# MisEty/X-SLAM

Measured on AMD Instinct MI355X. Metric: fps XKinectFusion 512^3 TSDF 640x480 CSFD @1/2/4/8 GPU; HBM GB/s on integrate, higher is better.
Workload: dtype f32 (complex<f32> CSFD)

## Files before the change

### include/xslam_amd.h

```cpp
#ifndef XSLAM_AMD_H
#define XSLAM_AMD_H
#include <stddef.h>
#include <stdint.h>

#ifdef __cplusplus
extern "C" {
#endif

const char *xs_last_error(void);

unsigned xs_const_div_prepare(float c);
unsigned xs_const_div_state(float c);
int xs_const_div_enable(int on);
int xs_abi_version(void);

int xs_init_volume(float *value, int *weight, float *grad, size_t step_bytes, const int *res, int z0, int z1, void *stream);

int xs_scale_depth(const uint16_t *depth, size_t depth_step, int rows, int cols, float *scaled, size_t scaled_step, void *stream);
int xs_scale_depth_max(const uint16_t *depth, size_t depth_step, int rows, int cols, float *scaled, size_t scaled_step,
                       float *max_dev, void *stream);
size_t xs_depth_tiles_bytes(int rows, int cols);
int xs_scale_depth_tiles(const uint16_t *depth, size_t depth_step, int rows, int cols, float *scaled, size_t scaled_step,
                         float *max_dev, void *tiles_dev, void *stream);
int xs_depth_tiles(const float *scaled, size_t scaled_step, int rows, int cols, void *tiles_dev, void *stream);

int xs_integrate_tsdf_volume(const uint16_t *depth, size_t depth_step, int rows, int cols, const float *intr4, int max_weight,
                             const int *res, float voxel_size, const float *Rv2c18, const float *tv2c6, float tranc_dist,
                             float *value, int *weight, float *grad, size_t vol_step, float *depth_scaled, size_t scaled_step,
                             float threshold, int z0, int z1, unsigned long long *updated_dev, void *stream);
int xs_integrate_scaled(const float *depth_scaled, size_t scaled_step, int rows, int cols, const float *intr4, int max_weight,
                        const int *res, float voxel_size, const float *Rv2c18, const float *tv2c6, float tranc_dist, float *value,
                        int *weight, float *grad, size_t vol_step, float threshold, int z0, int z1,
                        unsigned long long *updated_dev, const float *depth_max_dev, void *workspace, void *stream);
#define XS_INTEGRATE_HEADER_IS_CLEAR 1u
#define XS_INTEGRATE_NO_FOLD 2u
#define XS_INTEGRATE_ALWAYS_STORE 8u
#define XS_INTEGRATE_NO_TILES 32u
#define XS_INTEGRATE_COUNT_CLASSES 64u
#define XS_INTEGRATE_RECLASSIFY_BOXES 128u
#define XS_INTEGRATE_LIST_IS_READY 4u
int xs_integrate_scaled_ex(const float *depth_scaled, size_t scaled_step, int rows, int cols, const float *intr4, int max_weight,
                           const int *res, float voxel_size, const float *Rv2c18, const float *tv2c6, float tranc_dist, float *value,
                           int *weight, float *grad, size_t vol_step, float threshold, int z0, int z1,
                           unsigned long long *updated_dev, const float *depth_max_dev, void *workspace, unsigned flags, void *stream);
int xs_integrate_workspace_clear(void *workspace, void *stream);
int xs_integrate_fold_counts(void *workspace, unsigned long long *updated_dev, void *stream);
int xs_integrate_classify(int rows, int cols, const float *intr4, const int *res, float voxel_size, const float *Rv2c18, const float *tv2c6,
                          float tranc_dist, int z0, int z1, const float *depth_max_dev, void *workspace, float slack_scale, unsigned flags,
                          void *stream);
int xs_integrate_list_covers(int rows, int cols, const float *intr4, const int *res, float voxel_size, const float *Rv2c18_list,
                             const float *tv2c6_list, float slack_scale, const float *Rv2c18, const float *tv2c6);
size_t xs_integrate_workspace_bytes(const int *res, int nz);

typedef struct xs_integrate_opts {
    unsigned struct_bytes;
    unsigned flags;
    const void *depth_tiles;
    void *signmap;
    void *start_event, *stop_event;
} xs_integrate_opts;
int xs_integrate_scaled_ex2(const float *depth_scaled, size_t scaled_step, int rows, int cols, const float *intr4, int max_weight,
                            const int *res, float voxel_size, const float *Rv2c18, const float *tv2c6, float tranc_dist, float *value,
                            int *weight, float *grad, size_t vol_step, float threshold, int z0, int z1,
                            unsigned long long *updated_dev, const float *depth_max_dev, void *workspace, const xs_integrate_opts *opts, void *stream);
int xs_integrate_classify_ex(int rows, int cols, const float *intr4, const int *res, float voxel_size, const float *Rv2c18, const float *tv2c6,
                             float tranc_dist, int z0, int z1, const float *depth_max_dev, void *workspace, float slack_scale,
                             const xs_integrate_opts *opts, void *stream);
typedef struct xs_raycast_opts {
    unsigned struct_bytes;
    int signmap_shift;
    const void *signmap;
    float signmap_tranc_dist;
    float *pyr_vmap1, *pyr_nmap1;
    size_t pyr_step1;
    float *pyr_vmap2, *pyr_nmap2;
    size_t pyr_step2;
    void *completion_event;
    int *steps_dev;
    int pyramid_built;
} xs_raycast_opts;
int xs_raycast_ex(const float *intr4, const float *Rc2v18, const float *tc2v6, const float *Rv2w18, const float *tv2w6,
                  float tranc_dist, const int *res, float voxel_size, const float *value, const float *grad, size_t vol_step,
                  float *vmap, float *nmap, size_t map_step, int rows, int cols, unsigned long long *hits_dev, float *workspace,
                  xs_raycast_opts *opts, void *stream);
int xs_raycast_slab_ex(const float *intr4, const float *Rc2v18, const float *tc2v6, const float *Rv2w18, const float *tv2w6,
                       float tranc_dist, const int *res, float voxel_size, const float *value, const float *grad, size_t vol_step,
                       int zs0, int zs1, int z0, int z1, float *vmap, float *nmap, size_t map_step, int rows, int cols, int *keys_dev,
                       const xs_raycast_opts *opts, void *stream);
int xs_resize_pyramid_ex(const float *vmap0, const float *nmap0, size_t in_step, int rows0, int cols0, float *vmap1, float *nmap1,
                         size_t mid_step, float *vmap2, float *nmap2, size_t out_step, void *completion_event, void *stream);

size_t xs_tsdf_reduce_workspace_bytes(void);
int xs_tsdf_reduce_workspace_init(void *workspace, void *stream);
int xs_compute_local_tsdf_hessian(const float *depth_scaled, size_t scaled_step, int rows, int cols, const float *intr4,
                                  const int *res, float voxel_size, const float *Rv2c36, const float *tv2c12, float tranc_dist,
                                  const float *gt, float *real_out, float *grad_out, float *hess_out, int *count_out, int z0, int z1,
                                  void *workspace, double *out4_dev, void *stream);
int xs_compute_local_tsdf_loss(const float *depth_scaled, size_t scaled_step, int rows, int cols, const float *intr4, const int *res,
                               float voxel_size, const float *Rv2c9, const float *tv2c3, float tranc_dist, const float *gt,
                               float *real_out, int *count_out, int z0, int z1, void *workspace, double *out2_dev, void *stream);

int xs_bilateral_filter(const uint16_t *src, size_t src_step, int rows, int cols, float *dst, size_t dst_step, void *stream);
int xs_pyr_down(const float *src, size_t src_step, int src_rows, int src_cols, float *dst, size_t dst_step, void *stream);
int xs_create_vmap(const float *intr4, const float *depth, size_t depth_step, int rows, int cols, float *vmap, size_t vmap_step,
                   void *stream);
int xs_create_nmap(const float *vmap, float *nmap, size_t map_step, int rows, int cols, void *stream);
int xs_create_vnmaps(int levels, const float *intr4s, const float *const *depths, const size_t *depth_steps, int rows0, int cols0,
                     float *const *vmaps, float *const *nmaps, const size_t *map_steps, void *stream);
int xs_create_vnmaps_real(int levels, const float *intr4s, const float *const *depths, const size_t *depth_steps, int rows0, int cols0,
                          float *const *vmaps, float *const *nmaps, const size_t *map_steps, float *const *vreal, float *const *nreal,
                          const size_t *real_steps, void *stream);
int xs_resize_vmap(const float *in, size_t in_step, int src_rows, int src_cols, float *out, size_t out_step, void *stream);
int xs_resize_nmap(const float *in, size_t in_step, int src_rows, int src_cols, float *out, size_t out_step, void *stream);
int xs_resize_pyramid(const float *vmap0, const float *nmap0, size_t in_step, int rows0, int cols0, float *vmap1, float *nmap1,
                      size_t mid_step, float *vmap2, float *nmap2, size_t out_step, void *stream);

int xs_raycast(const float *intr4, const float *Rc2v18, const float *tc2v6, const float *Rv2w18, const float *tv2w6,
               float tranc_dist, const int *res, float voxel_size, const float *value, const float *grad, size_t vol_step,
               float *vmap, float *nmap, size_t map_step, int rows, int cols, unsigned long long *hits_dev, float *workspace,
               void *stream);

int xs_raycast_signmap_shift(const float *intr4, float voxel_size, float tranc_dist);
size_t xs_signmap_bytes(const int *res, int shift);
int xs_signmap_reset(void *signmap, const int *res, int shift, float tranc_dist, void *stream);
int xs_signmap_rebuild(void *signmap, const int *res, int shift, float tranc_dist, const float *value, size_t vol_step, void *stream);
int xs_signmap_rebuild_slab(void *signmap, const int *res, int shift, float tranc_dist, const float *value, size_t vol_step, int zs0, int zs1,
                            void *stream);


int xs_raycast_slab(const float *intr4, const float *Rc2v18, const float *tc2v6, const float *Rv2w18, const float *tv2w6,
                    float tranc_dist, const int *res, float voxel_size, const float *value, const float *grad, size_t vol_step,
                    int zs0, int zs1, int z0, int z1, float *vmap, float *nmap, size_t map_step, int rows, int cols, int *keys_dev,
                    void *stream);
int xs_raycast_compose_mask(const int *own_keys_dev, const int *min_keys_dev, float *vmap, float *nmap, size_t map_step, int rows,
                            int cols, void *stream);
int xs_raycast_compose_finish(const int *min_keys_dev, float *vmap, float *nmap, size_t map_step, int rows, int cols,
                              unsigned long long *hits_dev, void *stream);
size_t xs_raycast_compose_entry_bytes(void);
int xs_raycast_compose_pack(const int *own_keys_dev, const int *min_keys_dev, const float *vmap, const float *nmap, size_t map_step, int rows, int cols,
                            void *entries_dev, int *count_dev, void *stream);
int xs_raycast_compose_scatter(const void *entries_dev, long n, float *vmap, float *nmap, size_t map_step, int rows, int cols, void *stream);

int xs_tsdf_gauss_newton_terms(const float *depth_scaled, size_t scaled_step, int rows, int cols, const float *intr4, const int *res,
                               float voxel_size, const float *Rv2c108, const float *tv2c36, float tranc_dist, const float *gt, int z0, int z1,
                               void *workspace, double *out29_dev, void *stream);
typedef struct xs_gn_opts {
    unsigned struct_bytes;
    unsigned mailbox_seq;
    const void *pose_mailbox;
    double *publish_host;
    unsigned long long publish_seq;
} xs_gn_opts;
int xs_tsdf_gauss_newton_terms_ex(const float *depth_scaled, size_t scaled_step, int rows, int cols, const float *intr4, const int *res,
                                  float voxel_size, const float *Rv2c108, const float *tv2c36, float tranc_dist, const float *gt, int z0, int z1,
                                  void *workspace, double *out29_dev, const xs_gn_opts *opts, void *stream);
size_t xs_gn_publish_bytes(void);
size_t xs_gn_mailbox_bytes(void);
void xs_gn_post_poses(void *mailbox_host, const float *Rv2c108, const float *tv2c36, unsigned mailbox_seq, int cmd);
int xs_gn_publish_sums(const double *sums_dev, int n, double *publish_host, unsigned long long seq, void *stream);

#define XS_BAND_MAX_FRAMES 32
#define XS_BAND_OVER_CAPACITY (-3)
typedef struct xs_band_index {
    unsigned long long *keys;
    float *values;
    long long capacity;
    long long *segs;
    long long count;
    int nblocks;
    int res[3], z0, z1;
} xs_band_index;
size_t xs_tsdf_band_segs_bytes(const int *res, int z0, int z1);
int xs_tsdf_band_build(const float *gt, const int *res, int z0, int z1, xs_band_index *index, void *stream);
size_t xs_tsdf_band_workspace_bytes(int frames);
int xs_tsdf_gauss_newton_terms_band(int frames, const float *const *depth_scaled, size_t scaled_step, int rows, int cols, const float *intr4,
                                    float voxel_size, const float *Rv2c108xF, const float *tv2c36xF, float tranc_dist, const xs_band_index *index,
                                    void *workspace, double *out29xF_dev, void *stream);
size_t xs_tsdf_pose_hessian_workspace_bytes(int frames);
int xs_tsdf_pose_hessian_band(int frames, const float *const *depth_scaled, size_t scaled_step, int rows, int cols, const float *intr4,
                              float voxel_size, const float *Rv2c36x21xF, const float *tv2c12x21xF, float tranc_dist, const xs_band_index *index,
                              void *workspace, double *out29xF_dev, void *stream);
#define XS_SCORE_MAX_POSES 4096
size_t xs_tsdf_score_poses_workspace_bytes(int poses);
int xs_tsdf_score_poses_band(int poses, const float *depth_scaled, size_t scaled_step, int rows, int cols, const float *intr4,
                             float voxel_size, const float *Rv2c9xP, const float *tv2c3xP, float tranc_dist,
                             const xs_band_index *index, void *workspace, double *out2xP_dev, void *stream);

size_t xs_view_grid_bytes(const int *res);
int xs_view_grid_build(const float *value, const int *weight, size_t vol_step, const int *res, int min_weight, void *grid, void *stream);
int xs_view_grid_expand(const void *grid, const int *res, unsigned char *states_dev, void *stream);
#define XS_VIEW_MAX_POSES 4096
typedef struct xs_view_opts {
    unsigned struct_bytes;
    int rays_x, rays_y;
    float t_near, t_far;
    float step;
} xs_view_opts;
int xs_score_views(int poses, const float *Rc2v9xP, const float *tc2v3xP, const float *intr4, int rows, int cols, const int *res,
                   float voxel_size, const void *grid, const xs_view_opts *opts, unsigned *out4xP_dev, void *stream);

#define XS_CLEARANCE_MAX_RADIUS 255
size_t xs_clearance_bytes(const int *res);
size_t xs_clearance_workspace_bytes(const int *res);
int xs_clearance_build(const void *grid, const int *res, int max_radius, int unknown_blocks, void *workspace, unsigned short *field_dev, void *stream);
#define XS_REACH_MAX_SEEDS 64
size_t xs_reach_bytes(const int *res);
int xs_reach_passable(const void *grid, const unsigned short *field_dev, const int *res, int r2, void *reach, void *stream);
int xs_reach_flood(const void *grid, const unsigned short *field_dev, const int *res, int r2, const int *seeds3xN, int seeds, void *reach,
                   int *rounds_out, void *stream);
int xs_reach_expand(const void *reach, const int *res, int passable, unsigned char *out_dev, void *stream);
#define XS_REACH_MAX_SNAP 16
int xs_reach_query(int n, const float *points3xN_dev, const int *res, float voxel_size, const void *reach, int over_passable,
                   const unsigned short *field_dev, int snap, unsigned char *reachable_dev, unsigned short *clear2_dev, int *voxel3xN_dev,
                   void *stream);

#define XS_TRAVEL_NONE 65535
#define XS_TRAVEL_MAX 65534
#define XS_TRAVEL_MAX_TARGETS 64
size_t xs_travel_bytes(const int *res);
size_t xs_travel_workspace_bytes(void);
int xs_travel_build(const void *reach, const int *res, const int *seeds3xN, int seeds, int limit, unsigned short *travel_dev, void *workspace,
                    int *rounds_out, void *stream);
int xs_travel_query(int n, const int *voxel3xN_dev, const int *res, const unsigned short *travel_dev, unsigned short *out_dev, void *stream);
int xs_travel_path(int n, const int *target3xN_dev, const int *res, const void *reach, const unsigned short *travel_dev, int limit, int capacity,
                   int *path3_dev, int *len_dev, void *stream);

#define XS_FRONTIER_NONE 0xFFFFFFFFu
#define XS_FRONTIER_RECORD_WORDS 8
size_t xs_frontier_mask_bytes(const int *res);
size_t xs_frontier_label_bytes(const int *res);
size_t xs_frontier_workspace_bytes(const int *res, int capacity);
int xs_frontier_mask(const void *grid, const int *res, void *mask, void *stream);
int xs_frontier_label(const void *mask, const int *res, int cell, unsigned *labels_dev, void *workspace, int *rounds_out, void *stream);
int xs_frontier_clusters(const void *mask, const unsigned *labels_dev, const int *res, int capacity, unsigned long long *records_dev,
                         unsigned *count_dev, unsigned *count_host, void *workspace, void *stream);
int xs_frontier_expand(const void *mask, const int *res, unsigned char *out_dev, void *stream);

size_t xs_extract_workspace_bytes(const int *res);
int xs_extract_points(const float *value, size_t vol_step, const int *res, float voxel_size, int zs0, int z0, int z1, float *points_dev,
                      size_t capacity, void *workspace, size_t *count_host, size_t *found_host, void *stream);
int xs_extract_normals(const float *value, size_t vol_step, const int *res, float voxel_size, int zs0, int zs1, const float *points_dev,
                       size_t n, float *normals_dev, void *stream);

#define XS_MESH_OVER_CAPACITY (-2)
typedef struct xs_mesh_opts {
    unsigned struct_bytes;
    int zs0, zs1;
    int z0, z1;
    int min_weight;
    int want_normals;
    const void *signmap;
    int signmap_shift;
} xs_mesh_opts;
size_t xs_mesh_workspace_bytes(const int *res, const xs_mesh_opts *opts);
int xs_extract_mesh(const float *value, const int *weight, const float *grad, size_t vol_step, const int *res, float voxel_size,
                    const xs_mesh_opts *opts, float *vertices_dev, float *vertex_im_dev, float *normals_dev, unsigned long long *keys_dev,
                    size_t vertex_capacity, int *triangles_dev, size_t triangle_capacity, void *workspace, size_t *vertex_count_host,
                    size_t *triangle_count_host, void *stream);
int xs_mesh_case_table(int cube_case, signed char out16[16]);

size_t xs_icp_workspace_bytes(void);
int xs_icp_workspace_init(void *workspace, void *stream);
#define XS_ICP_PUBLISH_PAIRS ((unsigned long long *)(size_t)1)
#define XS_ICP_PAIRS_BYTES (55 * 16)
int xs_icp_wait_pairs(const void *pairs_host, unsigned long long seq, double *sums55, long long max_spins);
int xs_icp_accumulate(const float *Rcurr18, const float *tcurr6, const float *vmap_curr, const float *nmap_curr,
                      const float *Rprev_inv18, const float *tprev6, const float *intr4, const float *vmap_g_prev,
                      const float *nmap_g_prev, size_t map_step, int rows, int cols, float distThres, float angleThres, int y0, int y1,
                      void *workspace, double *sums_dev, unsigned long long *done_flag, unsigned long long done_seq, void *stream);
size_t xs_icp_records_bytes(void);
int xs_icp_records_count(int cols, int y0, int y1);
int xs_icp_accumulate_records(const float *Rcurr18, const float *tcurr6, const void *mailbox, unsigned mailbox_seq, const float *vmap_curr,
                              const float *nmap_curr, const float *Rprev_inv18, const float *tprev6, const float *intr4, const float *vmap_g_prev,
                              const float *nmap_g_prev, size_t map_step, int rows, int cols, float distThres, float angleThres, int y0, int y1,
                              double *records_host, unsigned long long seq, void *stream);
int xs_icp_sum_records(const double *records_host, int count, unsigned long long seq, double *sums55, long long max_spins);

int xs_icp_gate_selftest(const float *z2n_dev, int n, float thres, int or_equal, unsigned *counts_dev, void *stream);
size_t xs_icp_mailbox_bytes(void);
int xs_icp_mailbox_alloc(void **mailbox, int *in_device_memory);
int xs_icp_mailbox_free(void *mailbox, int in_device_memory);
int xs_icp_accumulate_posted(const void *mailbox, unsigned mailbox_seq, const float *vmap_curr, const float *nmap_curr,
                             const float *Rprev_inv18, const float *tprev6, const float *intr4, const float *vmap_g_prev,
                             const float *nmap_g_prev, size_t map_step, int rows, int cols, float distThres, float angleThres, int y0,
                             int y1, void *workspace, double *sums_dev, unsigned long long *done_flag, unsigned long long done_seq,
                             void *stream);
void xs_icp_post_pose(void *mailbox_host, const float *Rcurr18, const float *tcurr6, unsigned mailbox_seq, int cmd);
int xs_icp_accumulate_real(const float *Rcurr18, const float *tcurr6, const float *vmap_curr, const float *nmap_curr,
                           const float *vmap_curr_real, const float *nmap_curr_real, size_t real_step, const float *Rprev_inv18,
                           const float *tprev6, const float *intr4, const float *vmap_g_prev, const float *nmap_g_prev, size_t map_step,
                           int rows, int cols, float distThres, float angleThres, int y0, int y1, void *workspace, double *sums_dev,
                           unsigned long long *done_flag, unsigned long long done_seq, void *stream);
int xs_icp_accumulate_posted_real(const void *mailbox, unsigned mailbox_seq, const float *vmap_curr, const float *nmap_curr,
                                  const float *vmap_curr_real, const float *nmap_curr_real, size_t real_step, const float *Rprev_inv18,
                                  const float *tprev6, const float *intr4, const float *vmap_g_prev, const float *nmap_g_prev,
                                  size_t map_step, int rows, int cols, float distThres, float angleThres, int y0, int y1, void *workspace,
                                  double *sums_dev, unsigned long long *done_flag, unsigned long long done_seq, void *stream);
size_t xs_icp_pose_state_bytes(void);
int xs_icp_iterate(const float *Rcurr18, const float *tcurr6, const float *vmap_curr, const float *nmap_curr,
                   const float *Rprev_inv18, const float *tprev6, const float *intr4, const float *vmap_g_prev,
                   const float *nmap_g_prev, size_t map_step, int rows, int cols, float distThres, float angleThres, void *workspace,
                   double *sums_dev, double *sums_host, void *pose_state, void *pose_state_host, unsigned long long *done_flag,
                   unsigned long long done_seq, void *stream);
int xs_estimate_combined(const float *Rcurr18, const float *tcurr6, const float *vmap_curr, const float *nmap_curr,
                         const float *Rprev_inv18, const float *tprev6, const float *intr4, const float *vmap_g_prev,
                         const float *nmap_g_prev, size_t map_step, int rows, int cols, float distThres, float angleThres,
                         void *workspace, double *sums_dev, double *A72_host, double *b12_host, long long *inliers, void *stream);
void xs_icp_unpack(const double *sums54, double *A72, double *b12);

int xs_csfd_array_op(int which, int our, const float *a, const float *b, float *out, long n, void *stream);
int xs_dcsfd_f1(const float *x, const float *y, float *out, long n, void *stream);
int xs_complex_table(int dual, int op, const float *a, const float *b, float *out, long n, void *stream);

#ifdef __cplusplus
}
#endif
#endif
```

### x-slam_amd/capi.py

```python
import ctypes as C
import os

import numpy as np

_HERE = os.path.dirname(os.path.abspath(__file__))
LIB_PATH = os.path.join(_HERE, "libxslam_hip.so")

_vp = C.c_void_p
_sz = C.c_size_t
_f32p = C.POINTER(C.c_float)
_i32p = C.POINTER(C.c_int)
_f64p = C.POINTER(C.c_double)


class XsError(RuntimeError):
    pass


def _load():
    if not os.path.exists(LIB_PATH):
        raise ImportError(
            f"{LIB_PATH} not found: build the HIP extension first (python -c 'import __graft_entry__ as g; g.build()' "
            "or make -C x-slam_amd/csrc).  There is no CPU fallback.")
    return C.CDLL(LIB_PATH)


_lib = _load()

class IntegrateOpts(C.Structure):
    _fields_ = [("struct_bytes", C.c_uint), ("flags", C.c_uint), ("depth_tiles", C.c_void_p), ("signmap", C.c_void_p),
                ("start_event", C.c_void_p), ("stop_event", C.c_void_p)]


class RaycastOpts(C.Structure):
    _fields_ = [("struct_bytes", C.c_uint), ("signmap_shift", C.c_int), ("signmap", C.c_void_p), ("signmap_tranc_dist", C.c_float),
                ("pyr_vmap1", C.c_void_p), ("pyr_nmap1", C.c_void_p), ("pyr_step1", C.c_size_t), ("pyr_vmap2", C.c_void_p), ("pyr_nmap2", C.c_void_p),
                ("pyr_step2", C.c_size_t), ("completion_event", C.c_void_p), ("steps_dev", C.c_void_p), ("pyramid_built", C.c_int)]


class MeshOpts(C.Structure):
    _fields_ = [("struct_bytes", C.c_uint), ("zs0", C.c_int), ("zs1", C.c_int), ("z0", C.c_int), ("z1", C.c_int), ("min_weight", C.c_int),
                ("want_normals", C.c_int), ("signmap", C.c_void_p), ("signmap_shift", C.c_int)]


class BandIndex(C.Structure):
    _fields_ = [("keys", C.c_void_p), ("values", C.c_void_p), ("capacity", C.c_longlong), ("segs", C.c_void_p), ("count", C.c_longlong),
                ("nblocks", C.c_int), ("res", C.c_int * 3), ("z0", C.c_int), ("z1", C.c_int)]


class ViewOpts(C.Structure):
    _fields_ = [("struct_bytes", C.c_uint), ("rays_x", C.c_int), ("rays_y", C.c_int), ("t_near", C.c_float), ("t_far", C.c_float), ("step", C.c_float)]


_SIGS = {
    "xs_view_grid_bytes": (_sz, [_i32p]),
    "xs_view_grid_build": (C.c_int, [_vp, _vp, _sz, _i32p, C.c_int, _vp, _vp]),
    "xs_view_grid_expand": (C.c_int, [_vp, _i32p, _vp, _vp]),
    "xs_score_views": (C.c_int, [C.c_int, _f32p, _f32p, _f32p, C.c_int, C.c_int, _i32p, C.c_float, _vp, C.POINTER(ViewOpts), _vp, _vp]),
    "xs_clearance_bytes": (_sz, [_i32p]),
    "xs_clearance_workspace_bytes": (_sz, [_i32p]),
    "xs_clearance_build": (C.c_int, [_vp, _i32p, C.c_int, C.c_int, _vp, _vp, _vp]),
    "xs_reach_bytes": (_sz, [_i32p]),
    "xs_reach_passable": (C.c_int, [_vp, _vp, _i32p, C.c_int, _vp, _vp]),
    "xs_reach_flood": (C.c_int, [_vp, _vp, _i32p, C.c_int, _i32p, C.c_int, _vp, _i32p, _vp]),
    "xs_reach_expand": (C.c_int, [_vp, _i32p, C.c_int, _vp, _vp]),
    "xs_reach_query": (C.c_int, [C.c_int, _vp, _i32p, C.c_float, _vp, C.c_int, _vp, C.c_int, _vp, _vp, _vp, _vp]),
    "xs_travel_bytes": (_sz, [_i32p]),
    "xs_travel_workspace_bytes": (_sz, []),
    "xs_travel_build": (C.c_int, [_vp, _i32p, _i32p, C.c_int, C.c_int, _vp, _vp, _i32p, _vp]),
    "xs_travel_query": (C.c_int, [C.c_int, _vp, _i32p, _vp, _vp, _vp]),
    "xs_travel_path": (C.c_int, [C.c_int, _vp, _i32p, _vp, _vp, C.c_int, C.c_int, _vp, _vp, _vp]),
    "xs_frontier_mask_bytes": (_sz, [_i32p]),
    "xs_frontier_label_bytes": (_sz, [_i32p]),
    "xs_frontier_workspace_bytes": (_sz, [_i32p, C.c_int]),
    "xs_frontier_mask": (C.c_int, [_vp, _i32p, _vp, _vp]),
    "xs_frontier_label": (C.c_int, [_vp, _i32p, C.c_int, _vp, _vp, _i32p, _vp]),
    "xs_frontier_clusters": (C.c_int, [_vp, _vp, _i32p, C.c_int, _vp, _vp, C.POINTER(C.c_uint), _vp, _vp]),
    "xs_frontier_expand": (C.c_int, [_vp, _i32p, _vp, _vp]),
    "xs_integrate_scaled_ex2": (C.c_int, [_vp, _sz, C.c_int, C.c_int, _f32p, C.c_int, _i32p, C.c_float, _f32p, _f32p, C.c_float, _vp, _vp, _vp,
                                         _sz, C.c_float, C.c_int, C.c_int, _vp, _vp, _vp, C.POINTER(IntegrateOpts), _vp]),
    "xs_integrate_classify_ex": (C.c_int, [C.c_int, C.c_int, _f32p, _i32p, C.c_float, _f32p, _f32p, C.c_float, C.c_int, C.c_int, _vp, _vp,
                                           C.c_float, C.POINTER(IntegrateOpts), _vp]),
    "xs_raycast_ex": (C.c_int, [_f32p, _f32p, _f32p, _f32p, _f32p, C.c_float, _i32p, C.c_float, _vp, _vp, _sz, _vp, _vp, _sz,
                                C.c_int, C.c_int, _vp, _vp, C.POINTER(RaycastOpts), _vp]),
    "xs_raycast_slab_ex": (C.c_int, [_f32p, _f32p, _f32p, _f32p, _f32p, C.c_float, _i32p, C.c_float, _vp, _vp, _sz, C.c_int, C.c_int,
                                     C.c_int, C.c_int, _vp, _vp, _sz, C.c_int, C.c_int, _vp, C.POINTER(RaycastOpts), _vp]),
    "xs_resize_pyramid_ex": (C.c_int, [_vp, _vp, _sz, C.c_int, C.c_int, _vp, _vp, _sz, _vp, _vp, _sz, _vp, _vp]),
    "xs_last_error": (C.c_char_p, []),
    "xs_abi_version": (C.c_int, []),
    "xs_init_volume": (C.c_int, [_vp, _vp, _vp, _sz, _i32p, C.c_int, C.c_int, _vp]),
    "xs_scale_depth": (C.c_int, [_vp, _sz, C.c_int, C.c_int, _vp, _sz, _vp]),
    "xs_integrate_tsdf_volume": (C.c_int, [_vp, _sz, C.c_int, C.c_int, _f32p, C.c_int, _i32p, C.c_float, _f32p, _f32p, C.c_float,
                                           _vp, _vp, _vp, _sz, _vp, _sz, C.c_float, C.c_int, C.c_int, _vp, _vp]),
    "xs_integrate_scaled": (C.c_int, [_vp, _sz, C.c_int, C.c_int, _f32p, C.c_int, _i32p, C.c_float, _f32p, _f32p, C.c_float,
                                      _vp, _vp, _vp, _sz, C.c_float, C.c_int, C.c_int, _vp, _vp, _vp, _vp]),
    "xs_integrate_scaled_ex": (C.c_int, [_vp, _sz, C.c_int, C.c_int, _f32p, C.c_int, _i32p, C.c_float, _f32p, _f32p, C.c_float, _vp, _vp, _vp,
                                        _sz, C.c_float, C.c_int, C.c_int, _vp, _vp, _vp, C.c_uint, _vp]),
    "xs_integrate_workspace_clear": (C.c_int, [_vp, _vp]),
    "xs_integrate_fold_counts": (C.c_int, [_vp, _vp, _vp]),
    "xs_integrate_classify": (C.c_int, [C.c_int, C.c_int, _f32p, _i32p, C.c_float, _f32p, _f32p, C.c_float, C.c_int, C.c_int, _vp, _vp,
                                        C.c_float, C.c_uint, _vp]),
    "xs_integrate_list_covers": (C.c_int, [C.c_int, C.c_int, _f32p, _i32p, C.c_float, _f32p, _f32p, C.c_float, _f32p, _f32p]),
    "xs_integrate_workspace_bytes": (_sz, [_i32p, C.c_int]),
    "xs_scale_depth_max": (C.c_int, [_vp, _sz, C.c_int, C.c_int, _vp, _sz, _vp, _vp]),
    "xs_scale_depth_tiles": (C.c_int, [_vp, _sz, C.c_int, C.c_int, _vp, _sz, _vp, _vp, _vp]),
    "xs_depth_tiles": (C.c_int, [_vp, _sz, C.c_int, C.c_int, _vp, _vp]),
    "xs_depth_tiles_bytes": (_sz, [C.c_int, C.c_int]),
    "xs_tsdf_reduce_workspace_bytes": (_sz, []),
    "xs_tsdf_band_segs_bytes": (_sz, [_i32p, C.c_int, C.c_int]),
    "xs_tsdf_band_build": (C.c_int, [_vp, _i32p, C.c_int, C.c_int, C.POINTER(BandIndex), _vp]),
    "xs_tsdf_band_workspace_bytes": (_sz, [C.c_int]),
    "xs_tsdf_gauss_newton_terms_band": (C.c_int, [C.c_int, C.POINTER(_vp), _sz, C.c_int, C.c_int, _f32p, C.c_float, _f32p, _f32p, C.c_float,
                                                  C.POINTER(BandIndex), _vp, _vp, _vp]),
    "xs_tsdf_pose_hessian_workspace_bytes": (_sz, [C.c_int]),
    "xs_tsdf_pose_hessian_band": (C.c_int, [C.c_int, C.POINTER(_vp), _sz, C.c_int, C.c_int, _f32p, C.c_float, _f32p, _f32p, C.c_float,
                                            C.POINTER(BandIndex), _vp, _vp, _vp]),
    "xs_tsdf_score_poses_workspace_bytes": (_sz, [C.c_int]),
    "xs_tsdf_score_poses_band": (C.c_int, [C.c_int, _vp, _sz, C.c_int, C.c_int, _f32p, C.c_float, _f32p, _f32p, C.c_float, C.POINTER(BandIndex), _vp,
                                           _vp, _vp]),
    "xs_tsdf_reduce_workspace_init": (C.c_int, [_vp, _vp]),
    "xs_compute_local_tsdf_hessian": (C.c_int, [_vp, _sz, C.c_int, C.c_int, _f32p, _i32p, C.c_float, _f32p, _f32p, C.c_float, _vp,
                                                _vp, _vp, _vp, _vp, C.c_int, C.c_int, _vp, _vp, _vp]),
    "xs_compute_local_tsdf_loss": (C.c_int, [_vp, _sz, C.c_int, C.c_int, _f32p, _i32p, C.c_float, _f32p, _f32p, C.c_float, _vp,
                                             _vp, _vp, C.c_int, C.c_int, _vp, _vp, _vp]),
    "xs_bilateral_filter": (C.c_int, [_vp, _sz, C.c_int, C.c_int, _vp, _sz, _vp]),
    "xs_pyr_down": (C.c_int, [_vp, _sz, C.c_int, C.c_int, _vp, _sz, _vp]),
    "xs_create_vmap": (C.c_int, [_f32p, _vp, _sz, C.c_int, C.c_int, _vp, _sz, _vp]),
    "xs_create_nmap": (C.c_int, [_vp, _vp, _sz, C.c_int, C.c_int, _vp]),
    "xs_create_vnmaps": (C.c_int, [C.c_int, _f32p, C.POINTER(_vp), C.POINTER(_sz), C.c_int, C.c_int, C.POINTER(_vp), C.POINTER(_vp),
                                   C.POINTER(_sz), _vp]),
    "xs_create_vnmaps_real": (C.c_int, [C.c_int, _f32p, C.POINTER(_vp), C.POINTER(_sz), C.c_int, C.c_int, C.POINTER(_vp), C.POINTER(_vp),
                                        C.POINTER(_sz), C.POINTER(_vp), C.POINTER(_vp), C.POINTER(_sz), _vp]),
    "xs_resize_vmap": (C.c_int, [_vp, _sz, C.c_int, C.c_int, _vp, _sz, _vp]),
    "xs_resize_nmap": (C.c_int, [_vp, _sz, C.c_int, C.c_int, _vp, _sz, _vp]),
    "xs_raycast": (C.c_int, [_f32p, _f32p, _f32p, _f32p, _f32p, C.c_float, _i32p, C.c_float, _vp, _vp, _sz, _vp, _vp, _sz,
                             C.c_int, C.c_int, _vp, _vp, _vp]),
    "xs_raycast_slab": (C.c_int, [_f32p, _f32p, _f32p, _f32p, _f32p, C.c_float, _i32p, C.c_float, _vp, _vp, _sz, C.c_int, C.c_int,
                                  C.c_int, C.c_int, _vp, _vp, _sz, C.c_int, C.c_int, _vp, _vp]),
    "xs_raycast_compose_mask": (C.c_int, [_vp, _vp, _vp, _vp, _sz, C.c_int, C.c_int, _vp]),
    "xs_raycast_compose_finish": (C.c_int, [_vp, _vp, _vp, _sz, C.c_int, C.c_int, _vp, _vp]),
    "xs_raycast_compose_entry_bytes": (_sz, []),
    "xs_raycast_compose_pack": (C.c_int, [_vp, _vp, _vp, _vp, _sz, C.c_int, C.c_int, _vp, _vp, _vp]),
    "xs_raycast_compose_scatter": (C.c_int, [_vp, C.c_long, _vp, _vp, _sz, C.c_int, C.c_int, _vp]),
    "xs_resize_pyramid": (C.c_int, [_vp, _vp, _sz, C.c_int, C.c_int, _vp, _vp, _sz, _vp, _vp, _sz, _vp]),
    "xs_tsdf_gauss_newton_terms": (C.c_int, [_vp, _sz, C.c_int, C.c_int, _f32p, _i32p, C.c_float, _f32p, _f32p, C.c_float, _vp, C.c_int,
                                             C.c_int, _vp, _vp, _vp]),
    "xs_tsdf_gauss_newton_terms_ex": (C.c_int, [_vp, _sz, C.c_int, C.c_int, _f32p, _i32p, C.c_float, _f32p, _f32p, C.c_float, _vp, C.c_int,
                                                C.c_int, _vp, _vp, _vp, _vp]),
    "xs_gn_publish_bytes": (_sz, []),
    "xs_gn_mailbox_bytes": (_sz, []),
    "xs_gn_post_poses": (None, [_vp, _f32p, _f32p, C.c_uint, C.c_int]),
    "xs_gn_publish_sums": (C.c_int, [_vp, C.c_int, _vp, C.c_ulonglong, _vp]),
    "xs_extract_workspace_bytes": (_sz, [_i32p]),
    "xs_extract_points": (C.c_int, [_vp, _sz, _i32p, C.c_float, C.c_int, C.c_int, C.c_int, _vp, _sz, _vp, C.POINTER(_sz), C.POINTER(_sz), _vp]),
    "xs_extract_normals": (C.c_int, [_vp, _sz, _i32p, C.c_float, C.c_int, C.c_int, _vp, _sz, _vp, _vp]),
    "xs_mesh_workspace_bytes": (_sz, [_i32p, C.POINTER(MeshOpts)]),
    "xs_extract_mesh": (C.c_int, [_vp, _vp, _vp, _sz, _i32p, C.c_float, C.POINTER(MeshOpts), _vp, _vp, _vp, _vp, _sz, _vp, _sz, _vp,
                                  C.POINTER(_sz), C.POINTER(_sz), _vp]),
    "xs_mesh_case_table": (C.c_int, [C.c_int, C.c_void_p]),
    "xs_icp_wait_pairs": (C.c_int, [_vp, C.c_ulonglong, _vp, C.c_longlong]),
    "xs_icp_workspace_bytes": (_sz, []),
    "xs_icp_workspace_init": (C.c_int, [_vp, _vp]),
    "xs_icp_accumulate": (C.c_int, [_f32p, _f32p, _vp, _vp, _f32p, _f32p, _f32p, _vp, _vp, _sz, C.c_int, C.c_int, C.c_float,
                                    C.c_float, C.c_int, C.c_int, _vp, _vp, _vp, C.c_ulonglong, _vp]),
    "xs_icp_pose_state_bytes": (_sz, []),
    "xs_icp_mailbox_bytes": (_sz, []),
    "xs_icp_mailbox_alloc": (C.c_int, [C.POINTER(C.c_void_p), C.POINTER(C.c_int)]),
    "xs_icp_mailbox_free": (C.c_int, [_vp, C.c_int]),
    "xs_icp_accumulate_posted": (C.c_int, [_vp, C.c_uint, _vp, _vp, _f32p, _f32p, _f32p, _vp, _vp, _sz, C.c_int, C.c_int, C.c_float,
                                           C.c_float, C.c_int, C.c_int, _vp, _vp, _vp, C.c_ulonglong, _vp]),
    "xs_icp_post_pose": (None, [_vp, _f32p, _f32p, C.c_uint, C.c_int]),
    "xs_icp_accumulate_real": (C.c_int, [_f32p, _f32p, _vp, _vp, _vp, _vp, _sz, _f32p, _f32p, _f32p, _vp, _vp, _sz, C.c_int, C.c_int, C.c_float,
                                         C.c_float, C.c_int, C.c_int, _vp, _vp, _vp, C.c_ulonglong, _vp]),
    "xs_icp_accumulate_posted_real": (C.c_int, [_vp, C.c_uint, _vp, _vp, _vp, _vp, _sz, _f32p, _f32p, _f32p, _vp, _vp, _sz, C.c_int, C.c_int,
                                                C.c_float, C.c_float, C.c_int, C.c_int, _vp, _vp, _vp, C.c_ulonglong, _vp]),
    "xs_icp_records_bytes": (_sz, []),
    "xs_icp_records_count": (C.c_int, [C.c_int, C.c_int, C.c_int]),
    "xs_icp_accumulate_records": (C.c_int, [_f32p, _f32p, _vp, C.c_uint, _vp, _vp, _f32p, _f32p, _f32p, _vp, _vp, _sz, C.c_int, C.c_int, C.c_float,
                                            C.c_float, C.c_int, C.c_int, _vp, C.c_ulonglong, _vp]),
    "xs_icp_sum_records": (C.c_int, [_vp, C.c_int, C.c_ulonglong, _f64p, C.c_longlong]),
    "xs_icp_gate_selftest": (C.c_int, [_vp, C.c_int, C.c_float, C.c_int, _vp, _vp]),
    "xs_icp_iterate": (C.c_int, [_f32p, _f32p, _vp, _vp, _f32p, _f32p, _f32p, _vp, _vp, _sz, C.c_int, C.c_int, C.c_float,
                                 C.c_float, _vp, _vp, _vp, _vp, _vp, _vp, C.c_ulonglong, _vp]),
    "xs_estimate_combined": (C.c_int, [_f32p, _f32p, _vp, _vp, _f32p, _f32p, _f32p, _vp, _vp, _sz, C.c_int, C.c_int, C.c_float,
                                       C.c_float, _vp, _vp, _f64p, _f64p, C.POINTER(C.c_longlong), _vp]),
    "xs_icp_unpack": (None, [_f64p, _f64p, _f64p]),
    "xs_csfd_array_op": (C.c_int, [C.c_int, C.c_int, _vp, _vp, _vp, C.c_long, _vp]),
    "xs_dcsfd_f1": (C.c_int, [_vp, _vp, _vp, C.c_long, _vp]),
    "xs_complex_table": (C.c_int, [C.c_int, C.c_int, _vp, _vp, _vp, C.c_long, _vp]),
    "xs_const_div_prepare": (C.c_uint, [C.c_float]),
    "xs_raycast_signmap_shift": (C.c_int, [_f32p, C.c_float, C.c_float]),
    "xs_signmap_bytes": (C.c_size_t, [_i32p, C.c_int]),
    "xs_signmap_reset": (C.c_int, [_vp, _i32p, C.c_int, C.c_float, _vp]),
    "xs_signmap_rebuild": (C.c_int, [_vp, _i32p, C.c_int, C.c_float, _vp, C.c_size_t, _vp]),
    "xs_signmap_rebuild_slab": (C.c_int, [_vp, _i32p, C.c_int, C.c_float, _vp, C.c_size_t, C.c_int, C.c_int, _vp]),
    "xs_const_div_state": (C.c_uint, [C.c_float]),
    "xs_const_div_enable": (C.c_int, [C.c_int]),
}


def _bind():
    for name, (res, args) in _SIGS.items():
        f = getattr(_lib, name)
        f.restype = res
        f.argtypes = args


_bind()


def const_div_prepare(c):
    return int(_lib.xs_const_div_prepare(float(c)))


def const_div_state(c):
    return int(_lib.xs_const_div_state(float(c)))


def const_div_enable(on):
    return int(_lib.xs_const_div_enable(int(bool(on))))


_prepared = set()


def _prep(*consts):
    for c in consts:
        c = float(np.float32(c))
        if c not in _prepared:
            _prepared.add(c)
            _lib.xs_const_div_prepare(c)


def check(rc):
    if rc != 0:
        raise XsError(f"hip error {rc}: {_lib.xs_last_error().decode()}")


def _fa(x, n):
    a = np.ascontiguousarray(x, dtype=np.float32).reshape(-1)
    assert a.size == n, (a.size, n)
    return a


def _ia(x, n):
    a = np.ascontiguousarray(x, dtype=np.int32).reshape(-1)
    assert a.size == n
    return a


def _ptr(t):
    if t is None:
        return None
    if isinstance(t, int):
        return t
    return t.data_ptr()


def _stream(stream):
    if stream is None:
        return None
    return stream.cuda_stream if hasattr(stream, "cuda_stream") else int(stream)


def abi_version():
    return _lib.xs_abi_version()
# ... 303 lines not shown
    k, R, t, r = _fa(intr, 4), _fa(R, 9 * P), _fa(tc2vxP, 3 * P), _ia(res, 3)
    check(_lib.xs_score_views(P, R.ctypes.data_as(_f32p), t.ctypes.data_as(_f32p), k.ctypes.data_as(_f32p), rows, cols, r.ctypes.data_as(_i32p),
                              voxel_size, _ptr(grid), C.byref(opts) if opts is not None else None, _ptr(out4xP), _stream(stream)))


CLEARANCE_MAX_RADIUS, REACH_MAX_SEEDS, REACH_MAX_SNAP = 255, 64, 16


def _res3(res):
    r = np.ascontiguousarray(res, dtype=np.int32).reshape(-1)
    assert r.size == 3
    return r


def clearance_bytes(res):
    return int(_lib.xs_clearance_bytes(_res3(res).ctypes.data_as(_i32p)))


def clearance_workspace_bytes(res):
    return int(_lib.xs_clearance_workspace_bytes(_res3(res).ctypes.data_as(_i32p)))


def reach_bytes(res):
    return int(_lib.xs_reach_bytes(_res3(res).ctypes.data_as(_i32p)))


def clearance_build(grid, res, max_radius, unknown_blocks, workspace, field, stream=None):
    r = _res3(res)
    check(_lib.xs_clearance_build(_ptr(grid), r.ctypes.data_as(_i32p), int(max_radius), int(unknown_blocks), _ptr(workspace), _ptr(field), _stream(stream)))


def reach_passable(grid, field, res, r2, reach, stream=None):
    r = _res3(res)
    check(_lib.xs_reach_passable(_ptr(grid), _ptr(field), r.ctypes.data_as(_i32p), int(r2), _ptr(reach), _stream(stream)))


def reach_flood(grid, field, res, r2, seeds, reach, stream=None):
    r = _res3(res)
    s = np.ascontiguousarray(seeds, dtype=np.int32).reshape(-1)
    assert s.size % 3 == 0
    rounds = C.c_int(-1)
    check(_lib.xs_reach_flood(_ptr(grid), _ptr(field), r.ctypes.data_as(_i32p), int(r2), s.ctypes.data_as(_i32p), s.size // 3, _ptr(reach),
                              C.byref(rounds), _stream(stream)))
    return int(rounds.value)


def reach_expand(reach, res, out, passable=False, stream=None):
    r = _res3(res)
    check(_lib.xs_reach_expand(_ptr(reach), r.ctypes.data_as(_i32p), int(bool(passable)), _ptr(out), _stream(stream)))


def reach_query(n, points, res, voxel_size, reach, field, reachable, clear2, snap=0, over_passable=False, voxel=None, stream=None):
    r = _res3(res)
    check(_lib.xs_reach_query(int(n), _ptr(points), r.ctypes.data_as(_i32p), float(voxel_size), _ptr(reach), int(bool(over_passable)), _ptr(field),
                              int(snap), _ptr(reachable), _ptr(clear2), _ptr(voxel), _stream(stream)))


TRAVEL_NONE, TRAVEL_MAX, TRAVEL_MAX_TARGETS = 65535, 65534, 64


def travel_bytes(res):
    return int(_lib.xs_travel_bytes(_res3(res).ctypes.data_as(_i32p)))


def travel_workspace_bytes():
    return int(_lib.xs_travel_workspace_bytes())


def travel_build(reach, res, seeds, limit, travel, workspace, stream=None):
    r = _res3(res)
    s = np.ascontiguousarray(seeds, dtype=np.int32).reshape(-1)
    assert s.size % 3 == 0
    rounds = C.c_int(0)
    check(_lib.xs_travel_build(_ptr(reach), r.ctypes.data_as(_i32p), s.ctypes.data_as(_i32p), s.size // 3, int(limit), _ptr(travel), _ptr(workspace),
                               C.byref(rounds), _stream(stream)))
    return int(rounds.value)


def travel_query(n, voxels, res, travel, out, stream=None):
    r = _res3(res)
    check(_lib.xs_travel_query(int(n), _ptr(voxels), r.ctypes.data_as(_i32p), _ptr(travel), _ptr(out), _stream(stream)))


def travel_path(n, targets, res, reach, travel, limit, capacity, path, lengths, stream=None):
    r = _res3(res)
    check(_lib.xs_travel_path(int(n), _ptr(targets), r.ctypes.data_as(_i32p), _ptr(reach), _ptr(travel), int(limit), int(capacity), _ptr(path),
                              _ptr(lengths), _stream(stream)))


FRONTIER_NONE, FRONTIER_RECORD_WORDS = 0xFFFFFFFF, 8


def frontier_mask_bytes(res):
    return int(_lib.xs_frontier_mask_bytes(_res3(res).ctypes.data_as(_i32p)))


def frontier_label_bytes(res):
    return int(_lib.xs_frontier_label_bytes(_res3(res).ctypes.data_as(_i32p)))


def frontier_workspace_bytes(res, capacity=0):
    return int(_lib.xs_frontier_workspace_bytes(_res3(res).ctypes.data_as(_i32p), int(capacity)))


def frontier_mask(grid, res, mask, stream=None):
    r = _res3(res)
    check(_lib.xs_frontier_mask(_ptr(grid), r.ctypes.data_as(_i32p), _ptr(mask), _stream(stream)))


def frontier_label(mask, res, cell, labels, workspace, stream=None):
    r = _res3(res)
    rounds = C.c_int(0)
    check(_lib.xs_frontier_label(_ptr(mask), r.ctypes.data_as(_i32p), int(cell), _ptr(labels), _ptr(workspace), C.byref(rounds), _stream(stream)))
    return int(rounds.value)


def frontier_clusters(mask, labels, res, capacity, records, count, workspace, stream=None):
    r = _res3(res)
    n = C.c_uint(0)
    check(_lib.xs_frontier_clusters(_ptr(mask), _ptr(labels), r.ctypes.data_as(_i32p), int(capacity), _ptr(records), _ptr(count), C.byref(n), _ptr(workspace),
                                    _stream(stream)))
    return int(n.value)


def frontier_expand(mask, res, out, stream=None):
    r = _res3(res)
    check(_lib.xs_frontier_expand(_ptr(mask), r.ctypes.data_as(_i32p), _ptr(out), _stream(stream)))



class GnOpts(C.Structure):
    _fields_ = [("struct_bytes", C.c_uint), ("mailbox_seq", C.c_uint), ("pose_mailbox", C.c_void_p), ("publish_host", C.c_void_p),
                ("publish_seq", C.c_ulonglong)]


def tsdf_gauss_newton_terms_ex(depth_scaled, scaled_step, rows, cols, intr, res, voxel_size, Rv2c6, tv2c6, tranc_dist, gt, workspace, out29,
                               z0=0, z1=None, stream=None, pose_mailbox=None, mailbox_seq=0, publish_host=None, publish_seq=0):
    r = _ia(res, 3)
    k = _fa(intr, 4)
    z1 = int(r[2]) if z1 is None else z1
    o = GnOpts()
    o.struct_bytes = C.sizeof(GnOpts)
    o.mailbox_seq, o.pose_mailbox, o.publish_host, o.publish_seq = mailbox_seq, _ptr(pose_mailbox), _ptr(publish_host), publish_seq
    if Rv2c6 is None:
        pR = pt = None
    else:
        R, t = _fa(Rv2c6, 108), _fa(tv2c6, 36)
        pR, pt = R.ctypes.data_as(_f32p), t.ctypes.data_as(_f32p)
    check(_lib.xs_tsdf_gauss_newton_terms_ex(_ptr(depth_scaled), scaled_step, rows, cols, k.ctypes.data_as(_f32p), r.ctypes.data_as(_i32p),
                                             voxel_size, pR, pt, tranc_dist, _ptr(gt), z0, z1, _ptr(workspace), _ptr(out29), C.byref(o),
                                             _stream(stream)))


def gn_publish_bytes():
    return int(_lib.xs_gn_publish_bytes())


def gn_post_poses(mailbox, Rv2c6, tv2c6, mailbox_seq, cmd=0):
    if Rv2c6 is None:
        _lib.xs_gn_post_poses(_ptr(mailbox), None, None, mailbox_seq, cmd)
    else:
        R, t = _fa(Rv2c6, 108), _fa(tv2c6, 36)
        _lib.xs_gn_post_poses(_ptr(mailbox), R.ctypes.data_as(_f32p), t.ctypes.data_as(_f32p), mailbox_seq, cmd)


def extract_workspace_bytes(res):
    r = _ia(res, 3)
    return _lib.xs_extract_workspace_bytes(r.ctypes.data_as(_i32p))


def extract_points(value, vol_step, res, voxel_size, points, capacity, workspace, zs0=0, z0=0, z1=None, stream=None):
    r = _ia(res, 3)
    z1 = int(r[2]) - 1 if z1 is None else z1
    cnt, found = _sz(0), _sz(0)
    check(_lib.xs_extract_points(_ptr(value), vol_step, r.ctypes.data_as(_i32p), voxel_size, zs0, z0, z1, _ptr(points), capacity,
                                 _ptr(workspace), C.byref(cnt), C.byref(found), _stream(stream)))
    return int(cnt.value), int(found.value)


def extract_normals(value, vol_step, res, voxel_size, points, n, normals, zs0=0, zs1=None, stream=None):
    r = _ia(res, 3)
    zs1 = int(r[2]) if zs1 is None else zs1
    check(_lib.xs_extract_normals(_ptr(value), vol_step, r.ctypes.data_as(_i32p), voxel_size, zs0, zs1, _ptr(points), n, _ptr(normals),
                                  _stream(stream)))


MESH_OVER_CAPACITY = -2


def mesh_opts(z0=0, z1=None, res=None, zs0=0, zs1=0, min_weight=1, want_normals=True, signmap=None, signmap_shift=3):
    o = MeshOpts()
    o.struct_bytes = C.sizeof(MeshOpts)
    o.zs0, o.zs1, o.z0 = zs0, zs1, z0
    o.z1 = int(res[2]) - 1 if z1 is None else z1
    o.min_weight, o.want_normals = min_weight, int(bool(want_normals))
    o.signmap, o.signmap_shift = _ptr(signmap), signmap_shift if signmap is not None else 0
    return o


def mesh_workspace_bytes(res, opts=None):
    r = _ia(res, 3)
    return _lib.xs_mesh_workspace_bytes(r.ctypes.data_as(_i32p), C.byref(opts) if opts is not None else None)


def mesh_case_table(cube_case):
    out = (C.c_byte * 16)()
    check(_lib.xs_mesh_case_table(int(cube_case), out))
    e = [v for v in out if v >= 0]
    return [tuple(e[i:i + 3]) for i in range(0, len(e), 3)]


def extract_mesh_raw(value, weight, grad, vol_step, res, voxel_size, opts, vertices, vertex_im, normals, keys, vcap, triangles, tcap,
                     workspace, stream=None):
    r = _ia(res, 3)
    nv, nt = _sz(0), _sz(0)
    rc = _lib.xs_extract_mesh(_ptr(value), _ptr(weight), _ptr(grad), vol_step, r.ctypes.data_as(_i32p), voxel_size, C.byref(opts),
                              _ptr(vertices), _ptr(vertex_im), _ptr(normals), _ptr(keys), vcap, _ptr(triangles), tcap, _ptr(workspace),
                              C.byref(nv), C.byref(nt), _stream(stream))
    if rc != MESH_OVER_CAPACITY:
        check(rc)
    return rc, int(nv.value), int(nt.value)


def extract_mesh(value, weight, grad, vol_step, res, voxel_size, z0=0, z1=None, zs0=0, zs1=0, min_weight=1, want_normals=True,
                 signmap=None, signmap_shift=3, stream=None):
    import torch
    dev = value.device
    opts = mesh_opts(z0, z1, res, zs0, zs1, min_weight, want_normals, signmap, signmap_shift)
    ws = torch.empty(max(1, mesh_workspace_bytes(res, opts)), dtype=torch.uint8, device=dev)
    args = (value, weight, grad, vol_step, res, voxel_size, opts)
    rc, nv, nt = extract_mesh_raw(*args, None, None, None, None, 0, None, 0, ws, stream)
    f = lambda n: torch.empty((n, 3), dtype=torch.float32, device=dev)
    out = {"vertices": f(nv), "vertex_im": f(nv) if grad is not None else None, "normals": f(nv) if want_normals else None,
           "triangles": torch.empty((nt, 3), dtype=torch.int32, device=dev), "edge_keys": torch.empty(nv, dtype=torch.uint64, device=dev)}
    if rc == MESH_OVER_CAPACITY:
        rc, nv2, nt2 = extract_mesh_raw(*args, out["vertices"], out["vertex_im"], out["normals"], out["edge_keys"], nv, out["triangles"], nt,
                                        ws, stream)
        assert rc == 0 and (nv2, nt2) == (nv, nt), (rc, nv2, nt2, nv, nt)
    return out


def resize_pyramid(vmap0, nmap0, in_step, rows0, cols0, vmap1, nmap1, mid_step, vmap2, nmap2, out_step, stream=None):
    check(_lib.xs_resize_pyramid(_ptr(vmap0), _ptr(nmap0), in_step, rows0, cols0, _ptr(vmap1), _ptr(nmap1), mid_step, _ptr(vmap2), _ptr(nmap2),
                                 out_step, _stream(stream)))


def create_nmap(vmap, nmap, map_step, rows, cols, stream=None):
    check(_lib.xs_create_nmap(_ptr(vmap), _ptr(nmap), map_step, rows, cols, _stream(stream)))


def resize_vmap(src, src_step, src_rows, src_cols, dst, dst_step, stream=None):
    check(_lib.xs_resize_vmap(_ptr(src), src_step, src_rows, src_cols, _ptr(dst), dst_step, _stream(stream)))


def resize_nmap(src, src_step, src_rows, src_cols, dst, dst_step, stream=None):
    check(_lib.xs_resize_nmap(_ptr(src), src_step, src_rows, src_cols, _ptr(dst), dst_step, _stream(stream)))


def raycast(intr, Rc2v, tc2v, Rv2w, tv2w, tranc_dist, res, voxel_size, value, grad, vol_step, vmap, nmap, map_step, rows, cols,
            hits=None, workspace=None, stream=None, **opts):
    if opts:
        o = _ray_opts(opts)
        raycast_ex(intr, Rc2v, tc2v, Rv2w, tv2w, tranc_dist, res, voxel_size, value, grad, vol_step, vmap, nmap, map_step, rows, cols, o, hits=hits,
                   workspace=workspace, stream=stream)
        return o
    r = _ia(res, 3)
    _prep(voxel_size)
    k, a, b, c, d = _fa(intr, 4), _fa(Rc2v, 18), _fa(tc2v, 6), _fa(Rv2w, 18), _fa(tv2w, 6)
    P = lambda x: x.ctypes.data_as(_f32p)
    check(_lib.xs_raycast(P(k), P(a), P(b), P(c), P(d), tranc_dist, r.ctypes.data_as(_i32p), voxel_size, _ptr(value), _ptr(grad),
                          vol_step, _ptr(vmap), _ptr(nmap), map_step, rows, cols, _ptr(hits), _ptr(workspace), _stream(stream)))


def _ray_opts(kw):
    kw = dict(kw)
    if "signmap_shift" in kw:
        kw["shift"] = kw.pop("signmap_shift")
    if "signmap_tranc_dist" in kw:
        kw["tranc_dist"] = kw.pop("signmap_tranc_dist")
    return raycast_opts(**kw)


def raycast_opts(signmap=None, shift=3, tranc_dist=0.0, pyramid=None, completion_event=None, steps=None):
    o = RaycastOpts()
    o.struct_bytes = C.sizeof(RaycastOpts)
    o.signmap, o.signmap_shift, o.signmap_tranc_dist = _ptr(signmap), shift, tranc_dist
    if pyramid is not None:
        o.pyr_vmap1, o.pyr_nmap1, o.pyr_step1, o.pyr_vmap2, o.pyr_nmap2, o.pyr_step2 = (_ptr(pyramid[0]), _ptr(pyramid[1]), pyramid[2],
                                                                                       _ptr(pyramid[3]), _ptr(pyramid[4]), pyramid[5])
    o.completion_event = completion_event.value if hasattr(completion_event, "value") else completion_event
    o.steps_dev = _ptr(steps)
    return o


def raycast_ex(intr, Rc2v, tc2v, Rv2w, tv2w, tranc_dist, res, voxel_size, value, grad, vol_step, vmap, nmap, map_step, rows, cols, opts,
               hits=None, workspace=None, stream=None):
    _prep(voxel_size)
    r = _ia(res, 3)
    k = _fa(intr, 4)
    a, b, c, d = _fa(Rc2v, 18), _fa(tc2v, 6), _fa(Rv2w, 18), _fa(tv2w, 6)
    P = lambda x: x.ctypes.data_as(_f32p)
    check(_lib.xs_raycast_ex(P(k), P(a), P(b), P(c), P(d), tranc_dist, r.ctypes.data_as(_i32p), voxel_size, _ptr(value), _ptr(grad), vol_step,
                             _ptr(vmap), _ptr(nmap), map_step, rows, cols, _ptr(hits), _ptr(workspace), C.byref(opts), _stream(stream)))


def raycast_signmap_shift(intr, voxel_size, tranc_dist):
# ... 212 lines not shown
```

### x-slam_amd/csrc/xs_band.hip

```cpp
#include <hip/hip_runtime.h>
#include <string.h>
#include <type_traits>
#include <vector>
#include "xs_gn_band.h"
#include "../../include/xslam_amd.h"

static_assert(XS_BAND_MAX_FRAMES == 32, "the header's bound");
enum { BAND_RECORD_DOUBLES = 32, BAND_POSES_OFFSET = 256 };
static size_t band_records_offset() { return BAND_POSES_OFFSET + (size_t)XS_BAND_MAX_FRAMES * sizeof(GnPoses); }

__device__ __forceinline__ unsigned long long band_key(int x, int y, int z) {
    return (unsigned long long)x | ((unsigned long long)y << 21) | ((unsigned long long)z << 42);
}

template <bool WRITE>
__global__ void __launch_bounds__(256) k_band_record(const HessArgs a, long long *segs, unsigned long long *keys, unsigned *values) {
    const int lane = threadIdx.x, wave = threadIdx.y;
    const unsigned nseg = gridDim.x * 4u, seg = blockIdx.x * 4u + (unsigned)wave;
    const long long base = WRITE ? segs[seg] : 0;
    long long k = 0;
    walk_band(a, [&](int x, int y, int z, size_t, float gt) {
        if (WRITE) {
            const long long e = base + 64 * k + lane;
            keys[e] = band_key(x, y, z);
            values[e] = __float_as_uint(gt);
        }
        ++k;
    });
    if (!WRITE) {
        const unsigned long long n = wave_sum_u64((unsigned long long)k);
        if (lane == 0) segs[nseg + seg] = (long long)n;
    }
}

struct BandGnArgs {
    HessArgs a;
    const float *depth[XS_BAND_MAX_FRAMES];
    const unsigned long long *keys;
    const float *values;
    const long long *segs;
    const GnPoses *poses;
    double *records;
    unsigned *tickets;
    double *out;
};
__global__ void __launch_bounds__(256) k_band_gauss_newton(const BandGnArgs g) {
    __shared__ GnPoses P;
    const int f = blockIdx.y, lane = threadIdx.x, wave = threadIdx.y;
    const unsigned nblocks = gridDim.x, nseg = 4u * nblocks, seg = blockIdx.x * 4u + (unsigned)wave;
    {
        const float *src = reinterpret_cast<const float *>(g.poses + f);
        float *dst = reinterpret_cast<float *>(&P);
        for (int i = threadIdx.y * 64 + threadIdx.x; i < (int)(sizeof(GnPoses) / sizeof(float)); i += 256) dst[i] = src[i];
        __syncthreads();
    }
    HessArgs a = g.a;
    a.depth = g.depth[f];
    double acc[29];
#pragma unroll
    for (int k = 0; k < 29; ++k) acc[k] = 0.0;
    const long long off = g.segs[seg], n = g.segs[nseg + seg];
    for (long long e = lane; e < n; e += 64) {
        const unsigned long long key = g.keys[off + e];
        const int x = (int)(key & 0x1fffff), y = (int)((key >> 21) & 0x1fffff), z = (int)(key >> 42);
        gn_terms_add(a, P, x, y, z, g.values[off + e], acc);
    }
    block_fold_and_finish_of<29>(acc, g.records + (size_t)f * nblocks * BAND_RECORD_DOUBLES, g.tickets + f, g.out + 29 * f, nullptr, 0, false,
                                 nblocks, blockIdx.x);
}

extern "C" size_t xs_tsdf_band_segs_bytes(const int *res, int z0, int z1) {
    if (!res || z0 < 0 || z1 > res[2] || z1 <= z0) return 0;
    unsigned most = 0;
    for (uintptr_t addr : {(uintptr_t)256, (uintptr_t)4}) {
        HessArgs a; dim3 grid;
        if (hess_tiling(a, res, reinterpret_cast<const float *>(addr), z0, z1, grid, true)) return 0;
        most = grid.x > most ? grid.x : most;
    }
    return (size_t)most * 4 * 2 * sizeof(long long);
}

extern "C" int xs_tsdf_band_build(const float *gt, const int *res, int z0, int z1, xs_band_index *index, void *stream) {
    if (!gt || !res || !index || !index->segs) return xs_set_error(hipErrorInvalidValue, "xs_tsdf_band_build: null pointer");
    if (z0 < 0 || z1 > res[2] || z1 <= z0) return xs_set_error(hipErrorInvalidValue, "xs_tsdf_band_build: bad slab");
    if (index->capacity > 0 && (!index->keys || !index->values)) return xs_set_error(hipErrorInvalidValue, "xs_tsdf_band_build: capacity without arrays");
    if ((long long)res[0] > 0x1fffff || (long long)res[1] > 0x1fffff || (long long)res[2] > 0x3fffff)
        return xs_set_error(hipErrorInvalidValue, "xs_tsdf_band_build: volume too large for the packed keys");
    hipStream_t st = (hipStream_t)stream;
    HessArgs a; dim3 grid;
    memset(&a, 0, sizeof(a));
    int rc = hess_tiling(a, res, gt, z0, z1, grid, true);
    if (rc) return rc;
    const unsigned nseg = grid.x * 4u;
    index->count = 0; index->nblocks = 0;
    hipLaunchKernelGGL(k_band_record<false>, grid, dim3(64, 4), 0, st, a, index->segs, nullptr, nullptr);
    XS_CHECK(hipGetLastError());
    std::vector<long long> segs(2 * (size_t)nseg);
    XS_CHECK(hipMemcpyAsync(segs.data() + nseg, index->segs + nseg, nseg * sizeof(long long), hipMemcpyDeviceToHost, st));
    XS_CHECK(hipStreamSynchronize(st));
    long long total = 0;
    for (unsigned s = 0; s < nseg; ++s) { segs[s] = total; total += segs[nseg + s]; }
    index->count = total;
    index->nblocks = (int)grid.x;
    index->res[0] = res[0]; index->res[1] = res[1]; index->res[2] = res[2];
    index->z0 = z0; index->z1 = z1;
    if (total > index->capacity) return XS_BAND_OVER_CAPACITY;
    XS_CHECK(hipMemcpyAsync(index->segs, segs.data(), nseg * sizeof(long long), hipMemcpyHostToDevice, st));
    hipLaunchKernelGGL(k_band_record<true>, grid, dim3(64, 4), 0, st, a, index->segs, index->keys, reinterpret_cast<unsigned *>(index->values));
    XS_CHECK(hipGetLastError());
    XS_CHECK(hipStreamSynchronize(st));
    return 0;
}

extern "C" size_t xs_tsdf_band_workspace_bytes(int frames) {
    if (frames < 1 || frames > XS_BAND_MAX_FRAMES) return 0;
    return band_records_offset() + (size_t)frames * XS_TSDF_REDUCE_MAX_BLOCKS_C * BAND_RECORD_DOUBLES * sizeof(double);
}

extern "C" int xs_tsdf_gauss_newton_terms_band(int frames, const float *const *depth_scaled, size_t scaled_step, int rows, int cols, const float *intr4,
                                               float voxel_size, const float *Rv2c108xF, const float *tv2c36xF, float tranc_dist,
                                               const xs_band_index *index, void *workspace, double *out29xF_dev, void *stream) {
    if (frames < 1 || frames > XS_BAND_MAX_FRAMES) return xs_set_error(hipErrorInvalidValue, "xs_tsdf_gauss_newton_terms_band: frames outside 1 .. XS_BAND_MAX_FRAMES");
    if (!depth_scaled || !intr4 || !Rv2c108xF || !tv2c36xF || !index || !workspace || !out29xF_dev)
        return xs_set_error(hipErrorInvalidValue, "xs_tsdf_gauss_newton_terms_band: null pointer");
    if (index->nblocks < 1 || index->nblocks > XS_TSDF_REDUCE_MAX_BLOCKS_C || !index->segs || (index->count > 0 && (!index->keys || !index->values)))
        return xs_set_error(hipErrorInvalidValue, "xs_tsdf_gauss_newton_terms_band: the index was not built");
    BandGnArgs g;
    memset(&g, 0, sizeof(g));
    for (int f = 0; f < frames; ++f) {
        if (!depth_scaled[f]) return xs_set_error(hipErrorInvalidValue, "xs_tsdf_gauss_newton_terms_band: null depth");
        g.depth[f] = depth_scaled[f];
    }
    HessArgs &a = g.a;
    a.depth = depth_scaled[0]; a.dstep = scaled_step; a.drows = rows; a.dcols = cols;
    a.voxel_size = voxel_size; a.tranc_dist = tranc_dist; a.tranc_dist_inv = 1.0f / tranc_dist;
    a.intr = Intr{intr4[0], intr4[1], intr4[2], intr4[3]};
    a.X = index->res[0]; a.Y = index->res[1]; a.Z = index->res[2]; a.z0 = index->z0; a.z1 = index->z1;
    std::vector<GnPoses> P((size_t)frames);
    memset(P.data(), 0, P.size() * sizeof(GnPoses));
    for (int f = 0; f < frames; ++f)
        for (int k = 0; k < 6; ++k) { load_mat(Rv2c108xF + 108 * f + 18 * k, P[f].R[k]); load_vec(tv2c36xF + 36 * f + 6 * k, P[f].t[k]); }
    char *ws = static_cast<char *>(workspace);
    g.tickets = reinterpret_cast<unsigned *>(ws);
    g.poses = reinterpret_cast<const GnPoses *>(ws + BAND_POSES_OFFSET);
    g.records = reinterpret_cast<double *>(ws + band_records_offset());
    g.keys = index->keys; g.values = index->values; g.segs = index->segs; g.out = out29xF_dev;
    hipStream_t st = (hipStream_t)stream;
    XS_CHECK(hipMemcpyAsync(ws + BAND_POSES_OFFSET, P.data(), P.size() * sizeof(GnPoses), hipMemcpyHostToDevice, st));
    hipLaunchKernelGGL(k_band_gauss_newton, dim3((unsigned)index->nblocks, (unsigned)frames), dim3(64, 4), 0, st, g);
    XS_CHECK(hipGetLastError());
    return 0;
}

enum { NEWTON_PAIRS = 21, NEWTON_TERMS = 28, NEWTON_POSES_OFFSET = 256 };
static size_t newton_records_offset() { return NEWTON_POSES_OFFSET + (size_t)XS_BAND_MAX_FRAMES * NEWTON_PAIRS * sizeof(HessPoseD); }
static_assert(sizeof(HessPoseD) == 48 * sizeof(float), "36 + 12 floats per dual-complex pose");

struct BandHessArgs {
    HessArgs a;
    const float *depth[XS_BAND_MAX_FRAMES];
    const unsigned long long *keys;
    const float *values;
    long long count;
    const HessPoseD *poses;
    double *records;
    unsigned *tickets;
    double *out;
};
__global__ void __launch_bounds__(256) k_band_pose_hessian(const BandHessArgs g) {
    __shared__ HessPoseD P[NEWTON_PAIRS];
    __shared__ float s_term[NEWTON_TERMS][256];
    const int f = blockIdx.y, lane = threadIdx.x, wave = threadIdx.y, tid = wave * 64 + lane;
    {
        const float *src = reinterpret_cast<const float *>(g.poses + (size_t)f * NEWTON_PAIRS);
        float *dst = reinterpret_cast<float *>(&P[0]);
        for (int i = tid; i < (int)(NEWTON_PAIRS * sizeof(HessPoseD) / sizeof(float)); i += 256) dst[i] = src[i];
        __syncthreads();
    }
    HessArgs a = g.a;
    a.depth = g.depth[f];
    double acc[29];
#pragma unroll
    for (int k = 0; k < 29; ++k) acc[k] = 0.0;
    const long long nchunks = (g.count + 63) / 64;
    for (long long c = (long long)blockIdx.x * 4 + wave; c < nchunks; c += 4ll * gridDim.x) {
        const long long e = c * 64 + lane;
        if (e >= g.count) continue;
        const unsigned long long key = g.keys[e];
        const int x = (int)(key & 0x1fffff), y = (int)((key >> 21) & 0x1fffff), z = (int)(key >> 42);
        const float gt = g.values[e];
        bool ok = true;
        int pa = 0, pb = 0;
#pragma unroll 1
        for (int p = 0; p < NEWTON_PAIRS; ++p) {
            dcfloat loss;
            if (!tsdf_loss_d(a, P[p], x, y, z, gt, loss)) { ok = false; break; }
            s_term[p][tid] = loss.hessian();
            if (pa == pb) s_term[NEWTON_PAIRS + pa][tid] = loss.grad();
            if (p == 0) s_term[27][tid] = loss.value();
            if (++pb == 6) { ++pa; pb = pa; }
        }
        if (!ok) continue;
#pragma unroll
        for (int k = 0; k < NEWTON_TERMS; ++k) acc[k] += (double)s_term[k][tid];
        acc[28] += 1.0;
    }
    block_fold_and_finish_of<29>(acc, g.records + (size_t)f * gridDim.x * BAND_RECORD_DOUBLES, g.tickets + f, g.out + 29 * f, nullptr, 0, false,
                                 gridDim.x, blockIdx.x);
}

extern "C" size_t xs_tsdf_pose_hessian_workspace_bytes(int frames) {
    if (frames < 1 || frames > XS_BAND_MAX_FRAMES) return 0;
    return newton_records_offset() + (size_t)frames * XS_TSDF_REDUCE_MAX_BLOCKS_C * BAND_RECORD_DOUBLES * sizeof(double);
}

extern "C" int xs_tsdf_pose_hessian_band(int frames, const float *const *depth_scaled, size_t scaled_step, int rows, int cols, const float *intr4,
                                         float voxel_size, const float *Rv2c36x21xF, const float *tv2c12x21xF, float tranc_dist,
                                         const xs_band_index *index, void *workspace, double *out29xF_dev, void *stream) {
    if (frames < 1 || frames > XS_BAND_MAX_FRAMES) return xs_set_error(hipErrorInvalidValue, "xs_tsdf_pose_hessian_band: frames outside 1 .. XS_BAND_MAX_FRAMES");
    if (!depth_scaled || !intr4 || !Rv2c36x21xF || !tv2c12x21xF || !index || !workspace || !out29xF_dev)
        return xs_set_error(hipErrorInvalidValue, "xs_tsdf_pose_hessian_band: null pointer");
    if (index->nblocks < 1 || index->count < 0 || index->count > index->capacity || (index->count > 0 && (!index->keys || !index->values)))
        return xs_set_error(hipErrorInvalidValue, "xs_tsdf_pose_hessian_band: the index was not built");
    if (rows < 4 || cols < 4 || scaled_step < (size_t)cols * sizeof(float)) return xs_set_error(hipErrorInvalidValue, "xs_tsdf_pose_hessian_band: bad depth shape");
    BandHessArgs g;
    memset(&g, 0, sizeof(g));
    for (int f = 0; f < frames; ++f) {
        if (!depth_scaled[f]) return xs_set_error(hipErrorInvalidValue, "xs_tsdf_pose_hessian_band: null depth");
        g.depth[f] = depth_scaled[f];
    }
    HessArgs &a = g.a;
    a.depth = depth_scaled[0]; a.dstep = scaled_step; a.drows = rows; a.dcols = cols;
    a.voxel_size = voxel_size; a.tranc_dist = tranc_dist; a.tranc_dist_inv = 1.0f / tranc_dist;
    a.intr = Intr{intr4[0], intr4[1], intr4[2], intr4[3]};
    a.X = index->res[0]; a.Y = index->res[1]; a.Z = index->res[2]; a.z0 = index->z0; a.z1 = index->z1;
    std::vector<HessPoseD> P((size_t)frames * NEWTON_PAIRS);
    for (size_t k = 0; k < P.size(); ++k) {
        const float *p = Rv2c36x21xF + 36 * k, *t = tv2c12x21xF + 12 * k;
        for (int r = 0; r < 3; ++r) {
            P[k].R.data[r].x = dcfloat(p[12 * r + 0], p[12 * r + 1], p[12 * r + 2], p[12 * r + 3]);
            P[k].R.data[r].y = dcfloat(p[12 * r + 4], p[12 * r + 5], p[12 * r + 6], p[12 * r + 7]);
            P[k].R.data[r].z = dcfloat(p[12 * r + 8], p[12 * r + 9], p[12 * r + 10], p[12 * r + 11]);
        }
        P[k].t.x = dcfloat(t[0], t[1], t[2], t[3]);
        P[k].t.y = dcfloat(t[4], t[5], t[6], t[7]);
        P[k].t.z = dcfloat(t[8], t[9], t[10], t[11]);
    }
    const long long nchunks = (index->count + 63) / 64, want = (nchunks + 3) / 4;
    const unsigned nblocks = (unsigned)(want < 1 ? 1 : (want > XS_TSDF_REDUCE_MAX_BLOCKS_C ? XS_TSDF_REDUCE_MAX_BLOCKS_C : want));
    char *ws = static_cast<char *>(workspace);
    g.tickets = reinterpret_cast<unsigned *>(ws);
    g.poses = reinterpret_cast<const HessPoseD *>(ws + NEWTON_POSES_OFFSET);
    g.records = reinterpret_cast<double *>(ws + newton_records_offset());
    g.keys = index->keys; g.values = index->values; g.count = index->count; g.out = out29xF_dev;
    hipStream_t st = (hipStream_t)stream;
    XS_CHECK(hipMemcpyAsync(ws + NEWTON_POSES_OFFSET, P.data(), P.size() * sizeof(HessPoseD), hipMemcpyHostToDevice, st));
    hipLaunchKernelGGL(k_band_pose_hessian, dim3(nblocks, (unsigned)frames), dim3(64, 4), 0, st, g);
    XS_CHECK(hipGetLastError());
    return 0;
}

enum { SCORE_TILE = 64, SCORE_POSES_OFFSET = 256, SCORE_MAX_BLOCKS = 1024, SCORE_RECORD_BYTES = SCORE_TILE * (sizeof(double) + sizeof(unsigned)) };
static_assert(XS_SCORE_MAX_POSES / SCORE_TILE * sizeof(unsigned) == SCORE_POSES_OFFSET, "one ticket per tile in the first 256 bytes");
static_assert(sizeof(HessPoseF) == 12 * sizeof(float), "twelve floats per real pose");
static size_t score_records_offset() { return SCORE_POSES_OFFSET + (size_t)XS_SCORE_MAX_POSES * sizeof(HessPoseF); }

__device__ __forceinline__ float wave_tree_sum_f32(float v) {
    auto dpp = [](float x, auto ctrl) { return __int_as_float(__builtin_amdgcn_update_dpp(0, __float_as_int(x), decltype(ctrl)::value, 0xf, 0xf, false)); };
    v += dpp(v, std::integral_constant<int, 0xb1>());
    v += dpp(v, std::integral_constant<int, 0x4e>());
    v += dpp(v, std::integral_constant<int, 0x141>());
    v += dpp(v, std::integral_constant<int, 0x140>());
    v += __shfl_xor(v, 16, 64);
    v += __shfl_xor(v, 32, 64);
    return v;
}

struct BandScoreArgs {
    HessArgs a;
    const unsigned long long *keys;
    const float *values;
    long long count;
    int poses;
    const HessPoseF *poses_dev;
    char *records;
    unsigned *tickets;
    double *out;
};
__global__ void __launch_bounds__(256) k_band_score_poses(const BandScoreArgs g) {
    __shared__ double s_sum[4][SCORE_TILE];
    __shared__ unsigned s_cnt[4][SCORE_TILE];
    __shared__ unsigned s_last;
    const int lane = threadIdx.x, wave = __builtin_amdgcn_readfirstlane(threadIdx.y), tid = wave * 64 + lane;
    const unsigned nblocks = gridDim.x, bid = blockIdx.x, tile = blockIdx.y;
    const int p0 = (int)tile * SCORE_TILE, np = min(SCORE_TILE, g.poses - p0);
    const HessPoseF *__restrict__ poses = g.poses_dev + p0;
    double acc = 0.0;
    unsigned cnt = 0;
    const long long nchunks = (g.count + 63) / 64;
    for (long long c = (long long)bid * 4 + wave; c < nchunks; c += 4ll * nblocks) {
        const long long e = c * 64 + lane;
        const bool valid = e < g.count;
// ... 103 lines not shown
```

### x-slam_amd/csrc/xs_gn_band.h

```cpp
#pragma once
#include "xs_device.h"
#include "xs_env.h"

using namespace xs;
#if defined(__HIP_DEVICE_COMPILE__) && !defined(__gfx942__) && !defined(__gfx950__)
#error "write-through record publish: gfx942 / gfx950 only (use a release fence + acq_rel ticket on other targets)"
#endif

struct HessArgs {
    const float *depth; size_t dstep; int drows, dcols;
    int X, Y, Z, z0, z1, zchunk;
    float voxel_size, tranc_dist, tranc_dist_inv;
    Intr intr;
    const float *gt;
    double *partials;
    unsigned *ticket;
    double *out;
    float *real_out, *grad_out, *hess_out; int *count_out;
    int tiles_x, tiles_y, tiles_z;
    double *publish; unsigned long long publish_seq;
    const unsigned *mailbox; unsigned mailbox_seq;
    int il;
    int wide;
};
struct HessPoseD { MatD33 R; dcfloat3 t; };
struct HessPoseF { float R[9]; float t[3]; };

enum { XS_TSDF_REDUCE_MAX_BLOCKS_C = 4096 };
enum : unsigned { TICKET_ARRIVED = 1u, TICKET_LEFT = 0x10000u, TICKET_COUNT_MASK = 0xffffu };
template <int NV>
__device__ __forceinline__ void block_fold_and_finish_of(double (&v)[NV], double *partials, unsigned *ticket, double *out, double *publish,
                                                         unsigned long long publish_seq, bool left, unsigned nblocks, unsigned bid) {
    constexpr int STRIDE = NV <= 8 ? 8 : 32;
    __shared__ double sm[4][NV];
    __shared__ unsigned s_last;
    const int tid = threadIdx.y * blockDim.x + threadIdx.x;
    const int lane = tid & 63, wave = tid >> 6;
    if (!left) {
#pragma unroll
        for (int k = 0; k < NV; ++k) {
            const double s = wave_sum_f64(v[k]);
            if (lane == 0) sm[wave][k] = s;
        }
        __syncthreads();
        if (tid < NV) {
            const double s = ((sm[0][tid] + sm[1][tid]) + sm[2][tid]) + sm[3][tid];
            __hip_atomic_store(&partials[(size_t)bid * STRIDE + tid], s, __ATOMIC_RELAXED, __HIP_MEMORY_SCOPE_AGENT);
        }
    }
    static_assert(NV <= 64, "the record is stored by one wave");
    static_assert(XS_TSDF_REDUCE_MAX_BLOCKS_C <= (int)TICKET_COUNT_MASK, "the ticket counts arrivals in sixteen bits");
    if (wave == 0) asm volatile("s_waitcnt vmcnt(0)" ::: "memory");
    if (tid == 0) {
        const unsigned tk = __hip_atomic_fetch_add(ticket, left ? TICKET_ARRIVED + TICKET_LEFT : TICKET_ARRIVED, __ATOMIC_RELAXED, __HIP_MEMORY_SCOPE_AGENT);
        s_last = (tk & TICKET_COUNT_MASK) != nblocks - 1 ? 0u : ((tk >> 16) != 0 || left ? 2u : 1u);
        if (s_last) __builtin_amdgcn_fence(__ATOMIC_ACQUIRE, "agent");
        asm volatile("s_waitcnt vmcnt(0)" ::: "memory");
    }
    __syncthreads();
    if (s_last == 2u) {
        if (tid == 0) {
            __hip_atomic_store(ticket, 0u, __ATOMIC_RELAXED, __HIP_MEMORY_SCOPE_AGENT);
            if (publish) __hip_atomic_store(reinterpret_cast<unsigned long long *>(publish) + 32, publish_seq | (1ull << 63), __ATOMIC_RELAXED, __HIP_MEMORY_SCOPE_SYSTEM);
        }
        return;
    }
    if (s_last) {
        constexpr int G = 256 / STRIDE;
        __shared__ double s_red[G][STRIDE];
        const int c = tid % STRIDE, g = tid / STRIDE;
        const double *p = partials + c;
        double s = 0.0;
        unsigned b = g;
        for (; b + G * 15 < nblocks; b += G * 16) {
            double v[16];
#pragma unroll
            for (int k = 0; k < 16; ++k) v[k] = p[(size_t)(b + G * k) * STRIDE];
#pragma unroll
            for (int k = 0; k < 16; ++k) s += v[k];
        }
        for (; b < nblocks; b += G) s += p[(size_t)b * STRIDE];
        s_red[g][c] = s;
        __syncthreads();
        if (tid < NV) {
            double t = s_red[0][tid];
#pragma unroll
            for (int gg = 1; gg < G; ++gg) t += s_red[gg][tid];
            out[tid] = t;
            if (publish) __hip_atomic_store(&publish[tid], t, __ATOMIC_RELAXED, __HIP_MEMORY_SCOPE_SYSTEM);
        }
        if (tid == 0) __hip_atomic_store(ticket, 0u, __ATOMIC_RELAXED, __HIP_MEMORY_SCOPE_AGENT);
        if (publish && wave == 0) {
            __builtin_amdgcn_fence(__ATOMIC_RELEASE, "");
            if (tid == 0) __hip_atomic_store(reinterpret_cast<unsigned long long *>(publish) + 32, publish_seq, __ATOMIC_RELAXED, __HIP_MEMORY_SCOPE_SYSTEM);
        }
    }
}

template <int NV>
__device__ __forceinline__ void block_fold_and_finish(double (&v)[NV], double *partials, unsigned *ticket, double *out, double *publish = nullptr,
                                                      unsigned long long publish_seq = 0, bool left = false) {
    block_fold_and_finish_of(v, partials, ticket, out, publish, publish_seq, left, gridDim.x * gridDim.y * gridDim.z,
                             blockIdx.x + gridDim.x * (blockIdx.y + gridDim.y * blockIdx.z));
}

struct BandQueue {
    enum { CAP = 128 };
    unsigned long long (*q)[CAP];
    unsigned head, tail;
};
template <class F>
__device__ __forceinline__ void band_queue_take(const HessArgs &a, BandQueue &Q, int wave, int lane, unsigned count, F &&body) {
    asm volatile("s_waitcnt lgkmcnt(0)" ::: "memory");
    if ((unsigned)lane < count) {
        const unsigned long long e = Q.q[wave][(Q.head + lane) % BandQueue::CAP];
        const int x = (int)(e & 0x1fffff), y = (int)((e >> 21) & 0x1fffff), z = (int)(e >> 42);
        const size_t index = ((size_t)(z - a.z0) * a.Y + y) * a.X + x;
        body(x, y, z, index, a.gt[index]);
    }
    Q.head += count;
    asm volatile("s_waitcnt lgkmcnt(0)" ::: "memory");
}
template <class F, class XYZ>
__device__ __forceinline__ void band_queue_append(const HessArgs &a, BandQueue &Q, int wave, int lane, bool mine, XYZ &&xyz, F &&body) {
    const unsigned long long who = __ballot(mine);
    if (!who) return;
    if (mine) {
        const unsigned pos = Q.tail + __popcll(who & ((1ull << lane) - 1ull));
        Q.q[wave][pos % BandQueue::CAP] = xyz();
    }
    Q.tail += (unsigned)__popcll(who);
    if (Q.tail - Q.head >= 64u) band_queue_take(a, Q, wave, lane, 64u, body);
}
typedef float xs_f4 __attribute__((ext_vector_type(4)));
template <class F>
__device__ __forceinline__ void for_band_voxels(const HessArgs &a, BandQueue &Q, int wave, int lane, int x, int y, bool in_volume, int zb, int ze,
                                                F &&body) {
    constexpr int ZB = 32;
    const size_t plane = (size_t)a.Y * a.X;
    const size_t first = in_volume ? (size_t)(zb - a.z0) * plane + (size_t)y * a.X + x : 0;
    for (int zc = zb; zc < ze; zc += ZB) {
        const float *col = a.gt + first + (size_t)(zc - zb) * plane;
        unsigned mask = 0;
        if (in_volume) {
#pragma unroll
            for (int j = 0; j < ZB; ++j) {
                const float g = (zc + j < ze) ? col[(size_t)j * plane] : 0.f;
                if (!(g == 0 || fabsf(g) > 0.95)) mask |= 1u << j;
            }
        }
        if (!__ballot(mask != 0)) continue;
        for (int j = 0; j < ZB; ++j)
            band_queue_append(a, Q, wave, lane, (mask >> j) & 1u,
                              [&] { return (unsigned long long)x | ((unsigned long long)y << 21) | ((unsigned long long)(zc + j) << 42); }, body);
    }
}
template <class F>
__device__ __forceinline__ void for_band_voxels_wide(const HessArgs &a, BandQueue &Q, int wave, int lane, int x0, int y, bool in_volume, int zfirst, int zstep, int zend,
                                                     F &&body) {
    constexpr int ZB = 8;
    const size_t plane = (size_t)a.Y * a.X;
    const int il = a.il;
    auto zof = [&](int zc, int j) { return zc + (j % il) + (j / il) * il * zstep; };
    const float *col = a.gt + (in_volume ? (size_t)(zfirst - a.z0) * plane + (size_t)y * a.X + x0 : 0);
    for (int zc = zfirst; zc < zend; zc += ZB * zstep, col += (size_t)ZB * zstep * plane) {
        unsigned mask = 0;
        if (in_volume) {
            xs_f4 v[ZB];
#pragma unroll
            for (int j = 0; j < ZB; ++j)
                v[j] = (zof(zc, j) < zend) ? __builtin_nontemporal_load(reinterpret_cast<const xs_f4 *>(col + (size_t)(zof(zc, j) - zc) * plane)) : xs_f4{0.f, 0.f, 0.f, 0.f};
#pragma unroll
            for (int j = 0; j < ZB; ++j) {
                if (!(v[j].x == 0 || fabsf(v[j].x) > 0.95)) mask |= 1u << (4 * j);
                if (!(v[j].y == 0 || fabsf(v[j].y) > 0.95)) mask |= 2u << (4 * j);
                if (!(v[j].z == 0 || fabsf(v[j].z) > 0.95)) mask |= 4u << (4 * j);
                if (!(v[j].w == 0 || fabsf(v[j].w) > 0.95)) mask |= 8u << (4 * j);
            }
        }
        if (!__ballot(mask != 0)) continue;
        for (int b = 0; b < 32; ++b)
            band_queue_append(a, Q, wave, lane, (mask >> b) & 1u,
                              [&] { return (unsigned long long)(x0 + (b & 3)) | ((unsigned long long)y << 21) | ((unsigned long long)zof(zc, b >> 2) << 42); }, body);
    }
}
template <class F>
__device__ __forceinline__ void walk_band(const HessArgs &a, F &&body) {
    __shared__ unsigned long long s_queue[4][BandQueue::CAP];
    BandQueue Q{s_queue, 0u, 0u};
    const int lane = threadIdx.x, wave = threadIdx.y;
    const int ntiles = a.tiles_x * a.tiles_y * a.tiles_z;
    const bool skew = a.wide == 2 && (gridDim.x % (unsigned)a.tiles_z) == 0;
    for (int tile = blockIdx.x, round = 0; tile < ntiles; tile += gridDim.x, ++round) {
        if (a.wide == 2) {
            const int G = a.tiles_z, column = tile / G, g = (tile % G + (skew ? round : 0)) % G;
            const int x0 = 4 * (int)threadIdx.x + (column % a.tiles_x) * 256, y = threadIdx.y + (column / a.tiles_x) * 4;
            for_band_voxels_wide(a, Q, wave, lane, x0, y, x0 < a.X && y < a.Y, a.z0 + g * a.il, G, a.z1, body);
            continue;
        }
        const int y = threadIdx.y + ((tile / a.tiles_x) % a.tiles_y) * 4;
        const int zb = a.z0 + (tile / (a.tiles_x * a.tiles_y)) * a.zchunk, ze = min(zb + a.zchunk, a.z1);
        if (a.wide) {
            const int x0 = 4 * (int)threadIdx.x + (tile % a.tiles_x) * 256;
            for_band_voxels_wide(a, Q, wave, lane, x0, y, x0 < a.X && y < a.Y, zb, 1, ze, body);
        } else {
            const int x = threadIdx.x + (tile % a.tiles_x) * 64;
            for_band_voxels(a, Q, wave, lane, x, y, x < a.X && y < a.Y, zb, ze, body);
        }
    }
    band_queue_take(a, Q, wave, lane, Q.tail - Q.head, body);
}

struct GnPoses { MatS33 R[6]; cfloat3 t[6]; };
__device__ __forceinline__ bool tsdf_error_c(const HessArgs &a, const MatS33 &R, const cfloat3 &t, float vgx, float vgy, float vgz, float gt,
                                             cfloat &error) {
    cfloat3 v_g; v_g.x = cfloat(vgx); v_g.y = cfloat(vgy); v_g.z = cfloat(vgz);
    cfloat3 v_c;
    v_c.x = dot(R.data[0], v_g) + t.x;
    v_c.y = dot(R.data[1], v_g) + t.y;
    v_c.z = dot(R.data[2], v_g) + t.z;
    const cfloat inv_z = cfloat(1.0f) / v_c.z;
    if (inv_z.re < 0) return false;
    const cfloat image_x = v_c.x * inv_z * a.intr.fx + a.intr.cx;
    const cfloat image_y = v_c.y * inv_z * a.intr.fy + a.intr.cy;
    const int coo_x = __float2int_rd(image_x.re - 0.5f), coo_y = __float2int_rd(image_y.re - 0.5f);
    if (!(coo_x > 1 && coo_y > 1 && coo_x < a.dcols - 1 && coo_y < a.drows - 1)) return false;
    const int near_x = __float2int_rn(image_x.re), near_y = __float2int_rn(image_y.re);
    cfloat Dp(row_ptr(a.depth, a.dstep, near_y)[near_x]);
    const float d00 = row_ptr(a.depth, a.dstep, coo_y)[coo_x], d10 = row_ptr(a.depth, a.dstep, coo_y)[coo_x + 1];
    const float d01 = row_ptr(a.depth, a.dstep, coo_y + 1)[coo_x], d11 = row_ptr(a.depth, a.dstep, coo_y + 1)[coo_x + 1];
    if (d00 != 0.0f && d01 != 0.0f && d10 != 0.0f && d11 != 0.0f) {
        const cfloat one(1.0f);
        const cfloat fa = image_x - cfloat(float(coo_x) + 0.5f);
        const cfloat fb = image_y - cfloat(float(coo_y) + 0.5f);
        Dp = d00 * (one - fa) * (one - fb) + d10 * fa * (one - fb) + d01 * (one - fa) * fb + d11 * fa * fb;
    }
    if (Dp.re > 5 || Dp.re < 0.2) return false;
    const cfloat xl = (image_x - a.intr.cx) / a.intr.fx;
    const cfloat yl = (image_y - a.intr.cy) / a.intr.fy;
    const cfloat3 v_c_1 = mk3(Dp * xl, Dp * yl, Dp);
    const cfloat distance = norm(v_c_1) - norm(v_c);
    const cfloat gt_distance = cfloat(gt) * a.tranc_dist;
    error = (distance - gt_distance) * a.tranc_dist_inv;
    return !(fabsf(error.re) > 1);
}

__device__ __forceinline__ void gn_terms_add(const HessArgs &a, const GnPoses &P, int xq, int yq, int z, float gt, double (&acc)[29]) {
    const float vgx = (float(xq) + 0.5f) * a.voxel_size, vgy = (float(yq) + 0.5f) * a.voxel_size, vgz = (float(z) + 0.5f) * a.voxel_size;
    cfloat e[6];
    bool ok = true;
#pragma unroll
    for (int k = 0; k < 6; ++k) {
        ok = ok && tsdf_error_c(a, P.R[k], P.t[k], vgx, vgy, vgz, gt, e[k]);
        asm volatile("" : "+v"(e[k].re), "+v"(e[k].im) :: "memory");
    }
    if (!ok) return;
    const double r = (double)e[0].re;
    int s = 0;
#pragma unroll
    for (int j = 0; j < 6; ++j)
#pragma unroll
        for (int k = j; k < 6; ++k) acc[s++] += (double)e[j].im * (double)e[k].im;
#pragma unroll
    for (int k = 0; k < 6; ++k) acc[21 + k] += (double)e[k].im * r;
    acc[27] += r * r;
    acc[28] += 1.0;
}

__device__ __forceinline__ bool tsdf_loss_d(const HessArgs &a, const HessPoseD &P, int xq, int yq, int z, float gt, dcfloat &loss) {
    const dcfloat gt_tsdf(gt);
    const dcfloat vgx((float(xq) + 0.5f) * a.voxel_size);
    const dcfloat vgy((float(yq) + 0.5f) * a.voxel_size);
    const dcfloat vgz((float(z) + 0.5f) * a.voxel_size);
    dcfloat3 v_g; v_g.x = vgx; v_g.y = vgy; v_g.z = vgz;
    dcfloat3 v_c;
    v_c.x = dot(P.R.data[0], v_g) + P.t.x;
    v_c.y = dot(P.R.data[1], v_g) + P.t.y;
    v_c.z = dot(P.R.data[2], v_g) + P.t.z;
    const dcfloat inv_z = dcfloat(1.0f) / v_c.z;
    if (inv_z.value() < 0) return false;
    const dcfloat image_x = v_c.x * inv_z * a.intr.fx + a.intr.cx;
    const dcfloat image_y = v_c.y * inv_z * a.intr.fy + a.intr.cy;
    const int coo_x = __float2int_rd(image_x.value() - 0.5f), coo_y = __float2int_rd(image_y.value() - 0.5f);
    if (!(coo_x > 1 && coo_y > 1 && coo_x < a.dcols - 1 && coo_y < a.drows - 1)) return false;
    const int near_x = __float2int_rn(image_x.value()), near_y = __float2int_rn(image_y.value());
    dcfloat Dp(row_ptr(a.depth, a.dstep, near_y)[near_x]);
    const dcfloat d00(row_ptr(a.depth, a.dstep, coo_y)[coo_x]), d10(row_ptr(a.depth, a.dstep, coo_y)[coo_x + 1]);
    const dcfloat d01(row_ptr(a.depth, a.dstep, coo_y + 1)[coo_x]), d11(row_ptr(a.depth, a.dstep, coo_y + 1)[coo_x + 1]);
    if (d00.value() != 0.0f && d01.value() != 0.0f && d10.value() != 0.0f && d11.value() != 0.0f) {
        const dcfloat one(1.0f);
        const dcfloat fa = image_x - dcfloat(float(coo_x) + 0.5f);
        const dcfloat fb = image_y - dcfloat(float(coo_y) + 0.5f);
        Dp = d00 * (one - fa) * (one - fb) + d10 * fa * (one - fb) + d01 * (one - fa) * fb + d11 * fa * fb;
    }
    if (Dp.value() > 5 || Dp.value() < 0.2) return false;
    const dcfloat xl = (image_x - a.intr.cx) / a.intr.fx;
    const dcfloat yl = (image_y - a.intr.cy) / a.intr.fy;
    dcfloat3 v_c_1; v_c_1.x = Dp * xl; v_c_1.y = Dp * yl; v_c_1.z = Dp;
    const dcfloat distance = norm(v_c_1) - norm(v_c);
    const dcfloat gt_distance = gt_tsdf * a.tranc_dist;
    const dcfloat error = (distance - gt_distance) * a.tranc_dist_inv;
    if (fabsf(error.value()) > 1) return false;
    loss = error * error;
    return true;
}

__device__ __forceinline__ bool tsdf_loss_f(const HessArgs &a, const HessPoseF &P, int xq, int yq, int z, float gt, float &loss) {
    const float vgx = (float(xq) + 0.5f) * a.voxel_size, vgy = (float(yq) + 0.5f) * a.voxel_size, vgz = (float(z) + 0.5f) * a.voxel_size;
    const float vcx = (P.R[0] * vgx + P.R[1] * vgy + P.R[2] * vgz) + P.t[0];
    const float vcy = (P.R[3] * vgx + P.R[4] * vgy + P.R[5] * vgz) + P.t[1];
    const float vcz = (P.R[6] * vgx + P.R[7] * vgy + P.R[8] * vgz) + P.t[2];
    const float inv_z = 1.0f / vcz;
    if (inv_z < 0) return false;
    const float image_x = vcx * inv_z * a.intr.fx + a.intr.cx;
    const float image_y = vcy * inv_z * a.intr.fy + a.intr.cy;
    const int coo_x = __float2int_rd(image_x - 0.5f), coo_y = __float2int_rd(image_y - 0.5f);
    if (!(coo_x > 1 && coo_y > 1 && coo_x < a.dcols - 1 && coo_y < a.drows - 1)) return false;
    const int near_x = __float2int_rn(image_x), near_y = __float2int_rn(image_y);
    float Dp = row_ptr(a.depth, a.dstep, near_y)[near_x];
    const float d00 = row_ptr(a.depth, a.dstep, coo_y)[coo_x], d10 = row_ptr(a.depth, a.dstep, coo_y)[coo_x + 1];
    const float d01 = row_ptr(a.depth, a.dstep, coo_y + 1)[coo_x], d11 = row_ptr(a.depth, a.dstep, coo_y + 1)[coo_x + 1];
    if (d00 != 0.0f && d01 != 0.0f && d10 != 0.0f && d11 != 0.0f) {
        const float one = 1.0f;
        const float fa = image_x - (float(coo_x) + 0.5f), fb = image_y - (float(coo_y) + 0.5f);
        Dp = d00 * (one - fa) * (one - fb) + d10 * fa * (one - fb) + d01 * (one - fa) * fb + d11 * fa * fb;
    }
    if (Dp > 5 || Dp < 0.2) return false;
    const float xl = (image_x - a.intr.cx) / a.intr.fx, yl = (image_y - a.intr.cy) / a.intr.fy;
    const float v1x = Dp * xl, v1y = Dp * yl, v1z = Dp;
    const float distance = sqrtf(v1x * v1x + v1y * v1y + v1z * v1z) - sqrtf(vcx * vcx + vcy * vcy + vcz * vcz);
    const float gt_distance = gt * a.tranc_dist;
    const float error = (distance - gt_distance) * a.tranc_dist_inv;
    if (fabsf(error) > 1) return false;
    loss = error * error;
    return true;
}

int hess_tiling(HessArgs &a, const int *res, const float *gt, int z0, int z1, dim3 &grid, bool heavy_body);
```

### x-slam_amd/csrc/xs_residual.hip

```cpp
#include <string.h>
#include "xs_gn_band.h"
#include "xs_mailbox.h"
#include "xs_env.h"
#include "../../include/xslam_amd.h"

#ifndef XS_HESS_WAVES_PER_EU
#define XS_HESS_WAVES_PER_EU 3
#endif
#define XS_HESS_OCC __attribute__((amdgpu_waves_per_eu(XS_HESS_WAVES_PER_EU, XS_HESS_WAVES_PER_EU)))
__global__ void __launch_bounds__(256) XS_HESS_OCC k_tsdf_hessian(const HessArgs a, const HessPoseD Pk) {
    __shared__ HessPoseD P;
    {
        const float *src = reinterpret_cast<const float *>(&Pk);
        float *dst = reinterpret_cast<float *>(&P);
        for (int i = threadIdx.y * 64 + threadIdx.x; i < (int)(sizeof(HessPoseD) / sizeof(float)); i += 256) dst[i] = src[i];
    }
    __syncthreads();
    double acc[4] = {0.0, 0.0, 0.0, 0.0};
    walk_band(a, [&](int xq, int yq, int z, size_t index, float gt) {
        dcfloat loss;
        if (!tsdf_loss_d(a, P, xq, yq, z, gt, loss)) return;
        if (a.real_out) {
            a.real_out[index] = loss.value(); a.grad_out[index] = loss.grad();
            a.hess_out[index] = loss.hessian(); a.count_out[index] = 1;
        }
        acc[0] += loss.value(); acc[1] += loss.grad(); acc[2] += loss.hessian(); acc[3] += 1.0;
    });
    block_fold_and_finish<4>(acc, a.partials, a.ticket, a.out);
}

__global__ void __launch_bounds__(256) k_tsdf_loss(const HessArgs a, const HessPoseF P) {
    double acc[2] = {0.0, 0.0};
    walk_band(a, [&](int xq, int yq, int z, size_t index, float gt_tsdf) {
        float loss;
        if (!tsdf_loss_f(a, P, xq, yq, z, gt_tsdf, loss)) return;
        if (a.real_out) { a.real_out[index] = loss; a.count_out[index] = 1; }
        acc[0] += loss; acc[1] += 1.0;
    });
    block_fold_and_finish<2>(acc, a.partials, a.ticket, a.out);
}

#ifdef XS_GN_WAVES_PER_EU
#define XS_GN_OCC __attribute__((amdgpu_waves_per_eu(XS_GN_WAVES_PER_EU, XS_GN_WAVES_PER_EU)))
#else
#define XS_GN_OCC
#endif
template <bool POSTED>
__global__ void __launch_bounds__(256) XS_GN_OCC k_tsdf_gauss_newton(const HessArgs a, const GnPoses Pk) {
    __shared__ GnPoses P;
    bool left = false;
    if constexpr (POSTED) {
        __shared__ unsigned s_mail[xs::MAILBOX_WORDS];
        __shared__ unsigned s_cmd;
        if (threadIdx.y == 0) {
            const int lane = threadIdx.x;
            const unsigned long long t_resident = wall_clock64();
            const bool somebody_left = (__hip_atomic_load(a.ticket, __ATOMIC_RELAXED, __HIP_MEMORY_SCOPE_AGENT) >> 16) != 0;
            if (!somebody_left) xs::mailbox_wait(a.mailbox + 5 * xs::MAILBOX_WORDS, a.mailbox_seq, s_mail, lane);
            if (a.publish && blockIdx.x == 0 && lane == 0)
                __hip_atomic_store(&a.publish[30], (double)(wall_clock64() - t_resident), __ATOMIC_RELAXED, __HIP_MEMORY_SCOPE_SYSTEM);
            unsigned cmd = somebody_left ? 1u : (unsigned)__builtin_amdgcn_readfirstlane((int)s_mail[1]);
            float *dst = reinterpret_cast<float *>(&P);
            for (int k = 0; k < 6 && cmd == 0; ++k) {
                const unsigned w = __hip_atomic_load(a.mailbox + k * xs::MAILBOX_WORDS + (lane & 31), __ATOMIC_RELAXED, __HIP_MEMORY_SCOPE_SYSTEM);
                const unsigned s0 = __builtin_amdgcn_readlane(w, 0), s1 = __builtin_amdgcn_readlane(w, 8), s2 = __builtin_amdgcn_readlane(w, 16),
                               s3 = __builtin_amdgcn_readlane(w, 24);
                if (s0 != a.mailbox_seq || s1 != a.mailbox_seq || s2 != a.mailbox_seq || s3 != a.mailbox_seq) { cmd = 2; break; }
                const int f = xs::mailbox_float_of(lane & 31);
                if (lane < 32 && f >= 0) dst[f < 18 ? 18 * k + f : 108 + 6 * k + (f - 18)] = __uint_as_float(w);
            }
            if (lane == 0) s_cmd = cmd;
        }
        __syncthreads();
        left = s_cmd != 0;
    } else {
        const float *src = reinterpret_cast<const float *>(&Pk);
        float *dst = reinterpret_cast<float *>(&P);
        for (int i = threadIdx.y * 64 + threadIdx.x; i < (int)(sizeof(GnPoses) / sizeof(float)); i += 256) dst[i] = src[i];
        __syncthreads();
    }
    double acc[29];
#pragma unroll
    for (int k = 0; k < 29; ++k) acc[k] = 0.0;
    if (!left) walk_band(a, [&](int xq, int yq, int z, size_t, float gt) { gn_terms_add(a, P, xq, yq, z, gt, acc); });
    block_fold_and_finish<29>(acc, a.partials, a.ticket, a.out, a.publish, a.publish_seq, left);
}

enum { XS_TSDF_REDUCE_MAX_BLOCKS = XS_TSDF_REDUCE_MAX_BLOCKS_C };
extern "C" size_t xs_tsdf_reduce_workspace_bytes(void) { return (size_t)XS_TSDF_REDUCE_MAX_BLOCKS * 32 * sizeof(double) + 256; }
extern "C" int xs_tsdf_reduce_workspace_init(void *workspace, void *stream) {
    if (!workspace) return xs_set_error(hipErrorInvalidValue, "xs_tsdf_reduce_workspace_init: null pointer");
    XS_CHECK(hipMemsetAsync(workspace, 0, 256, (hipStream_t)stream));
    return 0;
}

static int hess_common(HessArgs &a, const float *depth_scaled, size_t scaled_step, int rows, int cols, const float *intr4, const int *res,
                       float voxel_size, float tranc_dist, const float *gt, int z0, int z1, void *workspace, double *out_dev, dim3 &grid,
                       void *stream, bool heavy_body) {
    if (!depth_scaled || !intr4 || !res || !gt || !workspace || !out_dev) return xs_set_error(hipErrorInvalidValue, "xs_tsdf_hessian/loss: null pointer");
    if (z0 < 0 || z1 > res[2] || z1 <= z0) return xs_set_error(hipErrorInvalidValue, "xs_tsdf_hessian/loss: bad slab");
    a.depth = depth_scaled; a.dstep = scaled_step; a.drows = rows; a.dcols = cols;
    a.voxel_size = voxel_size; a.tranc_dist = tranc_dist; a.tranc_dist_inv = 1.0f / tranc_dist;
    a.intr = Intr{intr4[0], intr4[1], intr4[2], intr4[3]};
    a.publish = nullptr; a.publish_seq = 0; a.mailbox = nullptr; a.mailbox_seq = 0;
    a.ticket = (unsigned *)workspace; a.partials = (double *)((char *)workspace + 256); a.out = out_dev;
    return hess_tiling(a, res, gt, z0, z1, grid, heavy_body);
}
int hess_tiling(HessArgs &a, const int *res, const float *gt, int z0, int z1, dim3 &grid, bool heavy_body) {
    a.X = res[0]; a.Y = res[1]; a.Z = res[2]; a.z0 = z0; a.z1 = z1;
    a.gt = gt;
    static const int env_blocks = exp_env_int("XS_HESS_BLOCKS", 0);
    static const bool env_narrow = exp_env_set("XS_HESS_NARROW");
    static const int env_ilg = exp_env_int("XS_HESS_IL", 1);
    a.il = (env_ilg == 2 || env_ilg == 4 || env_ilg == 8) ? env_ilg : 1;
    static const int env_il = exp_env_int("XS_HESS_INTERLEAVE", -1);
    const bool interleave = env_il < 0 ? heavy_body : env_il != 0;
    a.wide = (a.X % 4 == 0 && (reinterpret_cast<uintptr_t>(gt) % 16) == 0 && !env_narrow) ? (interleave ? 2 : 1) : 0;
    int gx = div_up(a.X, a.wide ? 256 : 64), gy = div_up(a.Y, 4), nz = z1 - z0, zsplit = 1;
    const long long cols_xy = (long long)gx * gy;
    const int cap = env_blocks > 0 && env_blocks <= XS_TSDF_REDUCE_MAX_BLOCKS ? env_blocks
                    : a.wide == 2 ? (int)XS_TSDF_REDUCE_MAX_BLOCKS
                    : a.wide ? (int)(cols_xy < 1024 ? 1024 : (cols_xy > XS_TSDF_REDUCE_MAX_BLOCKS ? XS_TSDF_REDUCE_MAX_BLOCKS : cols_xy))
                    : (int)(cols_xy < 1024 ? 1024 : (cols_xy > XS_TSDF_REDUCE_MAX_BLOCKS ? XS_TSDF_REDUCE_MAX_BLOCKS : cols_xy));
    if (a.wide == 2) {
        static const int env_zt = exp_env_int("XS_HESS_TILE_PLANES", 0);
        int G = nz >= 80 ? 5 : (nz >= 48 ? 3 : (nz >= 24 ? 2 : 1));
        if (env_zt >= 8) { G = 1; while (G * 2 * env_zt <= nz) G *= 2; }
        static const int env_g = exp_env_int("XS_HESS_GROUPS", 0);
        if (env_g >= 1 && env_g * 8 <= nz) G = env_g;
        a.tiles_x = gx; a.tiles_y = gy; a.tiles_z = G; a.zchunk = div_up(nz, G);
    } else {
        while ((long long)gx * gy * zsplit < cap && zsplit < nz && nz / (zsplit * 2) >= 16) zsplit *= 2;
        a.zchunk = div_up(nz, zsplit);
        a.tiles_x = gx; a.tiles_y = gy; a.tiles_z = div_up(nz, a.zchunk);
    }
    const long long ntiles = (long long)a.tiles_x * a.tiles_y * a.tiles_z;
    grid = dim3((unsigned)(ntiles < cap ? ntiles : cap));
    if ((long long)grid.x * grid.y * grid.z > XS_TSDF_REDUCE_MAX_BLOCKS) return xs_set_error(hipErrorInvalidValue, "xs_tsdf_hessian/loss: volume too large for the reduce workspace");
    return 0;
}

extern "C" int xs_compute_local_tsdf_hessian(const float *depth_scaled, size_t scaled_step, int rows, int cols, const float *intr4,
                                             const int *res, float voxel_size, const float *Rv2c36, const float *tv2c12,
                                             float tranc_dist, const float *gt, float *real_out, float *grad_out, float *hess_out,
                                             int *count_out, int z0, int z1, void *workspace, double *out4_dev, void *stream) {
    HessArgs a; dim3 grid;
    int rc = hess_common(a, depth_scaled, scaled_step, rows, cols, intr4, res, voxel_size, tranc_dist, gt, z0, z1, workspace, out4_dev, grid, stream, true);
    if (rc) return rc;
    if (!Rv2c36 || !tv2c12) return xs_set_error(hipErrorInvalidValue, "xs_compute_local_tsdf_hessian: null pose");
    const bool all = real_out && grad_out && hess_out && count_out, none = !real_out && !grad_out && !hess_out && !count_out;
    if (!all && !none) return xs_set_error(hipErrorInvalidValue, "xs_compute_local_tsdf_hessian: pass all four volumes or none");
    a.real_out = real_out; a.grad_out = grad_out; a.hess_out = hess_out; a.count_out = count_out;
    HessPoseD P;
    for (int r = 0; r < 3; ++r) {
        const float *p = Rv2c36 + r * 12;
        P.R.data[r].x = dcfloat(p[0], p[1], p[2], p[3]);
        P.R.data[r].y = dcfloat(p[4], p[5], p[6], p[7]);
        P.R.data[r].z = dcfloat(p[8], p[9], p[10], p[11]);
    }
    P.t.x = dcfloat(tv2c12[0], tv2c12[1], tv2c12[2], tv2c12[3]);
    P.t.y = dcfloat(tv2c12[4], tv2c12[5], tv2c12[6], tv2c12[7]);
    P.t.z = dcfloat(tv2c12[8], tv2c12[9], tv2c12[10], tv2c12[11]);
    hipLaunchKernelGGL(k_tsdf_hessian, grid, dim3(64, 4), 0, (hipStream_t)stream, a, P);
    XS_CHECK(hipGetLastError());
    return 0;
}

extern "C" int xs_compute_local_tsdf_loss(const float *depth_scaled, size_t scaled_step, int rows, int cols, const float *intr4,
                                          const int *res, float voxel_size, const float *Rv2c9, const float *tv2c3, float tranc_dist,
                                          const float *gt, float *real_out, int *count_out, int z0, int z1, void *workspace,
                                          double *out2_dev, void *stream) {
    HessArgs a; dim3 grid;
    int rc = hess_common(a, depth_scaled, scaled_step, rows, cols, intr4, res, voxel_size, tranc_dist, gt, z0, z1, workspace, out2_dev, grid, stream, false);
    if (rc) return rc;
    if (!Rv2c9 || !tv2c3) return xs_set_error(hipErrorInvalidValue, "xs_compute_local_tsdf_loss: null pose");
    if ((real_out == nullptr) != (count_out == nullptr)) return xs_set_error(hipErrorInvalidValue, "xs_compute_local_tsdf_loss: pass both volumes or none");
    a.real_out = real_out; a.grad_out = nullptr; a.hess_out = nullptr; a.count_out = count_out;
    HessPoseF P;
    for (int i = 0; i < 9; ++i) P.R[i] = Rv2c9[i];
    for (int i = 0; i < 3; ++i) P.t[i] = tv2c3[i];
    hipLaunchKernelGGL(k_tsdf_loss, grid, dim3(64, 4), 0, (hipStream_t)stream, a, P);
    XS_CHECK(hipGetLastError());
    return 0;
}

extern "C" int xs_tsdf_gauss_newton_terms(const float *depth_scaled, size_t scaled_step, int rows, int cols, const float *intr4, const int *res,
                                          float voxel_size, const float *Rv2c108, const float *tv2c36, float tranc_dist, const float *gt, int z0,
                                          int z1, void *workspace, double *out29_dev, void *stream) {
    return xs_tsdf_gauss_newton_terms_ex(depth_scaled, scaled_step, rows, cols, intr4, res, voxel_size, Rv2c108, tv2c36, tranc_dist, gt, z0, z1, workspace,
                                         out29_dev, nullptr, stream);
}
extern "C" int xs_tsdf_gauss_newton_terms_ex(const float *depth_scaled, size_t scaled_step, int rows, int cols, const float *intr4, const int *res,
                                             float voxel_size, const float *Rv2c108, const float *tv2c36, float tranc_dist, const float *gt, int z0,
                                             int z1, void *workspace, double *out29_dev, const xs_gn_opts *opts, void *stream) {
    if (opts && opts->struct_bytes != sizeof(xs_gn_opts)) return xs_set_error(hipErrorInvalidValue, "xs_tsdf_gauss_newton_terms_ex: opts->struct_bytes is not sizeof(xs_gn_opts)");
    HessArgs a; dim3 grid;
    int rc = hess_common(a, depth_scaled, scaled_step, rows, cols, intr4, res, voxel_size, tranc_dist, gt, z0, z1, workspace, out29_dev, grid, stream, true);
    if (rc) return rc;
    const bool posted = opts && opts->pose_mailbox && !Rv2c108 && !tv2c36;
    if (!posted && (!Rv2c108 || !tv2c36)) return xs_set_error(hipErrorInvalidValue, "xs_tsdf_gauss_newton_terms: give the six poses or a mailbox");
    a.real_out = nullptr; a.grad_out = nullptr; a.hess_out = nullptr; a.count_out = nullptr;
    if (opts) { a.publish = opts->publish_host; a.publish_seq = opts->publish_seq; }
    GnPoses P;
    memset(&P, 0, sizeof(P));
    if (posted) {
        a.mailbox = static_cast<const unsigned *>(opts->pose_mailbox); a.mailbox_seq = opts->mailbox_seq;
        hipLaunchKernelGGL(k_tsdf_gauss_newton<true>, grid, dim3(64, 4), 0, (hipStream_t)stream, a, P);
    } else {
        for (int k = 0; k < 6; ++k) { load_mat(Rv2c108 + 18 * k, P.R[k]); load_vec(tv2c36 + 6 * k, P.t[k]); }
        hipLaunchKernelGGL(k_tsdf_gauss_newton<false>, grid, dim3(64, 4), 0, (hipStream_t)stream, a, P);
    }
    XS_CHECK(hipGetLastError());
    return 0;
}
extern "C" size_t xs_gn_publish_bytes(void) { return 33 * sizeof(double); }
extern "C" size_t xs_gn_mailbox_bytes(void) { return 6 * xs::MAILBOX_WORDS * sizeof(unsigned); }
extern "C" void xs_gn_post_poses(void *mailbox_host, const float *Rv2c108, const float *tv2c36, unsigned mailbox_seq, int cmd) {
    alignas(64) unsigned img[6][xs::MAILBOX_WORDS];
    for (int k = 0; k < 6; ++k) mailbox_image(img[k], Rv2c108 ? Rv2c108 + 18 * k : nullptr, tv2c36 ? tv2c36 + 6 * k : nullptr, mailbox_seq, cmd);
    mailbox_post(mailbox_host, img, 6);
}
__global__ void k_publish_sums(const double *sums, int n, double *publish, unsigned long long seq) {
    const int tid = threadIdx.x;
    if (tid < n) __hip_atomic_store(&publish[tid], sums[tid], __ATOMIC_RELAXED, __HIP_MEMORY_SCOPE_SYSTEM);
    __builtin_amdgcn_fence(__ATOMIC_RELEASE, "");
    if (tid == 0) __hip_atomic_store(reinterpret_cast<unsigned long long *>(publish) + 32, seq, __ATOMIC_RELAXED, __HIP_MEMORY_SCOPE_SYSTEM);
}
extern "C" int xs_gn_publish_sums(const double *sums_dev, int n, double *publish_host, unsigned long long seq, void *stream) {
    if (!sums_dev || !publish_host || n < 1 || n > 32) return xs_set_error(hipErrorInvalidValue, "xs_gn_publish_sums: bad argument");
    hipLaunchKernelGGL(k_publish_sums, dim3(1), dim3(64), 0, (hipStream_t)stream, sums_dev, n, publish_host, seq);
    XS_CHECK(hipGetLastError());
    return 0;
}
// ... 1 lines not shown
```

### x-slam_amd/host/KinectFusionReconstruction.cpp

```cpp
#include "kf_internal.hpp"
#include <cmath>

using namespace xs_host;

KinectFusionReconstruction::KinectFusionReconstruction() {
    depth_width = 0;
    depth_height = 0;
    hipSafeCall(hipStreamCreateWithFlags(&aux_stream_, hipStreamNonBlocking));
    hipSafeCall(hipEventCreateWithFlags(&surface_done_, hipEventDisableTiming));
    hipSafeCall(hipEventCreateWithFlags(&integrate_done_, hipEventDisableTiming));
    hipSafeCall(hipEventCreateWithFlags(&scale_done_, hipEventDisableTiming));
    hipSafeCall(hipEventCreateWithFlags(&tail_done_, hipEventDisableTiming));
    hipSafeCall(hipEventCreateWithFlags(&surface_done_next_, hipEventDisableTiming));
    hipSafeCall(hipEventCreateWithFlags(&scale_done_next_, hipEventDisableTiming));
    hipSafeCall(hipHostMalloc((void **)&pinned_counters_, COUNTER_RING * 2 * sizeof(unsigned long long)));
    hipSafeCall(hipHostMalloc((void **)&pinned_sums_, PINNED_DOUBLES * sizeof(double), hipHostMallocCoherent | hipHostMallocMapped));
    for (int i = 0; i < PINNED_DOUBLES; ++i) pinned_sums_[i] = 0.0;
    hipSafeCall(hipHostMalloc((void **)&pinned_pairs_, XS_ICP_PAIRS_BYTES, hipHostMallocCoherent | hipHostMallocMapped));
    std::memset(pinned_pairs_, 0, XS_ICP_PAIRS_BYTES);
    hipSafeCall(hipHostMalloc((void **)&pinned_records_, xs_icp_records_bytes(), hipHostMallocCoherent | hipHostMallocMapped));
    std::memset(pinned_records_, 0, xs_icp_records_bytes());
}

void KinectFusionReconstruction::SetSharding(int rank, int count, collective_fn fn, void *user) {
    shard_rank = rank; shard_count = count < 1 ? 1 : count; collective = fn; collective_user = user;
}

KinectFusionReconstruction::~KinectFusionReconstruction() {
    if (aux_stream_) { (void)hipStreamSynchronize(aux_stream_); (void)hipStreamDestroy(aux_stream_); }
    if (surface_done_) (void)hipEventDestroy(surface_done_);
    if (integrate_done_) (void)hipEventDestroy(integrate_done_);
    if (tail_done_) (void)hipEventDestroy(tail_done_);
    if (surface_done_next_) (void)hipEventDestroy(surface_done_next_);
    if (scale_done_next_) (void)hipEventDestroy(scale_done_next_);
    if (scale_done_) (void)hipEventDestroy(scale_done_);
    if (pinned_counters_) (void)hipHostFree(pinned_counters_);
    if (gather_counts_host_) (void)hipHostFree(gather_counts_host_);
    if (pinned_sums_) (void)hipHostFree(pinned_sums_);
    if (pinned_pairs_) (void)hipHostFree(pinned_pairs_);
    if (pinned_records_) (void)hipHostFree(pinned_records_);
    if (icp_mailbox_) (void)xs_icp_mailbox_free(icp_mailbox_, icp_mailbox_in_device_);
    if (reloc_.gn_mailbox) (void)xs_icp_mailbox_free(reloc_.gn_mailbox, reloc_.gn_mailbox_in_device);
    if (reloc_.gn_publish) (void)hipHostFree(reloc_.gn_publish);
    for (int i = 0; i < 2; ++i) {
        if (ingest_pinned_[i]) { (void)hipEventSynchronize(ingest_done_[i]); (void)hipHostFree(ingest_pinned_[i]); (void)hipEventDestroy(ingest_done_[i]); }
    }
    if (tsdf_volume_d_ptr) ReleaseBuffers();
    for (auto &slot : prof_ring_)
        for (int s = 0; s < ST_COUNT; ++s) { (void)hipEventDestroy(slot.ev[s][0]); (void)hipEventDestroy(slot.ev[s][1]); }
}

void KinectFusionReconstruction::SetYamlParameters(const FlatYaml &config_) {
    for (const char *key : {"integrate_post_pose", "integrate_post_early", "integrate_classify_beside_icp", "integrate_classify_predicted"})
        if (config_.as<bool>(key, false)) throw std::runtime_error(std::string("retired YAML key (code removed): ") + key);
    if (config_.as<int>("integrate_classify_early", 0) != 0) throw std::runtime_error("retired YAML key (code removed): integrate_classify_early");
    this->config = config_;
    const int resolutionX = config.as<int>("tsdf_size_x");
    const int resolutionY = config.as<int>("tsdf_size_y");
    const int resolutionZ = config.as<int>("tsdf_size_z");
    volume_resolution = Vector3i(resolutionX, resolutionY, resolutionZ);
    voxel_size = config.as<float>("tsdf_voxel_size");
    max_integration_weight = config.as<int>("max_integration_weight");
    const float thres_range = config.as<float>("thres_range");

    csfd_seed_row = config.as<int>("csfd_seed_row", -1);
    csfd_seed_col = config.as<int>("csfd_seed_col", -1);
    csfd_seed_h = config.as<float>("csfd_seed_h", (float)H_);

    world2camera = Matrix4cf::Identity();
    if (csfd_seed_row >= 0 && csfd_seed_row < 4 && csfd_seed_col >= 0 && csfd_seed_col < 4)
        world2camera(csfd_seed_row, csfd_seed_col).imag(csfd_seed_h);
    world2camera_record.clear();
    world2camera_record.reserve(10000);
    world2camera_record.push_back(world2camera);
    world2volume = Matrix4cf::Identity();
    const float init_x = config.as<float>("init_x"), init_y = config.as<float>("init_y"), init_z = config.as<float>("init_z");
    const float r_x = config.as<float>("r_x") / 180.0f * float(M_PI);
    const float r_y = config.as<float>("r_y") / 180.0f * float(M_PI);
    const float r_z = config.as<float>("r_z") / 180.0f * float(M_PI);
    const Matrix3cf rotation = (angle_axis(hostComplex(r_x, 0.f), 0) * angle_axis(hostComplex(r_y, 0.f), 1)) * angle_axis(hostComplex(r_z, 0.f), 2);
    for (int i = 0; i < 3; ++i) for (int j = 0; j < 3; ++j) world2volume(i, j) = hostComplex(rotation(i, j).real(), 0.f);
    world2volume(0, 3) = hostComplex(init_x, 0.f);
    world2volume(1, 3) = hostComplex(init_y, 0.f);
    world2volume(2, 3) = hostComplex(init_z, 0.f);

    depth_width = config.as<int>("depth_width");
    depth_height = config.as<int>("depth_height");
    kinect_intrinsic.fx = config.as<float>("fx");
    kinect_intrinsic.fy = config.as<float>("fy");
    kinect_intrinsic.cx = config.as<float>("cx");
    kinect_intrinsic.cy = config.as<float>("cy");

    num_levels = config.as<int>("num_levels");
    if (num_levels > 3) {
        std::cout << "sorry, the max supported multi-level = 3" << "\n";
        num_levels = 3;
    }
    const int iters[] = {5, 4, 3};
    std::copy(iters, iters + num_levels, icp_iterations);

    distThres = config.as<float>("distThres");
    angleThres = float(sin(config.as<float>("angleThres") / 180.f * M_PI));

    biInterpolate_threshold = config.as<float>("biInterpolate_threshold");
    trunc_logistic_k = config.as<float>("trunc_logistic_k", 0.f);

    zo0 = (int)((long long)resolutionZ * shard_rank / shard_count);
    zo1 = (int)((long long)resolutionZ * (shard_rank + 1) / shard_count);
    zs0 = shard_count > 1 ? std::max(0, zo0 - HALO) : 0;
    zs1 = shard_count > 1 ? std::min(resolutionZ, zo1 + HALO) : resolutionZ;
    icp_solve_on_device = config.as<bool>("icp_solve_on_device", false);
    icp_shard_rows = config.as<bool>("icp_shard_rows", false);
    icp_post_pose = config.as<bool>("icp_post_pose", true);
    icp_real_current_maps = config.as<bool>("icp_real_current_maps", true);
    integrate_classify_ahead = config.as<bool>("integrate_classify_ahead", true);
    integrate_classify_slack = std::max(1.0f, config.as<float>("integrate_classify_slack", 2.0f));
    raycast_sign_map = config.as<bool>("raycast_sign_map", true);
    raycast_sign_map_shift = std::min(6, std::max(0, config.as<int>("raycast_sign_map_shift", 0)));
    icp_lookahead = config.as<int>("icp_lookahead", 1);
    icp_host_fold = config.as<bool>("icp_host_fold", false);
    icp_publish_pairs = config.as<bool>("icp_publish_pairs", true);
    force_shard_composite = config.as<bool>("force_shard_composite", false);
    shard_composite_gather = config.as<bool>("shard_composite_gather", true);
    raycast_builds_pyramid = config.as<bool>("raycast_builds_pyramid", true);
    gn_post_pose = config.as<bool>("gn_post_pose", true);
    gn_publish_sharded = config.as<bool>("gn_publish_sharded", true);
    profile_integrate_every = std::max(1, config.as<int>("profile_integrate_every", 4));
    AllocateBuffers();
    tsdf_volume_d_ptr = new TsdfVolume(Vector3i(resolutionX, resolutionY, zs1 - zs0), voxel_size, thres_range);
    invalidate_derived_maps();
    if (sign_map_on()) {
        const int finest = xs_raycast_signmap_shift(&kinect_intrinsic.fx, voxel_size, tsdf_volume_d_ptr->getTsdfTruncDist());
        raycast_sign_map_shift = finest ? std::max(raycast_sign_map_shift, finest) : 0;
        const size_t bytes = raycast_sign_map_shift ? xs_signmap_bytes(res3(), raycast_sign_map_shift) : 0;
        if (bytes) { sign_map_.create(bytes); RebuildSignMap(); }
        else raycast_sign_map = false;
    }

    use_gtPose = config.as<bool>("flag_use_gtPose", false);
    gt_poses.resize(0);
    frame_id = 0;
    frame_step = config.as<int>("frame_step", 1);
}

void KinectFusionReconstruction::AllocateBuffers() {
    depths_curr_d.resize(num_levels);
    vmaps_curr_d.resize(num_levels);
    nmaps_curr_d.resize(num_levels);
    vmaps_g_prev_d.resize(num_levels);
    nmaps_g_prev_d.resize(num_levels);
    for (int i = 0; i < num_levels; ++i) {
        const int pyr_rows = depth_height >> i, pyr_cols = depth_width >> i;
        depths_curr_d[i].create(pyr_rows, pyr_cols);
        vmaps_curr_d[i].create(pyr_rows * 3, pyr_cols);
        nmaps_curr_d[i].create(pyr_rows * 3, pyr_cols);
        if (i == 0) {
            const size_t step = ((size_t)pyr_cols * sizeof(devComplex) + 255) / 256 * 256;
            maps_prev0_block_.create(2 * (size_t)pyr_rows * 3 * step);
            vmaps_g_prev_d[0] = MapArr(pyr_rows * 3, pyr_cols, maps_prev0_block_.ptr(), step);
            nmaps_g_prev_d[0] = MapArr(pyr_rows * 3, pyr_cols, maps_prev0_block_.ptr() + (size_t)pyr_rows * 3 * step, step);
        } else {
            vmaps_g_prev_d[i].create(pyr_rows * 3, pyr_cols);
            nmaps_g_prev_d[i].create(pyr_rows * 3, pyr_cols);
        }
    }
    depthRawScaled_d.create(depth_height, depth_width);
    xs_const_div_prepare(voxel_size);
    {
        integrate_ws_.create(xs_integrate_workspace_bytes(res3(), zs1 - zs0));
        icp_ws_.create(xs_icp_workspace_bytes());
        check_rc(xs_icp_workspace_init(icp_ws_.ptr(), current_stream()), "icp workspace");
        if (!icp_mailbox_) check_rc(xs_icp_mailbox_alloc(&icp_mailbox_, &icp_mailbox_in_device_), "icp mailbox");
        icp_sums_.create(64);
        icp_pose_.create(xs_icp_pose_state_bytes());
        ray_ws_.create((size_t)depth_width * depth_height);
        if (shard_count > 1 || force_shard_composite) {
            ray_keys_.create((size_t)depth_width * depth_height);
            ray_min_keys_.create((size_t)depth_width * depth_height);
        }
    }
    counters_.create(2 * COUNTER_RING);
    hipSafeCall(hipMemsetAsync(counters_.ptr(), 0, 2 * COUNTER_RING * sizeof(unsigned long long), current_stream()));
    depth_max_.create(4);
    depth_tiles_.create(xs_depth_tiles_bytes(depth_height, depth_width));
}

void KinectFusionReconstruction::ReleaseBuffers() {
    for (int i = 0; i < (int)depths_curr_d.size(); ++i) {
        depths_curr_d[i].release();
        vmaps_curr_d[i].release();
        nmaps_curr_d[i].release();
        vmaps_g_prev_d[i].release();
        nmaps_g_prev_d[i].release();
    }
    maps_prev0_block_.release();
    g_buf.release();
    sum_buf.release();
    depthRawScaled_d.release();
    for (auto &m : vreal_curr_d) m.release();
    for (auto &m : nreal_curr_d) m.release();
    real_maps_valid_ = false;
    delete tsdf_volume_d_ptr;
    tsdf_volume_d_ptr = nullptr;
    invalidate_derived_maps();
}

int KinectFusionReconstruction::SmoothDepthFrame(MapArr &dst_d, const DeviceArray2D<ushort> &src_d) {
    if (src_d.rows() <= 0 || src_d.cols() <= 0) {
        std::cout << "error: KinectFusionReconstruction::SmoothDepthFrame, input map is empty" << std::endl;
        return 0;
    }
    if (dst_d.rows() != src_d.rows() || dst_d.cols() != src_d.cols()) {
        dst_d.release();
        dst_d.create(src_d.rows(), src_d.cols());
    }
    bilateralFilter(src_d, dst_d);
    return 1;
}

int KinectFusionReconstruction::ProcessFrame(const DeviceArray2D<ushort> &depth_frame_d) {
    const int align_return = AlignDepthToReconstruction(depth_frame_d, false);
    if (frame_id > 0 && !align_return) {
        std::cout << "Frame align failed!" << std::endl;
        return 0;
    }
    IntegrateFrame(depth_frame_d);
    frame_id += frame_step;
    if (profiling) end_profiled_frame();
    return 1;
}

ushort *KinectFusionReconstruction::IngestBuffer() {
    const int slot = ingest_seq_ & 1;
    const size_t bytes = (size_t)depth_width * depth_height * sizeof(ushort);
    if (!ingest_pinned_[slot]) {
        hipSafeCall(hipHostMalloc((void **)&ingest_pinned_[slot], bytes));
        hipSafeCall(hipEventCreateWithFlags(&ingest_done_[slot], hipEventDisableTiming));
    } else
        hipSafeCall(hipEventSynchronize(ingest_done_[slot]));
    return ingest_pinned_[slot];
}
int KinectFusionReconstruction::ProcessFrameHost(const ushort *depth_host) {
    if (depth_width <= 0 || depth_height <= 0 || !depth_host) return 0;
    const size_t row = (size_t)depth_width * sizeof(ushort);
    const ushort *src = depth_host;
    int slot = -1;
    if (depth_host == ingest_pinned_[0] || depth_host == ingest_pinned_[1]) slot = depth_host == ingest_pinned_[0] ? 0 : 1;
    else {
        hipPointerAttribute_t attr;
        const bool pinned = hipPointerGetAttributes(&attr, depth_host) == hipSuccess && attr.type == hipMemoryTypeHost;
        if (!pinned) {
            (void)hipGetLastError();
            ushort *stage = IngestBuffer();
            slot = ingest_seq_ & 1;
            std::memcpy(stage, depth_host, row * depth_height);
            src = stage;
        }
    }
    depth_ingest_d_.create(depth_height, depth_width);
    hipSafeCall(hipMemcpy2DAsync(depth_ingest_d_.ptr(), depth_ingest_d_.step(), src, row, row, depth_height, hipMemcpyHostToDevice, aux_stream_));
    if (slot >= 0) {
        hipSafeCall(hipEventRecord(ingest_done_[slot], aux_stream_));
        if (slot == (ingest_seq_ & 1)) ++ingest_seq_;
    }
    return ProcessFrame(depth_ingest_d_);
}

int KinectFusionReconstruction::AlignDepthToReconstruction(const DeviceArray2D<ushort> &depth_frame_d, bool ) {
    SurfaceMeasure(depth_frame_d);
    struct AtExit { KinectFusionReconstruction *k; ~AtExit() { k->EnqueueAnnouncedFrame(true); } } announced_at_exit{this};
    if (use_gtPose) return 1;
    Matrix4cf c2w_prev = inverse(world2camera_record.back());
    Matrix3frm Rprev = GetRotation(c2w_prev);
    Vector3cf tprev = GetTranslation(c2w_prev);
    Matrix3frm Rprev_inv = inverse(Rprev);
    Matrix3frm Rcurr = Rprev;
    Vector3cf tcurr = tprev;
    return PoseEstimate(Rcurr, tcurr, Rprev_inv, tprev);
}
// ... 729 lines not shown
```

### x-slam_amd/host/KinectFusionReconstruction.h

```cpp
#pragma once
#include "TsdfVolume.h"
#include "flat_yaml.hpp"
#include "../csrc/xs_host_wait.h"
#include <chrono>
#include <string>
#include <vector>

class KinectFusionReconstruction {
public:
    typedef xs_host::Matrix3cf Matrix3frm;
    typedef xs_host::Matrix4cf Matrix4cf;
    typedef xs_host::Vector3cf Vector3cf;
    enum Stage { ST_SURFACE = 0, ST_ICP, ST_SCALE, ST_INTEGRATE, ST_RAYCAST, ST_RESIZE, ST_COUNT };

    xs_host::FlatYaml config;
    int num_levels = 3;
    Matrix4cf world2camera;
    Matrix4cf world2volume;
    std::vector<Matrix4cf> world2camera_record;
    int frame_id = 0;
    int frame_step = 1;
    std::vector<Matrix4cf> gt_poses{};

    Intr kinect_intrinsic;
    int depth_width = 0, depth_height = 0;

    Vector3i volume_resolution;
    float voxel_size{};
    TsdfVolume *tsdf_volume_d_ptr = nullptr;
    int max_integration_weight = 0;

    int icp_iterations[3]{};
    float distThres{};
    float angleThres{};
    DeviceArray2D<devComplexICP> g_buf;
    DeviceArray<devComplexICP> sum_buf;

    float trunc_logistic_k = 0.f;
    float biInterpolate_threshold{0.005f};

    std::vector<DeviceArray2D<devComplex>> depths_curr_d, vmaps_curr_d, nmaps_curr_d, vmaps_g_prev_d, nmaps_g_prev_d;
    DeviceArray2D<float> depthRawScaled_d;
    std::vector<DeviceArray2D<float>> vreal_curr_d, nreal_curr_d;
    bool icp_real_current_maps = true;
    bool integrate_classify_ahead = true;
    long long list_cover_counts_[4] = {0, 0, 0, 0};
    long long composite_bytes_ = 0;
    float integrate_classify_slack = 2.0f;
    bool raycast_sign_map = true;
    int raycast_sign_map_shift = 0;
    void RebuildSignMap();
    void MarkSignMapStale() { sign_map_stale_ = true; }
    bool sign_map_stale_ = false;
    void HintNextFrame(const ushort *depth_dev, size_t step_bytes) {
        if (next_stage_ != 0) EnqueueAnnouncedFrame(true);
        next_hint_ptr_ = depth_dev; next_hint_step_ = step_bytes;
    }
    void EnqueueAnnouncedFrame(bool all);
    int next_stage_ = 0;
    void EnqueueMapsFromPyramid();
    void EnqueueScale(const DeviceArray2D<ushort> &depth_frame_d);
    void SwapMapSets();
    bool list_ready_ = false;
    float list_Rv2c_[18]{}, list_tv2c_[6]{};
    void ClassifyAhead(const Matrix3frm &Rcurr, const Vector3cf &tcurr);
    bool real_maps_valid_ = false;

    bool use_gtPose = false;

    int csfd_seed_row = -1, csfd_seed_col = -1;
    float csfd_seed_h = 1e-7f;

    typedef void (*collective_fn)(void *user, int op, void *dev_ptr, long count);
    enum { HALO = 6 };
    int shard_rank = 0, shard_count = 1;
    int zo0 = 0, zo1 = 0, zs0 = 0, zs1 = 0;
    collective_fn collective = nullptr;
    void *collective_user = nullptr;
    void SetSharding(int rank, int count, collective_fn fn, void *user);

    bool icp_solve_on_device = false;
    bool icp_post_pose = true;
    int icp_lookahead = 1;
    bool icp_host_fold = false;
    bool icp_publish_pairs = true;
    bool icp_shard_rows = false;
    bool force_shard_composite = false;

    bool profiling = false;
    double stage_ms[ST_COUNT] = {0, 0, 0, 0, 0, 0};
    long long stage_calls[ST_COUNT] = {0, 0, 0, 0, 0, 0};
    std::vector<double> icp_log;
    long long cum_updated = 0, cum_hits = 0;

    KinectFusionReconstruction();
    ~KinectFusionReconstruction();

    int getFrame() const { return frame_id; }
    int getVolumeSize() const { return volume_resolution[0] * volume_resolution[1] * volume_resolution[2]; }
    const int *res3() const { return volume_resolution.v; }
    Matrix4cf getCamera2Volume() { return world2volume * xs_host::inverse(world2camera); }

    void AllocateBuffers();
    void ReleaseBuffers();
    void SetYamlParameters(const xs_host::FlatYaml &config_);
    int ProcessFrame(const DeviceArray2D<ushort> &depth_frame_d);
    int ProcessFrameHost(const ushort *depth_host);
    ushort *IngestBuffer();
    void SurfaceMeasure(const DeviceArray2D<ushort> &depth_frame_d);
    int PoseEstimate(Matrix3frm Rcurr, Vector3cf tcurr, Matrix3frm Rprev_inv, Vector3cf tprev);
    int AlignDepthToReconstruction(const DeviceArray2D<ushort> &depth_frame_d, bool use_LM = false);
    int IntegrateFrame(const DeviceArray2D<ushort> &depth_frame_d);
    static int SmoothDepthFrame(MapArr &dst_d, const DeviceArray2D<ushort> &src_d);
    int CalculatePointCloud(MapArr &xyz_g_d, MapArr &normal_g_d);
    void ModelMapPyramid();

    static inline Vector3cf GetTranslation(Matrix4cf &trans_mat) { return xs_host::GetTranslation(trans_mat); }
    static inline Matrix3frm GetRotation(Matrix4cf &trans_mat) { return xs_host::GetRotation(trans_mat); }

    int GaussNewtonTerms(const DeviceArray2D<ushort> &depth_frame_d, const Matrix4cf &camera2volume, double out29[29]);
    int RelocalizeGaussNewton(const DeviceArray2D<ushort> &depth_frame_d, Matrix4cf &camera2volume, int iterations, float damping,
                              std::vector<double> *loss_history = nullptr);
    bool gn_post_pose = true;
    bool gn_publish_sharded = true;
    double gn_pass_us = 0, gn_kernel_ms = 0;
    long long gn_passes = 0, gn_kernel_calls = 0;
    double gn_poll_us = 0;
    long long gn_poll_passes = 0;
    const float *GaussNewtonPrepare(const DeviceArray2D<ushort> &depth_frame_d);
    void GaussNewtonEnqueue(const DeviceArray2D<ushort> &depth_frame_d, const float *gt, const float (*R)[18], const float (*t)[6], unsigned mail_seq,
                            unsigned long long seq);
    bool GaussNewtonWait(unsigned long long seq, double out29[29]);
    void GaussNewtonCollectEvents();
    int RelocalizeGaussNewtonBatch(const std::vector<DeviceArray2D<ushort>> &depths, Matrix4cf *camera2volume, int iterations, float damping,
                                   int *ok, std::vector<double> *loss_history = nullptr);
    int PoseHessianTerms(const DeviceArray2D<ushort> &depth_frame_d, const Matrix4cf &camera2volume, double out29[29]);
    int RelocalizeNewtonBatch(const std::vector<DeviceArray2D<ushort>> &depths, Matrix4cf *camera2volume, int iterations, float damping, int *ok,
                              std::vector<double> *loss_history = nullptr, int *fallbacks = nullptr);
    int ScorePoses(const DeviceArray2D<ushort> &depth_frame_d, const Matrix4cf *camera2volume, int P, double *out2xP);
    int RelocalizeGlobal(const DeviceArray2D<ushort> &depth_frame_d, const Matrix4cf *candidates, int P, int keep, int iterations, float damping,
                         Matrix4cf &best, double report[8]);
    int ScoreViews(const Matrix4cf *camera2volume, int P, const xs_view_opts *opts, int min_weight, unsigned *out4xP);
    int NextBestView(const Matrix4cf *camera2volume, int P, const xs_view_opts *opts, int min_weight, unsigned min_hits, unsigned *out4xP);
    int ClearanceField(int max_radius_vox, int unknown_blocks, int min_weight, unsigned short *host_out);
    int Reachable(const Matrix4cf *start, float radius_m, int snap_vox, int unknown_blocks, int min_weight, int P, const Matrix4cf *camera2volume,
                  unsigned char *reachable, unsigned short *clear2);
    int NextReachableView(const Matrix4cf *camera2volume, int P, const xs_view_opts *opts, int min_weight, unsigned min_hits, unsigned *out4xP,
                          float radius_m, int snap_vox, int unknown_blocks, unsigned char *reachable);
    int Travel(const Matrix4cf *start, float radius_m, int snap_vox, int unknown_blocks, int min_weight, float max_travel_m, int P,
               const Matrix4cf *camera2volume, unsigned char *reachable, unsigned short *clear2, unsigned short *travel3);
    int PathTo(const Matrix4cf *start, float radius_m, int snap_vox, int unknown_blocks, int min_weight, float max_travel_m, const Matrix4cf &target,
               int capacity, int *voxels3, float *points3, int *needed_out);
    int NextViewByTravel(const Matrix4cf *camera2volume, int P, const xs_view_opts *opts, int min_weight, unsigned min_hits, unsigned *out4xP,
                         float radius_m, int snap_vox, int unknown_blocks, float max_travel_m, float bias_m, unsigned short *travel3_out);
    int Frontiers(int cell, unsigned long long min_size, int min_weight, int capacity, unsigned long long *records8, int *count_out);
    int ProposeViews(float radius_m, int start_snap_vox, int unknown_blocks, int min_weight, int cell, unsigned long long min_size, int views_per_cluster,
                     float standoff_m, int snap_vox, int capacity, Matrix4cf *c2v_out, int *cluster_out, int *count_out);
    long long RelocalizationIndexVoxels() const { return reloc_.band_key.generation >= 0 ? reloc_.band.count : 0; }
    long long volume_generation = 0;

    struct CPointCloud {
        std::vector<float> positions, normals;
        size_t size() const { return positions.size() / 3; }
        bool exportPly(const std::string &filename) const;
    };
    CPointCloud ExportPointCloud(int max_buffer);
    struct CMesh {
        std::vector<float> positions, normals, vertex_im;
        std::vector<unsigned long long> edge_keys;
        std::vector<int> triangles;
        bool has_im = false;
        size_t vertices() const { return edge_keys.size(); }
        size_t faces() const { return triangles.size() / 3; }
        bool exportPly(const std::string &filename) const;
    };
    CMesh ExportMesh(int min_weight = 1);

    void saveTSDFVolume(const std::string &tsdf_filename);
    void saveCheckpoint(const std::string &filename);
    bool loadCheckpoint(const std::string &filename);

    long long lastUpdatedVoxels();
    long long lastRaycastHits();
    long long last_frame_counter(int which);
    void synchronize();

private:
    enum { COUNTER_RING = 512 };
    DeviceArray<unsigned long long> counters_;
    long long counter_frame_ = 0;
    unsigned long long *frame_counters() { return counters_.ptr() + 2 * (size_t)(counter_frame_ % COUNTER_RING); }
    unsigned long long *hits_counter_ = nullptr;
    DeviceArray<float> depth_max_;
    DeviceArray<unsigned char> integrate_ws_;
    DeviceArray<unsigned char> icp_ws_;
    DeviceArray<double> icp_sums_;
    DeviceArray<unsigned char> icp_pose_;
    struct BandKey { long long generation = -1; bool operator==(const BandKey &o) const { return generation == o.generation; } };
    struct GridKey { long long generation = -1; int min_weight = 0; bool operator==(const GridKey &o) const { return generation == o.generation && min_weight == o.min_weight; } };
    struct ClearKey { GridKey grid; int R = 0, unknown = -1; bool operator==(const ClearKey &o) const { return grid == o.grid && R == o.R && unknown == o.unknown; } };
    struct ReachKey {
        ClearKey field; int r2 = 0, seed[3] = {-1, -1, -1};
        bool operator==(const ReachKey &o) const { return field == o.field && r2 == o.r2 && seed[0] == o.seed[0] && seed[1] == o.seed[1] && seed[2] == o.seed[2]; }
    };
    struct TravelKey { ReachKey reach; int limit = -1; bool operator==(const TravelKey &o) const { return reach == o.reach && limit == o.limit; } };
    struct FrontierKey { GridKey grid; int cell = -1; bool operator==(const FrontierKey &o) const { return grid == o.grid && cell == o.cell; } };
    struct Reloc {
        DeviceArray<double> gn_sums;
        double *gn_publish = nullptr;
        void *gn_mailbox = nullptr;
        int gn_mailbox_in_device = 0;
        unsigned long long gn_seq = 0;
        unsigned gn_mail_seq = 0;
        std::vector<std::pair<hipEvent_t, hipEvent_t>> gn_events;
        DeviceArray<float> gn_dense;
        DeviceArray<unsigned char> gn_ws;
        xs_band_index band = {};
        BandKey band_key;
        DeviceArray<unsigned long long> band_keys;
        DeviceArray<float> band_values;
        DeviceArray<long long> band_segs;
        DeviceArray<unsigned char> band_ws;
        DeviceArray<double> band_sums;
        std::vector<DeviceArray2D<float>> band_depth;
        DeviceArray<unsigned char> newton_ws;
        DeviceArray<double> newton_sums;
        DeviceArray<unsigned char> score_ws;
        DeviceArray<double> score_sums;
        DeviceArray2D<float> score_depth;
    } reloc_;
    const float *GaussNewtonDenseView();
    void BandIndexPrepare();
    size_t BandBatchPrepare(const std::vector<DeviceArray2D<ushort>> &depths);
    void GaussNewtonBandLaunch(const int *frames, int n, const Matrix4cf *camera2volume, size_t scaled_step, int rows, int cols, double *raw);
    void PoseHessianLaunch(const int *frames, int n, const Matrix4cf *camera2volume, size_t scaled_step, int rows, int cols, double *raw);
    void ensure_reduce_workspace(DeviceArray<unsigned char> &ws, size_t bytes, const char *what);
    void fetch_sums(double *device_sums, size_t count, double *host_sums);
    struct Planning {
        DeviceArray<unsigned char> view_grid;
        DeviceArray<unsigned> view_counts;
        GridKey grid_key;
        DeviceArray<unsigned char> clear_field;
        DeviceArray<unsigned char> clear_ws;
        ClearKey clear_key;
        DeviceArray<unsigned char> reach;
        DeviceArray<unsigned char> reach_io;
        ReachKey reach_key;
        DeviceArray<unsigned char> travel;
        DeviceArray<unsigned char> travel_ws;
        DeviceArray<unsigned char> travel_io;
        DeviceArray<unsigned char> path_io;
        TravelKey travel_key;
        DeviceArray<unsigned char> frontier_mask;
        DeviceArray<unsigned char> frontier_labels;
        DeviceArray<unsigned char> frontier_ws;
        DeviceArray<unsigned long long> frontier_records_d;
        std::vector<unsigned long long> frontier_records;
        FrontierKey frontier_key;
    } plan_;
    bool ViewGridPrepare(int min_weight);
    bool ClearancePrepare(int R, int unknown_blocks, int min_weight);
    int ReachQuery(const float *points3xN, int n, int over_passable, int snap, unsigned char *reachable, unsigned short *clear2, int *voxel);
    int ReachPrepare(const Matrix4cf *start, float radius_m, int snap_vox, int unknown_blocks, int min_weight);
    bool TravelPrepare(int limit);
    bool FrontierPrepare(int cell, int min_weight);
    void reach_forget() { plan_.reach_key = ReachKey{}; plan_.travel_key = TravelKey{}; }
    void invalidate_derived_maps() { reloc_.band_key = BandKey{}; plan_.grid_key = GridKey{}; plan_.clear_key = ClearKey{}; plan_.frontier_key = FrontierKey{}; reach_forget(); }
    DeviceArray2D<ushort> depth_ingest_d_;
    ushort *ingest_pinned_[2] = {nullptr, nullptr};
    hipEvent_t ingest_done_[2] = {nullptr, nullptr};
    int ingest_seq_ = 0;
    DeviceArray<unsigned char> maps_prev0_block_;
    DeviceArray<float> ray_ws_;
    hipEvent_t tail_done_ = nullptr;
    bool tail_recorded_ = false;
    std::vector<MapArr> depths_next_d, vmaps_next_d, nmaps_next_d;
    std::vector<DeviceArray2D<float>> vreal_next_d, nreal_next_d;
    DeviceArray2D<float> depthRawScaled_next_d;
    DeviceArray<float> depth_max_next_;
    bool raycast_builds_pyramid = true;
    int profile_integrate_every = 4;
    bool IntegrateKernelTimedThisFrame() const;
    bool pyramid_in_raycast_ = false;
    bool PreparePyramidLevels();
    bool shard_composite_gather = true;
    DeviceArray<unsigned char> gather_buf_, pack_buf_;
    DeviceArray<int> gather_counts_;
    int *gather_counts_host_ = nullptr;
    DeviceArray<unsigned char> depth_tiles_, depth_tiles_next_;
    hipEvent_t surface_done_next_ = nullptr, scale_done_next_ = nullptr;
    bool real_maps_valid_next_ = false, scale_recorded_next_ = false;
    const void *next_hint_ptr_ = nullptr, *next_ready_ptr_ = nullptr;
    size_t next_hint_step_ = 0, next_ready_step_ = 0;
    bool next_ready_ = false;
    DeviceArray<unsigned char> sign_map_;
    bool sign_map_on() const { return raycast_sign_map; }
    unsigned char *sign_map_ptr() { return sign_map_on() ? sign_map_.ptr() : nullptr; }
    DeviceArray<int> ray_keys_, ray_min_keys_;
    enum { ICP_LOG_MAX = 62, PINNED_DOUBLES = 128 + 64 * ICP_LOG_MAX };
    double *pinned_sums_ = nullptr;
    unsigned long long *pinned_pairs_ = nullptr;
    bool integrate_split() const;
    void flush_pending_fold(hipStream_t st);
    bool integrate_header_clear_ = false;
    unsigned long long *pending_fold_ = nullptr;
    double *pinned_records_ = nullptr;
    void *icp_mailbox_ = nullptr;
    long long counters_prepared_for_ = -1;
    unsigned long long *PrepareFrameCounters(hipStream_t st);
    int icp_mailbox_in_device_ = 0;
    unsigned long long icp_seq_ = 0;
public:
    double icp_level_us[4] = {0, 0, 0, 0};
    long long icp_level_calls[4] = {0, 0, 0, 0};
    double tail_host_us[4] = {0, 0, 0, 0};
    long long tail_host_calls = 0;
    std::chrono::steady_clock::time_point t_last_sums_{};
    void DebugSetIcpSequence(unsigned long long v);
    int debug_fail_icp_iteration_ = -1;
    int debug_post_delay_us_[2] = {0, 0};
    unsigned debug_post_rng_ = 12345u;
private:
    void AbandonClassifiedList();
    hipStream_t aux_stream_ = nullptr;
    hipEvent_t surface_done_ = nullptr, integrate_done_ = nullptr, scale_done_ = nullptr;
    hipEvent_t integrate_done_now_ = nullptr;
    bool integrate_recorded_ = false, scale_recorded_ = false;
    bool profiling_icp_sync = false;
    int PoseEstimateOnDevice(Matrix3frm Rcurr, Vector3cf tcurr, const Matrix3frm &Rprev_inv, const Vector3cf &tprev, Matrix4cf c2w_curr,
                             int total_iters);
    enum class IcpSink { records, pairs, word };
    xs_wait_result wait_icp_sums(IcpSink sink, unsigned long long seq, int level);
    void icp_normal_equations(const MatS33 &Rcurr, const devComplex3 &tcurr, const MatS33 &Rprev_inv, const devComplex3 &tprev, int level,
                              hostComplexICP *A, hostComplexICP *b, long long *inliers);
    enum { PROF_RING = COUNTER_RING / 2 };
    struct ProfSlot { hipEvent_t ev[ST_COUNT][2]; bool used[ST_COUNT]; };
    std::vector<ProfSlot> prof_ring_;
    int prof_pending_ = 0;
    unsigned long long *pinned_counters_ = nullptr;
    void stage_begin(int st);
    void stage_end(int st);
    void end_profiled_frame();
public:
    void collect_stage_times();
    void set_profiling(int level);
    bool profiling_stages = false;
private:
};
```

### x-slam_amd/host/gn_host.hpp

```cpp
#pragma once
#include "host_algebra.hpp"
#include <algorithm>
#include <vector>

namespace xs_host {

constexpr double GN_H = 1e-7;

inline void gn_seeded_poses(const Matrix4cf &camera2volume, float R[6][18], float t[6][6]) {
    const Matrix4cf v2c = inverse(camera2volume);
    const hostComplex ih(0.f, (float)GN_H);
    for (int k = 0; k < 6; ++k) {
        hostComplex Rk[3][3], tk[3];
        for (int i = 0; i < 3; ++i) { for (int j = 0; j < 3; ++j) Rk[i][j] = v2c.m[i][j]; tk[i] = v2c.m[i][3]; }
        if (k < 3) {
            for (int i = 0; i < 3; ++i) tk[i].imag(tk[i].imag() - (ih * v2c.m[i][k]).imag());
        } else {
            const int a = k - 3, b = (a + 1) % 3, c = (a + 2) % 3;
            for (int i = 0; i < 3; ++i) {
                Rk[i][b].imag(Rk[i][b].imag() - (ih * v2c.m[i][c]).imag());
                Rk[i][c].imag(Rk[i][c].imag() + (ih * v2c.m[i][b]).imag());
            }
        }
        for (int i = 0; i < 3; ++i) {
            for (int j = 0; j < 3; ++j) { R[k][(i * 3 + j) * 2] = Rk[i][j].real(); R[k][(i * 3 + j) * 2 + 1] = Rk[i][j].imag(); }
            t[k][2 * i] = tk[i].real(); t[k][2 * i + 1] = tk[i].imag();
        }
    }
}
inline void gn_scale_sums(const double *raw, double out29[29]) {
    const double ih = 1.0 / (double)(float)GN_H;
    for (int i = 0; i < 21; ++i) out29[i] = raw[i] * ih * ih;
    for (int i = 21; i < 27; ++i) out29[i] = raw[i] * ih;
    out29[27] = raw[27]; out29[28] = raw[28];
}

inline bool damped_spd6_step(const double s[29], double damping, Matrix4cf &camera2volume) {
    if (s[28] < 6) return false;
    double A[36], b[6], x[6];
    int q = 0;
    for (int j = 0; j < 6; ++j)
        for (int k = j; k < 6; ++k, ++q) { A[j * 6 + k] = s[q]; A[k * 6 + j] = s[q]; }
    for (int k = 0; k < 6; ++k) { A[k * 6 + k] *= 1.0 + damping; b[k] = -s[21 + k]; }
    if (!solve_spd6(A, b, x)) return false;
    hostComplex xi[6];
    for (int k = 0; k < 6; ++k) xi[k] = hostComplex((float)x[k], 0.f);
    camera2volume = se3Exp(xi) * camera2volume;
    return true;
}

inline int gn_loop_step(const double s[29], int p, int iterations, float damping, xs_host::Matrix4cf &camera2volume, std::vector<double> *loss_history) {
    if (loss_history) loss_history->push_back(s[28] > 0 ? s[27] / s[28] : 0.0);
    if (p == iterations) return 1;
    return damped_spd6_step(s, (double)damping, camera2volume) ? 0 : -1;
}

template <class Evaluate, class Step>
int gn_batch_loop(int F, int iterations, std::vector<double> *loss_history, int *ok, int chunk, Evaluate &&evaluate, Step &&step) {
    for (int f = 0; f < F; ++f) ok[f] = 0;
    const int passes = iterations + (loss_history ? 1 : 0);
    if (passes <= 0) { for (int f = 0; f < F; ++f) ok[f] = 1; return F; }
    std::vector<int> active((size_t)F);
    for (int f = 0; f < F; ++f) active[(size_t)f] = f;
    std::vector<double> sums((size_t)chunk * 29);
    for (int p = 0; p < passes && !active.empty(); ++p) {
        std::vector<int> next;
        for (size_t c0 = 0; c0 < active.size(); c0 += (size_t)chunk) {
            const int n = (int)std::min(active.size() - c0, (size_t)chunk);
            evaluate(&active[c0], n, sums.data());
            for (int i = 0; i < n; ++i) {
                const int f = active[c0 + (size_t)i];
                const double *s = &sums[(size_t)i * 29];
                if (loss_history) loss_history[f].push_back(s[28] > 0 ? s[27] / s[28] : 0.0);
                if (p == iterations) { ok[f] = 1; continue; }
                if (s[28] < 6 || !step(f, s, p)) continue;
                if (p + 1 == passes) ok[f] = 1;
                else next.push_back(f);
            }
        }
        active.swap(next);
    }
    return (int)std::count(ok, ok + F, 1);
}

}
```

### x-slam_amd/host/kf_relocalize.cpp

```cpp
#include "kf_internal.hpp"
#include "newton_host.hpp"
#include "score_host.hpp"

using namespace xs_host;
static_assert(GN_H == H_, "gn_host.hpp restates the seed step of xs_types.hpp");

void KinectFusionReconstruction::ensure_reduce_workspace(DeviceArray<unsigned char> &ws, size_t bytes, const char *what) {
    if (ws.size() >= bytes) return;
    ws.create(bytes);
    check_rc(xs_tsdf_reduce_workspace_init(ws.ptr(), current_stream()), what);
}
void KinectFusionReconstruction::fetch_sums(double *device_sums, size_t count, double *host_sums) {
    hipStream_t st = current_stream();
    if (shard_count > 1 && collective) collective(collective_user, 0, device_sums, (long)count);
    hipSafeCall(hipMemcpyAsync(host_sums, device_sums, count * sizeof(double), hipMemcpyDeviceToHost, st));
    hipSafeCall(hipStreamSynchronize(st));
}

const float *KinectFusionReconstruction::GaussNewtonPrepare(const DeviceArray2D<ushort> &depth_frame_d) {
    hipStream_t st = current_stream();
    depthRawScaled_d.create(depth_frame_d.rows(), depth_frame_d.cols());
    check_rc(xs_scale_depth(depth_frame_d.ptr(), depth_frame_d.step(), depth_frame_d.rows(), depth_frame_d.cols(), depthRawScaled_d.ptr(),
                            depthRawScaled_d.step(), st), "scaleDepth");
    if (reloc_.gn_sums.size() < 32) reloc_.gn_sums.create(32);
    ensure_reduce_workspace(reloc_.gn_ws, xs_tsdf_reduce_workspace_bytes(), "reduce workspace");
    if (!reloc_.gn_publish) {
        hipSafeCall(hipHostMalloc((void **)&reloc_.gn_publish, xs_gn_publish_bytes(), hipHostMallocCoherent | hipHostMallocMapped));
        std::memset(reloc_.gn_publish, 0, xs_gn_publish_bytes());
    }
    if (!reloc_.gn_mailbox && gn_post_pose) check_rc(xs_icp_mailbox_alloc(&reloc_.gn_mailbox, &reloc_.gn_mailbox_in_device), "Gauss-Newton mailbox");
    return GaussNewtonDenseView();
}
const float *KinectFusionReconstruction::GaussNewtonDenseView() {
    hipStream_t st = current_stream();
    DeviceArray2D<float> value = tsdf_volume_d_ptr->value();
    const size_t row_bytes = (size_t)volume_resolution[0] * sizeof(float), plane_rows = (size_t)volume_resolution[1];
    const float *gt = reinterpret_cast<const float *>(reinterpret_cast<const char *>(value.ptr()) + (size_t)(zo0 - zs0) * plane_rows * value.step());
    if (value.step() != row_bytes) {
        const size_t rows = (size_t)(zo1 - zo0) * plane_rows;
        if (reloc_.gn_dense.size() < rows * volume_resolution[0]) reloc_.gn_dense.create(rows * volume_resolution[0]);
        hipSafeCall(hipMemcpy2DAsync(reloc_.gn_dense.ptr(), row_bytes, gt, value.step(), row_bytes, rows, hipMemcpyDeviceToDevice, st));
        gt = reloc_.gn_dense.ptr();
    }
    return gt;
}
void KinectFusionReconstruction::GaussNewtonEnqueue(const DeviceArray2D<ushort> &depth_frame_d, const float *gt, const float (*R)[18], const float (*t)[6],
                                                    unsigned mail_seq, unsigned long long seq) {
    hipStream_t st = current_stream();
    const bool sharded = shard_count > 1 && collective;
    xs_gn_opts o = {};
    o.struct_bytes = sizeof(o);
    o.pose_mailbox = R ? nullptr : reloc_.gn_mailbox; o.mailbox_seq = mail_seq;
    if (!sharded) { o.publish_host = reloc_.gn_publish; o.publish_seq = seq; }
    hipEvent_t e0 = nullptr, e1 = nullptr;
    if (profiling && reloc_.gn_events.size() < 64) {
        hipSafeCall(hipEventCreate(&e0)); hipSafeCall(hipEventCreate(&e1));
        reloc_.gn_events.push_back({e0, e1});
        hipSafeCall(hipEventRecord(e0, st));
    }
    check_rc(xs_tsdf_gauss_newton_terms_ex(depthRawScaled_d.ptr(), depthRawScaled_d.step(), depth_frame_d.rows(), depth_frame_d.cols(), &kinect_intrinsic.fx,
                                           res3(), voxel_size, R ? &R[0][0] : nullptr, t ? &t[0][0] : nullptr, tsdf_volume_d_ptr->getTsdfTruncDist(), gt, zo0,
                                           zo1, reloc_.gn_ws.ptr(), reloc_.gn_sums.ptr(), &o, st), "GaussNewtonTerms");
    if (e1) hipSafeCall(hipEventRecord(e1, st));
    if (sharded && gn_publish_sharded) {
        collective(collective_user, 0, reloc_.gn_sums.ptr(), 29);
        check_rc(xs_gn_publish_sums(reloc_.gn_sums.ptr(), 29, reloc_.gn_publish, seq, st), "GaussNewtonTerms");
    } else if (sharded) {
        fetch_sums(reloc_.gn_sums.ptr(), 29, reloc_.gn_publish);
        reinterpret_cast<volatile unsigned long long *>(reloc_.gn_publish)[32] = seq;
    }
}
bool KinectFusionReconstruction::GaussNewtonWait(unsigned long long seq, double out29[29]) {
    const xs_wait_result w = xs_host_wait([&] { return xs_poll_word(reloc_.gn_publish + 32, seq); }, kWaitPolls, current_stream());
    if (w.status == xs_wait::left) return false;
    if (w.status != xs_wait::published) wait_fatal("Gauss-Newton pass", w);
    gn_scale_sums(reloc_.gn_publish, out29);
    return true;
}
void KinectFusionReconstruction::GaussNewtonCollectEvents() {
    for (auto &e : reloc_.gn_events) {
        float ms = 0.f;
        if (hipEventSynchronize(e.second) == hipSuccess && hipEventElapsedTime(&ms, e.first, e.second) == hipSuccess) { gn_kernel_ms += ms; ++gn_kernel_calls; }
        (void)hipEventDestroy(e.first); (void)hipEventDestroy(e.second);
    }
    reloc_.gn_events.clear();
}

int KinectFusionReconstruction::GaussNewtonTerms(const DeviceArray2D<ushort> &depth_frame_d, const Matrix4cf &camera2volume, double out29[29]) {
    if (!tsdf_volume_d_ptr) return 0;
    const float *gt = GaussNewtonPrepare(depth_frame_d);
    float R[6][18], t[6][6];
    gn_seeded_poses(camera2volume, R, t);
    const unsigned long long seq = ++reloc_.gn_seq;
    GaussNewtonEnqueue(depth_frame_d, gt, R, t, 0u, seq);
    const bool ok = GaussNewtonWait(seq, out29);
    GaussNewtonCollectEvents();
    return ok ? 1 : 0;
}

int KinectFusionReconstruction::RelocalizeGaussNewton(const DeviceArray2D<ushort> &depth_frame_d, Matrix4cf &camera2volume, int iterations,
                                                      float damping, std::vector<double> *loss_history) {
    if (!tsdf_volume_d_ptr) return 0;
    const int passes = iterations + (loss_history ? 1 : 0);
    if (passes <= 0) return 1;
    const float *gt = GaussNewtonPrepare(depth_frame_d);
    const bool ahead = gn_post_pose && shard_count == 1 && reloc_.gn_mailbox && reloc_.gn_mailbox_in_device;
    float R[6][18], t[6][6];
    gn_seeded_poses(camera2volume, R, t);
    unsigned long long seq = ++reloc_.gn_seq;
    GaussNewtonEnqueue(depth_frame_d, gt, R, t, 0u, seq);
    int rc = 1;
    const auto t_begin = std::chrono::steady_clock::now();
    int done = 0;
    for (int p = 0; p < passes; ++p) {
        unsigned long long next_seq = 0;
        unsigned next_mail = 0;
        if (ahead && p + 1 < passes) {
            next_seq = ++reloc_.gn_seq; next_mail = ++reloc_.gn_mail_seq;
            if (next_mail == 0) next_mail = ++reloc_.gn_mail_seq;
            GaussNewtonEnqueue(depth_frame_d, gt, nullptr, nullptr, next_mail, next_seq);
        }
        auto leave = [&](int code) {
            if (next_seq) {
                xs_gn_post_poses(reloc_.gn_mailbox, nullptr, nullptr, next_mail, 1);
                double ignore[29];
                (void)GaussNewtonWait(next_seq, ignore);
            }
            rc = code;
        };
        double s[29];
        if (!GaussNewtonWait(seq, s)) { leave(0); break; }
        ++done;
        if (p > 0 && ahead) { gn_poll_us += reloc_.gn_publish[30] * 0.01; ++gn_poll_passes; }
        const int step = gn_loop_step(s, p, iterations, damping, camera2volume, loss_history);
        if (step > 0) break;
        if (step < 0) { leave(0); break; }
        if (p + 1 < passes) {
            gn_seeded_poses(camera2volume, R, t);
            if (next_seq) { xs_gn_post_poses(reloc_.gn_mailbox, &R[0][0], &t[0][0], next_mail, 0); seq = next_seq; }
            else { seq = ++reloc_.gn_seq; GaussNewtonEnqueue(depth_frame_d, gt, R, t, 0u, seq); }
        }
    }
    gn_pass_us += std::chrono::duration<double, std::micro>(std::chrono::steady_clock::now() - t_begin).count();
    gn_passes += done;
    GaussNewtonCollectEvents();
    return rc;
}

void KinectFusionReconstruction::BandIndexPrepare() {
    if (reloc_.band_key == BandKey{volume_generation} && reloc_.band.nblocks > 0) return;
    hipStream_t st = current_stream();
    const int *res = res3();
    const float *gt = GaussNewtonDenseView();
    const size_t segs_bytes = xs_tsdf_band_segs_bytes(res, zo0, zo1);
    if (segs_bytes == 0) { std::cout << "error::KinectFusionReconstruction, relocalisation index: bad slab" << std::endl; exit(-1); }
    if (reloc_.band_segs.size() < segs_bytes / sizeof(long long)) reloc_.band_segs.create(segs_bytes / sizeof(long long));
    for (int attempt = 0;; ++attempt) {
        reloc_.band.keys = reloc_.band_keys.ptr(); reloc_.band.values = reloc_.band_values.ptr(); reloc_.band.segs = reloc_.band_segs.ptr();
        reloc_.band.capacity = (long long)std::min(reloc_.band_keys.size(), reloc_.band_values.size());
        const int rc = xs_tsdf_band_build(gt, res, zo0, zo1, &reloc_.band, st);
        if (rc == 0) break;
        if (rc != XS_BAND_OVER_CAPACITY || attempt > 0) check_rc(rc, "relocalisation index");
        reloc_.band_keys.create((size_t)reloc_.band.count);
        reloc_.band_values.create((size_t)reloc_.band.count);
    }
    reloc_.band_key = BandKey{volume_generation};
}

size_t KinectFusionReconstruction::BandBatchPrepare(const std::vector<DeviceArray2D<ushort>> &depths) {
    const int F = (int)depths.size();
    hipStream_t st = current_stream();
    BandIndexPrepare();
    ensure_reduce_workspace(reloc_.band_ws, xs_tsdf_band_workspace_bytes(XS_BAND_MAX_FRAMES), "band workspace");
    if (reloc_.band_sums.size() < (size_t)XS_BAND_MAX_FRAMES * 29) reloc_.band_sums.create((size_t)XS_BAND_MAX_FRAMES * 29);
    if ((int)reloc_.band_depth.size() < F) reloc_.band_depth.resize((size_t)F);
    const int rows = depths[0].rows(), cols = depths[0].cols();
    for (int f = 0; f < F; ++f) {
        reloc_.band_depth[(size_t)f].create(rows, cols);
        check_rc(xs_scale_depth(depths[(size_t)f].ptr(), depths[(size_t)f].step(), rows, cols, reloc_.band_depth[(size_t)f].ptr(), reloc_.band_depth[(size_t)f].step(), st),
                 "scaleDepth");
    }
    const size_t scaled_step = reloc_.band_depth[0].step();
    for (int f = 1; f < F; ++f)
        if (reloc_.band_depth[(size_t)f].step() != scaled_step) { std::cout << "error::KinectFusionReconstruction, batch: depth steps differ" << std::endl; exit(-1); }
    return scaled_step;
}

void KinectFusionReconstruction::GaussNewtonBandLaunch(const int *frames, int n, const Matrix4cf *camera2volume, size_t scaled_step, int rows, int cols, double *raw) {
    std::vector<float> R((size_t)n * 108), t((size_t)n * 36);
    std::vector<const float *> dptr((size_t)n);
    for (int i = 0; i < n; ++i) {
        gn_seeded_poses(camera2volume[frames[i]], reinterpret_cast<float (*)[18]>(&R[(size_t)i * 108]), reinterpret_cast<float (*)[6]>(&t[(size_t)i * 36]));
        dptr[(size_t)i] = reloc_.band_depth[(size_t)frames[i]].ptr();
    }
    check_rc(xs_tsdf_gauss_newton_terms_band(n, dptr.data(), scaled_step, rows, cols, &kinect_intrinsic.fx, voxel_size, R.data(), t.data(),
                                             tsdf_volume_d_ptr->getTsdfTruncDist(), &reloc_.band, reloc_.band_ws.ptr(), reloc_.band_sums.ptr(), current_stream()),
             "GaussNewtonTermsBand");
    fetch_sums(reloc_.band_sums.ptr(), (size_t)n * 29, raw);
}

int KinectFusionReconstruction::RelocalizeGaussNewtonBatch(const std::vector<DeviceArray2D<ushort>> &depths, Matrix4cf *camera2volume, int iterations,
                                                           float damping, int *ok, std::vector<double> *loss_history) {
    const int F = (int)depths.size();
    if (!tsdf_volume_d_ptr) { std::fill(ok, ok + F, 0); return 0; }
    const size_t scaled_step = F > 0 && iterations + (loss_history ? 1 : 0) > 0 ? BandBatchPrepare(depths) : 0;
    return gn_batch_loop(F, iterations, loss_history, ok, XS_BAND_MAX_FRAMES,
        [&](const int *frames, int n, double *sums) {
            GaussNewtonBandLaunch(frames, n, camera2volume, scaled_step, depths[0].rows(), depths[0].cols(), sums);
            for (int i = 0; i < n; ++i) gn_scale_sums(sums + 29 * i, sums + 29 * i);
        },
        [&](int f, const double *s, int) { return damped_spd6_step(s, (double)damping, camera2volume[f]); });
}

void KinectFusionReconstruction::PoseHessianLaunch(const int *frames, int n, const Matrix4cf *camera2volume, size_t scaled_step, int rows, int cols, double *raw) {
    ensure_reduce_workspace(reloc_.newton_ws, xs_tsdf_pose_hessian_workspace_bytes(XS_BAND_MAX_FRAMES), "pose Hessian workspace");
    if (reloc_.newton_sums.size() < (size_t)XS_BAND_MAX_FRAMES * 29) reloc_.newton_sums.create((size_t)XS_BAND_MAX_FRAMES * 29);
    std::vector<float> R((size_t)n * 21 * 36), t((size_t)n * 21 * 12);
    std::vector<const float *> dptr((size_t)n);
    for (int i = 0; i < n; ++i) {
        newton_seeded_poses(camera2volume[frames[i]], reinterpret_cast<float (*)[36]>(&R[(size_t)i * 21 * 36]), reinterpret_cast<float (*)[12]>(&t[(size_t)i * 21 * 12]));
        dptr[(size_t)i] = reloc_.band_depth[(size_t)frames[i]].ptr();
    }
    check_rc(xs_tsdf_pose_hessian_band(n, dptr.data(), scaled_step, rows, cols, &kinect_intrinsic.fx, voxel_size, R.data(), t.data(),
                                       tsdf_volume_d_ptr->getTsdfTruncDist(), &reloc_.band, reloc_.newton_ws.ptr(), reloc_.newton_sums.ptr(), current_stream()),
             "PoseHessianBand");
    fetch_sums(reloc_.newton_sums.ptr(), (size_t)n * 29, raw);
}

int KinectFusionReconstruction::PoseHessianTerms(const DeviceArray2D<ushort> &depth_frame_d, const Matrix4cf &camera2volume, double out29[29]) {
    if (!tsdf_volume_d_ptr) return 0;
    const std::vector<DeviceArray2D<ushort>> depths(1, depth_frame_d);
    const size_t scaled_step = BandBatchPrepare(depths);
    const int frame = 0;
    PoseHessianLaunch(&frame, 1, &camera2volume, scaled_step, depth_frame_d.rows(), depth_frame_d.cols(), out29);
    newton_scale_sums(out29, out29);
    return 1;
}

int KinectFusionReconstruction::RelocalizeNewtonBatch(const std::vector<DeviceArray2D<ushort>> &depths, Matrix4cf *camera2volume, int iterations,
                                                      float damping, int *ok, std::vector<double> *loss_history, int *fallbacks) {
    const int F = (int)depths.size();
    if (fallbacks) std::fill(fallbacks, fallbacks + F, 0);
    if (!tsdf_volume_d_ptr) { std::fill(ok, ok + F, 0); return 0; }
    const size_t scaled_step = F > 0 && iterations + (loss_history ? 1 : 0) > 0 ? BandBatchPrepare(depths) : 0;
    return gn_batch_loop(F, iterations, loss_history, ok, XS_BAND_MAX_FRAMES,
        [&](const int *frames, int n, double *sums) {
            PoseHessianLaunch(frames, n, camera2volume, scaled_step, depths[0].rows(), depths[0].cols(), sums);
            for (int i = 0; i < n; ++i) newton_scale_sums(sums + 29 * i, sums + 29 * i);
        },
        [&](int f, const double *s, int) {
            if (newton_step(s, (double)damping, camera2volume[f])) return true;
            double gn[29];
            GaussNewtonBandLaunch(&f, 1, camera2volume, scaled_step, depths[0].rows(), depths[0].cols(), gn);
            gn_scale_sums(gn, gn);
            if (fallbacks) ++fallbacks[f];
            return damped_spd6_step(gn, (double)damping, camera2volume[f]);
        });
}

int KinectFusionReconstruction::ScorePoses(const DeviceArray2D<ushort> &depth_frame_d, const Matrix4cf *camera2volume, int P, double *out2xP) {
    if (!tsdf_volume_d_ptr || P < 0) return 0;
    if (P == 0) return 1;
    hipStream_t st = current_stream();
    BandIndexPrepare();
    ensure_reduce_workspace(reloc_.score_ws, xs_tsdf_score_poses_workspace_bytes(XS_SCORE_MAX_POSES), "score workspace");
    if (reloc_.score_sums.size() < (size_t)XS_SCORE_MAX_POSES * 2) reloc_.score_sums.create((size_t)XS_SCORE_MAX_POSES * 2);
    const int rows = depth_frame_d.rows(), cols = depth_frame_d.cols();
    reloc_.score_depth.create(rows, cols);
    check_rc(xs_scale_depth(depth_frame_d.ptr(), depth_frame_d.step(), rows, cols, reloc_.score_depth.ptr(), reloc_.score_depth.step(), st), "scaleDepth");
    std::vector<float> R((size_t)std::min(P, (int)XS_SCORE_MAX_POSES) * 9), t(R.size() / 3);
    for (int p0 = 0; p0 < P; p0 += XS_SCORE_MAX_POSES) {
        const int n = std::min(P - p0, (int)XS_SCORE_MAX_POSES);
        for (int i = 0; i < n; ++i) pack_real_pose(inverse(camera2volume[p0 + i]), &R[(size_t)i * 9], &t[(size_t)i * 3]);
        check_rc(xs_tsdf_score_poses_band(n, reloc_.score_depth.ptr(), reloc_.score_depth.step(), rows, cols, &kinect_intrinsic.fx, voxel_size, R.data(), t.data(),
                                          tsdf_volume_d_ptr->getTsdfTruncDist(), &reloc_.band, reloc_.score_ws.ptr(), reloc_.score_sums.ptr(), st), "ScorePosesBand");
        fetch_sums(reloc_.score_sums.ptr(), (size_t)n * 2, out2xP + 2 * (size_t)p0);
    }
    return 1;
}

int KinectFusionReconstruction::RelocalizeGlobal(const DeviceArray2D<ushort> &depth_frame_d, const Matrix4cf *candidates, int P, int keep, int iterations,
                                                 float damping, Matrix4cf &best, double report[8]) {
    for (int i = 0; i < 8; ++i) report[i] = 0.0;
    report[0] = -1.0;
    if (!tsdf_volume_d_ptr || P <= 0 || keep <= 0) return 0;
    std::vector<double> before((size_t)P * 2);
    if (!ScorePoses(depth_frame_d, candidates, P, before.data())) return 0;
    report[6] = (double)reloc_.band.count;
    const std::vector<int> top = score_top_k(before.data(), P, keep);
    const int K = (int)top.size();
    std::vector<Matrix4cf> refined((size_t)K);
    for (int k = 0; k < K; ++k) refined[(size_t)k] = candidates[top[(size_t)k]];
    const std::vector<DeviceArray2D<ushort>> depths((size_t)K, depth_frame_d);
    std::vector<int> ok((size_t)K, 0);
    report[5] = (double)RelocalizeGaussNewtonBatch(depths, refined.data(), iterations, damping, ok.data(), nullptr);
    std::vector<double> after((size_t)K * 2);
    ScorePoses(depth_frame_d, refined.data(), K, after.data());
    const int w = score_winner(after.data(), ok.data(), K);
    if (w < 0) return 0;
    best = refined[(size_t)w];
    report[0] = (double)top[(size_t)w];
    report[1] = score_S(&before[2 * (size_t)top[(size_t)w]]);
    report[2] = score_S(&after[2 * (size_t)w]);
// ... 5 lines not shown
```

Baseline: 4113.

## Route Gauss-Newton relocalisation loop through sparse band index with mailbox poses

Lets the per-pass Gauss-Newton relocalisation loop use the sparse truncation-band index instead of scanning the dense TSDF slab. The band is built once the expected pass count justifies it, or reused when still valid. The band kernel gains mailbox and argument pose modes and a host-sorted block order that schedules the longest segments first. The cost is a host-synchronised index build on first use and more kernel variants, while the integrate path the metric measures is untouched.

New measurement: 4101 (median of 2 runs). No clear change (-0.3%).

```diff
diff --git a/include/xslam_amd.h b/include/xslam_amd.h
--- a/include/xslam_amd.h
+++ b/include/xslam_amd.h
@@ -176,6 +176,9 @@
 int xs_tsdf_gauss_newton_terms_band(int frames, const float *const *depth_scaled, size_t scaled_step, int rows, int cols, const float *intr4,
                                     float voxel_size, const float *Rv2c108xF, const float *tv2c36xF, float tranc_dist, const xs_band_index *index,
                                     void *workspace, double *out29xF_dev, void *stream);
+int xs_tsdf_gauss_newton_terms_band_ex(int frames, const float *const *depth_scaled, size_t scaled_step, int rows, int cols, const float *intr4,
+                                       float voxel_size, const float *Rv2c108xF, const float *tv2c36xF, float tranc_dist, const xs_band_index *index,
+                                       void *workspace, double *out29xF_dev, const xs_gn_opts *opts, void *stream);
 size_t xs_tsdf_pose_hessian_workspace_bytes(int frames);
 int xs_tsdf_pose_hessian_band(int frames, const float *const *depth_scaled, size_t scaled_step, int rows, int cols, const float *intr4,
                               float voxel_size, const float *Rv2c36x21xF, const float *tv2c12x21xF, float tranc_dist, const xs_band_index *index,
diff --git a/x-slam_amd/capi.py b/x-slam_amd/capi.py
--- a/x-slam_amd/capi.py
+++ b/x-slam_amd/capi.py
@@ -112,6 +112,8 @@
     "xs_tsdf_band_workspace_bytes": (_sz, [C.c_int]),
     "xs_tsdf_gauss_newton_terms_band": (C.c_int, [C.c_int, C.POINTER(_vp), _sz, C.c_int, C.c_int, _f32p, C.c_float, _f32p, _f32p, C.c_float,
                                                   C.POINTER(BandIndex), _vp, _vp, _vp]),
+    "xs_tsdf_gauss_newton_terms_band_ex": (C.c_int, [C.c_int, C.POINTER(_vp), _sz, C.c_int, C.c_int, _f32p, C.c_float, _f32p, _f32p, C.c_float,
+                                                     C.POINTER(BandIndex), _vp, _vp, _vp, _vp]),
     "xs_tsdf_pose_hessian_workspace_bytes": (_sz, [C.c_int]),
     "xs_tsdf_pose_hessian_band": (C.c_int, [C.c_int, C.POINTER(_vp), _sz, C.c_int, C.c_int, _f32p, C.c_float, _f32p, _f32p, C.c_float,
                                             C.POINTER(BandIndex), _vp, _vp, _vp]),
@@ -721,6 +723,22 @@
                                              _stream(stream)))
 
 
+def tsdf_gauss_newton_terms_band_ex(depth_scaled, scaled_step, rows, cols, intr, voxel_size, Rv2c6, tv2c6, tranc_dist, index, workspace, out29,
+                                    stream=None, pose_mailbox=None, mailbox_seq=0, publish_host=None, publish_seq=0):
+    k = _fa(intr, 4)
+    o = GnOpts()
+    o.struct_bytes = C.sizeof(GnOpts)
+    o.mailbox_seq, o.pose_mailbox, o.publish_host, o.publish_seq = mailbox_seq, _ptr(pose_mailbox), _ptr(publish_host), publish_seq
+    if Rv2c6 is None:
+        pR = pt = None
+    else:
+        R, t = _fa(Rv2c6, 108), _fa(tv2c6, 36)
+        pR, pt = R.ctypes.data_as(_f32p), t.ctypes.data_as(_f32p)
+    P = (_vp * 1)(_ptr(depth_scaled))
+    check(_lib.xs_tsdf_gauss_newton_terms_band_ex(1, P, scaled_step, rows, cols, k.ctypes.data_as(_f32p), voxel_size, pR, pt, tranc_dist, C.byref(index),
+                                                  _ptr(workspace), _ptr(out29), C.byref(o), _stream(stream)))
+
+
 def gn_publish_bytes():
     return int(_lib.xs_gn_publish_bytes())
 
diff --git a/x-slam_amd/csrc/xs_band.hip b/x-slam_amd/csrc/xs_band.hip
--- a/x-slam_amd/csrc/xs_band.hip
+++ b/x-slam_amd/csrc/xs_band.hip
@@ -1,5 +1,6 @@
 #include <hip/hip_runtime.h>
 #include <string.h>
+#include <algorithm>
 #include <type_traits>
 #include <vector>
 #include "xs_gn_band.h"
@@ -44,29 +45,32 @@
     unsigned *tickets;
     double *out;
 };
-__global__ void __launch_bounds__(256) k_band_gauss_newton(const BandGnArgs g) {
+enum { GN_POSES_WORKSPACE = 0, GN_POSES_ARGUMENT = 1, GN_POSES_POSTED = 2 };
+template <int POSES>
+__global__ void __launch_bounds__(256) k_band_gauss_newton(const BandGnArgs g, const GnPoses Pk) {
     __shared__ GnPoses P;
     const int f = blockIdx.y, lane = threadIdx.x, wave = threadIdx.y;
-    const unsigned nblocks = gridDim.x, nseg = 4u * nblocks, seg = blockIdx.x * 4u + (unsigned)wave;
-    {
-        const float *src = reinterpret_cast<const float *>(g.poses + f);
-        float *dst = reinterpret_cast<float *>(&P);
-        for (int i = threadIdx.y * 64 + threadIdx.x; i < (int)(sizeof(GnPoses) / sizeof(float)); i += 256) dst[i] = src[i];
-        __syncthreads();
-    }
+    const unsigned nblocks = gridDim.x, nseg = 4u * nblocks, want = (unsigned)g.segs[2u * nseg + blockIdx.x];
+    const unsigned bid = want < nblocks ? want : blockIdx.x, seg = bid * 4u + (unsigned)wave;
+    bool left = false;
+    if constexpr (POSES == GN_POSES_POSTED) left = gn_poses_from_mailbox(g.a.mailbox, g.a.mailbox_seq, g.tickets + f, g.a.publish, blockIdx.x == 0 && f == 0, P);
+    else if constexpr (POSES == GN_POSES_ARGUMENT) gn_poses_from_argument(Pk, P);
+    else gn_poses_from_argument(g.poses[f], P);
     HessArgs a = g.a;
     a.depth = g.depth[f];
     double acc[29];
 #pragma unroll
     for (int k = 0; k < 29; ++k) acc[k] = 0.0;
-    const long long off = g.segs[seg], n = g.segs[nseg + seg];
-    for (long long e = lane; e < n; e += 64) {
-        const unsigned long long key = g.keys[off + e];
-        const int x = (int)(key & 0x1fffff), y = (int)((key >> 21) & 0x1fffff), z = (int)(key >> 42);
-        gn_terms_add(a, P, x, y, z, g.values[off + e], acc);
-    }
-    block_fold_and_finish_of<29>(acc, g.records + (size_t)f * nblocks * BAND_RECORD_DOUBLES, g.tickets + f, g.out + 29 * f, nullptr, 0, false,
-                                 nblocks, blockIdx.x);
+    if (!left) {
+        const long long off = g.segs[seg], n = g.segs[nseg + seg];
+        for (long long e = lane; e < n; e += 64) {
+            const unsigned long long key = g.keys[off + e];
+            const int x = (int)(key & 0x1fffff), y = (int)((key >> 21) & 0x1fffff), z = (int)(key >> 42);
+            gn_terms_add(a, P, x, y, z, g.values[off + e], acc);
+        }
+    }
+    block_fold_and_finish_of<29>(acc, g.records + (size_t)f * nblocks * BAND_RECORD_DOUBLES, g.tickets + f, g.out + 29 * f, g.a.publish, g.a.publish_seq, left,
+                                 nblocks, bid);
 }
 
 extern "C" size_t xs_tsdf_band_segs_bytes(const int *res, int z0, int z1) {
@@ -77,7 +81,7 @@
         if (hess_tiling(a, res, reinterpret_cast<const float *>(addr), z0, z1, grid, true)) return 0;
         most = grid.x > most ? grid.x : most;
     }
-    return (size_t)most * 4 * 2 * sizeof(long long);
+    return (size_t)most * (4 * 2 + 1) * sizeof(long long);
 }
 
 extern "C" int xs_tsdf_band_build(const float *gt, const int *res, int z0, int z1, xs_band_index *index, void *stream) {
@@ -106,6 +110,14 @@
     index->z0 = z0; index->z1 = z1;
     if (total > index->capacity) return XS_BAND_OVER_CAPACITY;
     XS_CHECK(hipMemcpyAsync(index->segs, segs.data(), nseg * sizeof(long long), hipMemcpyHostToDevice, st));
+    std::vector<long long> order(grid.x), longest(grid.x);
+    for (unsigned b = 0; b < grid.x; ++b) {
+        order[b] = b;
+        longest[b] = std::max(std::max(segs[nseg + 4 * b], segs[nseg + 4 * b + 1]), std::max(segs[nseg + 4 * b + 2], segs[nseg + 4 * b + 3]));
+    }
+    static const bool env_identity = exp_env_set("XS_BAND_IDENTITY_ORDER");
+    if (!env_identity) std::stable_sort(order.begin(), order.end(), [&](long long x, long long y) { return longest[(size_t)x] > longest[(size_t)y]; });
+    XS_CHECK(hipMemcpyAsync(index->segs + 2 * (size_t)nseg, order.data(), grid.x * sizeof(long long), hipMemcpyHostToDevice, st));
     hipLaunchKernelGGL(k_band_record<true>, grid, dim3(64, 4), 0, st, a, index->segs, index->keys, reinterpret_cast<unsigned *>(index->values));
     XS_CHECK(hipGetLastError());
     XS_CHECK(hipStreamSynchronize(st));
@@ -120,9 +132,19 @@
 extern "C" int xs_tsdf_gauss_newton_terms_band(int frames, const float *const *depth_scaled, size_t scaled_step, int rows, int cols, const float *intr4,
                                                float voxel_size, const float *Rv2c108xF, const float *tv2c36xF, float tranc_dist,
                                                const xs_band_index *index, void *workspace, double *out29xF_dev, void *stream) {
+    return xs_tsdf_gauss_newton_terms_band_ex(frames, depth_scaled, scaled_step, rows, cols, intr4, voxel_size, Rv2c108xF, tv2c36xF, tranc_dist, index, workspace,
+                                              out29xF_dev, nullptr, stream);
+}
+extern "C" int xs_tsdf_gauss_newton_terms_band_ex(int frames, const float *const *depth_scaled, size_t scaled_step, int rows, int cols, const float *intr4,
+                                                  float voxel_size, const float *Rv2c108xF, const float *tv2c36xF, float tranc_dist,
+                                                  const xs_band_index *index, void *workspace, double *out29xF_dev, const xs_gn_opts *opts, void *stream) {
+    if (opts && opts->struct_bytes != sizeof(xs_gn_opts)) return xs_set_error(hipErrorInvalidValue, "xs_tsdf_gauss_newton_terms_band_ex: opts->struct_bytes is not sizeof(xs_gn_opts)");
     if (frames < 1 || frames > XS_BAND_MAX_FRAMES) return xs_set_error(hipErrorInvalidValue, "xs_tsdf_gauss_newton_terms_band: frames outside 1 .. XS_BAND_MAX_FRAMES");
-    if (!depth_scaled || !intr4 || !Rv2c108xF || !tv2c36xF || !index || !workspace || !out29xF_dev)
+    if (opts && frames != 1) return xs_set_error(hipErrorInvalidValue, "xs_tsdf_gauss_newton_terms_band_ex: the loop protocol takes one frame");
+    const bool posted = opts && opts->pose_mailbox && !Rv2c108xF && !tv2c36xF;
+    if (!depth_scaled || !intr4 || !index || !workspace || !out29xF_dev)
         return xs_set_error(hipErrorInvalidValue, "xs_tsdf_gauss_newton_terms_band: null pointer");
+    if (!posted && (!Rv2c108xF || !tv2c36xF)) return xs_set_error(hipErrorInvalidValue, "xs_tsdf_gauss_newton_terms_band: give the six poses or a mailbox");
     if (index->nblocks < 1 || index->nblocks > XS_TSDF_REDUCE_MAX_BLOCKS_C || !index->segs || (index->count > 0 && (!index->keys || !index->values)))
         return xs_set_error(hipErrorInvalidValue, "xs_tsdf_gauss_newton_terms_band: the index was not built");
     BandGnArgs g;
@@ -136,18 +158,33 @@
     a.voxel_size = voxel_size; a.tranc_dist = tranc_dist; a.tranc_dist_inv = 1.0f / tranc_dist;
     a.intr = Intr{intr4[0], intr4[1], intr4[2], intr4[3]};
     a.X = index->res[0]; a.Y = index->res[1]; a.Z = index->res[2]; a.z0 = index->z0; a.z1 = index->z1;
-    std::vector<GnPoses> P((size_t)frames);
-    memset(P.data(), 0, P.size() * sizeof(GnPoses));
-    for (int f = 0; f < frames; ++f)
-        for (int k = 0; k < 6; ++k) { load_mat(Rv2c108xF + 108 * f + 18 * k, P[f].R[k]); load_vec(tv2c36xF + 36 * f + 6 * k, P[f].t[k]); }
     char *ws = static_cast<char *>(workspace);
     g.tickets = reinterpret_cast<unsigned *>(ws);
     g.poses = reinterpret_cast<const GnPoses *>(ws + BAND_POSES_OFFSET);
     g.records = reinterpret_cast<double *>(ws + band_records_offset());
     g.keys = index->keys; g.values = index->values; g.segs = index->segs; g.out = out29xF_dev;
     hipStream_t st = (hipStream_t)stream;
+    const dim3 grid((unsigned)index->nblocks, (unsigned)frames);
+    GnPoses Pk;
+    memset(&Pk, 0, sizeof(Pk));
+    if (opts) {
+        a.publish = opts->publish_host; a.publish_seq = opts->publish_seq;
+        if (posted) {
+            a.mailbox = static_cast<const unsigned *>(opts->pose_mailbox); a.mailbox_seq = opts->mailbox_seq;
+            hipLaunchKernelGGL(k_band_gauss_newton<GN_POSES_POSTED>, grid, dim3(64, 4), 0, st, g, Pk);
+        } else {
+            for (int k = 0; k < 6; ++k) { load_mat(Rv2c108xF + 18 * k, Pk.R[k]); load_vec(tv2c36xF + 6 * k, Pk.t[k]); }
+            hipLaunchKernelGGL(k_band_gauss_newton<GN_POSES_ARGUMENT>, grid, dim3(64, 4), 0, st, g, Pk);
+        }
+        XS_CHECK(hipGetLastError());
+        return 0;
+    }
+    std::vector<GnPoses> P((size_t)frames);
+    memset(P.data(), 0, P.size() * sizeof(GnPoses));
+    for (int f = 0; f < frames; ++f)
+        for (int k = 0; k < 6; ++k) { load_mat(Rv2c108xF + 108 * f + 18 * k, P[f].R[k]); load_vec(tv2c36xF + 36 * f + 6 * k, P[f].t[k]); }
     XS_CHECK(hipMemcpyAsync(ws + BAND_POSES_OFFSET, P.data(), P.size() * sizeof(GnPoses), hipMemcpyHostToDevice, st));
-    hipLaunchKernelGGL(k_band_gauss_newton, dim3((unsigned)index->nblocks, (unsigned)frames), dim3(64, 4), 0, st, g);
+    hipLaunchKernelGGL(k_band_gauss_newton<GN_POSES_WORKSPACE>, grid, dim3(64, 4), 0, st, g, Pk);
     XS_CHECK(hipGetLastError());
     return 0;
 }
diff --git a/x-slam_amd/csrc/xs_gn_band.h b/x-slam_amd/csrc/xs_gn_band.h
--- a/x-slam_amd/csrc/xs_gn_band.h
+++ b/x-slam_amd/csrc/xs_gn_band.h
@@ -1,6 +1,7 @@
 #pragma once
 #include "xs_device.h"
 #include "xs_env.h"
+#include "xs_mailbox.h"
 
 using namespace xs;
 #if defined(__HIP_DEVICE_COMPILE__) && !defined(__gfx942__) && !defined(__gfx950__)
@@ -212,6 +213,38 @@
 }
 
 struct GnPoses { MatS33 R[6]; cfloat3 t[6]; };
+__device__ __forceinline__ bool gn_poses_from_mailbox(const unsigned *mailbox, unsigned mailbox_seq, const unsigned *ticket, double *publish, bool first,
+                                                      GnPoses &P) {
+    __shared__ unsigned s_mail[xs::MAILBOX_WORDS];
+    __shared__ unsigned s_cmd;
+    if (threadIdx.y == 0) {
+        const int lane = threadIdx.x;
+        const unsigned long long t_resident = wall_clock64();
+        const bool somebody_left = (__hip_atomic_load(ticket, __ATOMIC_RELAXED, __HIP_MEMORY_SCOPE_AGENT) >> 16) != 0;
+        if (!somebody_left) xs::mailbox_wait(mailbox + 5 * xs::MAILBOX_WORDS, mailbox_seq, s_mail, lane);
+        if (publish && first && lane == 0)
+            __hip_atomic_store(&publish[30], (double)(wall_clock64() - t_resident), __ATOMIC_RELAXED, __HIP_MEMORY_SCOPE_SYSTEM);
+        unsigned cmd = somebody_left ? 1u : (unsigned)__builtin_amdgcn_readfirstlane((int)s_mail[1]);
+        float *dst = reinterpret_cast<float *>(&P);
+        for (int k = 0; k < 6 && cmd == 0; ++k) {
+            const unsigned w = __hip_atomic_load(mailbox + k * xs::MAILBOX_WORDS + (lane & 31), __ATOMIC_RELAXED, __HIP_MEMORY_SCOPE_SYSTEM);
+            const unsigned s0 = __builtin_amdgcn_readlane(w, 0), s1 = __builtin_amdgcn_readlane(w, 8), s2 = __builtin_amdgcn_readlane(w, 16),
+                           s3 = __builtin_amdgcn_readlane(w, 24);
+            if (s0 != mailbox_seq || s1 != mailbox_seq || s2 != mailbox_seq || s3 != mailbox_seq) { cmd = 2; break; }
+            const int f = xs::mailbox_float_of(lane & 31);
+            if (lane < 32 && f >= 0) dst[f < 18 ? 18 * k + f : 108 + 6 * k + (f - 18)] = __uint_as_float(w);
+        }
+        if (lane == 0) s_cmd = cmd;
+    }
+    __syncthreads();
+    return s_cmd != 0;
+}
+__device__ __forceinline__ void gn_poses_from_argument(const GnPoses &Pk, GnPoses &P) {
+    const float *src = reinterpret_cast<const float *>(&Pk);
+    float *dst = reinterpret_cast<float *>(&P);
+    for (int i = threadIdx.y * 64 + threadIdx.x; i < (int)(sizeof(GnPoses) / sizeof(float)); i += 256) dst[i] = src[i];
+    __syncthreads();
+}
 __device__ __forceinline__ bool tsdf_error_c(const HessArgs &a, const MatS33 &R, const cfloat3 &t, float vgx, float vgy, float vgz, float gt,
                                              cfloat &error) {
     cfloat3 v_g; v_g.x = cfloat(vgx); v_g.y = cfloat(vgy); v_g.z = cfloat(vgz);
diff --git a/x-slam_amd/csrc/xs_residual.hip b/x-slam_amd/csrc/xs_residual.hip
--- a/x-slam_amd/csrc/xs_residual.hip
+++ b/x-slam_amd/csrc/xs_residual.hip
@@ -49,36 +49,8 @@
 __global__ void __launch_bounds__(256) XS_GN_OCC k_tsdf_gauss_newton(const HessArgs a, const GnPoses Pk) {
     __shared__ GnPoses P;
     bool left = false;
-    if constexpr (POSTED) {
-        __shared__ unsigned s_mail[xs::MAILBOX_WORDS];
-        __shared__ unsigned s_cmd;
-        if (threadIdx.y == 0) {
-            const int lane = threadIdx.x;
-            const unsigned long long t_resident = wall_clock64();
-            const bool somebody_left = (__hip_atomic_load(a.ticket, __ATOMIC_RELAXED, __HIP_MEMORY_SCOPE_AGENT) >> 16) != 0;
-            if (!somebody_left) xs::mailbox_wait(a.mailbox + 5 * xs::MAILBOX_WORDS, a.mailbox_seq, s_mail, lane);
-            if (a.publish && blockIdx.x == 0 && lane == 0)
-                __hip_atomic_store(&a.publish[30], (double)(wall_clock64() - t_resident), __ATOMIC_RELAXED, __HIP_MEMORY_SCOPE_SYSTEM);
-            unsigned cmd = somebody_left ? 1u : (unsigned)__builtin_amdgcn_readfirstlane((int)s_mail[1]);
-            float *dst = reinterpret_cast<float *>(&P);
-            for (int k = 0; k < 6 && cmd == 0; ++k) {
-                const unsigned w = __hip_atomic_load(a.mailbox + k * xs::MAILBOX_WORDS + (lane & 31), __ATOMIC_RELAXED, __HIP_MEMORY_SCOPE_SYSTEM);
-                const unsigned s0 = __builtin_amdgcn_readlane(w, 0), s1 = __builtin_amdgcn_readlane(w, 8), s2 = __builtin_amdgcn_readlane(w, 16),
-                               s3 = __builtin_amdgcn_readlane(w, 24);
-                if (s0 != a.mailbox_seq || s1 != a.mailbox_seq || s2 != a.mailbox_seq || s3 != a.mailbox_seq) { cmd = 2; break; }
-                const int f = xs::mailbox_float_of(lane & 31);
-                if (lane < 32 && f >= 0) dst[f < 18 ? 18 * k + f : 108 + 6 * k + (f - 18)] = __uint_as_float(w);
-            }
-            if (lane == 0) s_cmd = cmd;
-        }
-        __syncthreads();
-        left = s_cmd != 0;
-    } else {
-        const float *src = reinterpret_cast<const float *>(&Pk);
-        float *dst = reinterpret_cast<float *>(&P);
-        for (int i = threadIdx.y * 64 + threadIdx.x; i < (int)(sizeof(GnPoses) / sizeof(float)); i += 256) dst[i] = src[i];
-        __syncthreads();
-    }
+    if constexpr (POSTED) left = gn_poses_from_mailbox(a.mailbox, a.mailbox_seq, a.ticket, a.publish, blockIdx.x == 0, P);
+    else gn_poses_from_argument(Pk, P);
     double acc[29];
 #pragma unroll
     for (int k = 0; k < 29; ++k) acc[k] = 0.0;
diff --git a/x-slam_amd/host/KinectFusionReconstruction.cpp b/x-slam_amd/host/KinectFusionReconstruction.cpp
--- a/x-slam_amd/host/KinectFusionReconstruction.cpp
+++ b/x-slam_amd/host/KinectFusionReconstruction.cpp
@@ -125,6 +125,8 @@
     raycast_builds_pyramid = config.as<bool>("raycast_builds_pyramid", true);
     gn_post_pose = config.as<bool>("gn_post_pose", true);
     gn_publish_sharded = config.as<bool>("gn_publish_sharded", true);
+    gn_band_loop = config.as<bool>("gn_band_loop", true);
+    gn_band_build_passes = std::max(1, config.as<int>("gn_band_build_passes", 4));
     profile_integrate_every = std::max(1, config.as<int>("profile_integrate_every", 4));
     AllocateBuffers();
     tsdf_volume_d_ptr = new TsdfVolume(Vector3i(resolutionX, resolutionY, zs1 - zs0), voxel_size, thres_range);
diff --git a/x-slam_amd/host/KinectFusionReconstruction.h b/x-slam_amd/host/KinectFusionReconstruction.h
--- a/x-slam_amd/host/KinectFusionReconstruction.h
+++ b/x-slam_amd/host/KinectFusionReconstruction.h
@@ -127,7 +127,9 @@
     long long gn_passes = 0, gn_kernel_calls = 0;
     double gn_poll_us = 0;
     long long gn_poll_passes = 0;
-    const float *GaussNewtonPrepare(const DeviceArray2D<ushort> &depth_frame_d);
+    bool gn_band_loop = true;
+    int gn_band_build_passes = 4;
+    const float *GaussNewtonPrepare(const DeviceArray2D<ushort> &depth_frame_d, int passes);
     void GaussNewtonEnqueue(const DeviceArray2D<ushort> &depth_frame_d, const float *gt, const float (*R)[18], const float (*t)[6], unsigned mail_seq,
                             unsigned long long seq);
     bool GaussNewtonWait(unsigned long long seq, double out29[29]);
@@ -230,6 +232,7 @@
         DeviceArray2D<float> score_depth;
     } reloc_;
     const float *GaussNewtonDenseView();
+    bool BandIndexValid() const;
     void BandIndexPrepare();
     size_t BandBatchPrepare(const std::vector<DeviceArray2D<ushort>> &depths);
     void GaussNewtonBandLaunch(const int *frames, int n, const Matrix4cf *camera2volume, size_t scaled_step, int rows, int cols, double *raw);
diff --git a/x-slam_amd/host/gn_host.hpp b/x-slam_amd/host/gn_host.hpp
--- a/x-slam_amd/host/gn_host.hpp
+++ b/x-slam_amd/host/gn_host.hpp
@@ -49,6 +49,12 @@
     return true;
 }
 
+inline bool gn_take_band(bool index_valid, int passes, int build_passes, bool dense_only) {
+    if (dense_only || passes < 1) return false;
+    if (index_valid) return true;
+    return passes >= std::max(build_passes, 1);
+}
+
 inline int gn_loop_step(const double s[29], int p, int iterations, float damping, xs_host::Matrix4cf &camera2volume, std::vector<double> *loss_history) {
     if (loss_history) loss_history->push_back(s[28] > 0 ? s[27] / s[28] : 0.0);
     if (p == iterations) return 1;
diff --git a/x-slam_amd/host/kf_relocalize.cpp b/x-slam_amd/host/kf_relocalize.cpp
--- a/x-slam_amd/host/kf_relocalize.cpp
+++ b/x-slam_amd/host/kf_relocalize.cpp
@@ -17,18 +17,23 @@
     hipSafeCall(hipStreamSynchronize(st));
 }
 
-const float *KinectFusionReconstruction::GaussNewtonPrepare(const DeviceArray2D<ushort> &depth_frame_d) {
+const float *KinectFusionReconstruction::GaussNewtonPrepare(const DeviceArray2D<ushort> &depth_frame_d, int passes) {
     hipStream_t st = current_stream();
     depthRawScaled_d.create(depth_frame_d.rows(), depth_frame_d.cols());
     check_rc(xs_scale_depth(depth_frame_d.ptr(), depth_frame_d.step(), depth_frame_d.rows(), depth_frame_d.cols(), depthRawScaled_d.ptr(),
                             depthRawScaled_d.step(), st), "scaleDepth");
     if (reloc_.gn_sums.size() < 32) reloc_.gn_sums.create(32);
-    ensure_reduce_workspace(reloc_.gn_ws, xs_tsdf_reduce_workspace_bytes(), "reduce workspace");
     if (!reloc_.gn_publish) {
         hipSafeCall(hipHostMalloc((void **)&reloc_.gn_publish, xs_gn_publish_bytes(), hipHostMallocCoherent | hipHostMallocMapped));
         std::memset(reloc_.gn_publish, 0, xs_gn_publish_bytes());
     }
     if (!reloc_.gn_mailbox && gn_post_pose) check_rc(xs_icp_mailbox_alloc(&reloc_.gn_mailbox, &reloc_.gn_mailbox_in_device), "Gauss-Newton mailbox");
+    if (gn_take_band(BandIndexValid(), passes, gn_band_build_passes, !gn_band_loop)) {
+        BandIndexPrepare();
+        ensure_reduce_workspace(reloc_.band_ws, xs_tsdf_band_workspace_bytes(XS_BAND_MAX_FRAMES), "band workspace");
+        return nullptr;
+    }
+    ensure_reduce_workspace(reloc_.gn_ws, xs_tsdf_reduce_workspace_bytes(), "reduce workspace");
     return GaussNewtonDenseView();
 }
 const float *KinectFusionReconstruction::GaussNewtonDenseView() {
@@ -58,9 +63,16 @@
         reloc_.gn_events.push_back({e0, e1});
         hipSafeCall(hipEventRecord(e0, st));
     }
-    check_rc(xs_tsdf_gauss_newton_terms_ex(depthRawScaled_d.ptr(), depthRawScaled_d.step(), depth_frame_d.rows(), depth_frame_d.cols(), &kinect_intrinsic.fx,
-                                           res3(), voxel_size, R ? &R[0][0] : nullptr, t ? &t[0][0] : nullptr, tsdf_volume_d_ptr->getTsdfTruncDist(), gt, zo0,
-                                           zo1, reloc_.gn_ws.ptr(), reloc_.gn_sums.ptr(), &o, st), "GaussNewtonTerms");
+    if (gt) {
+        check_rc(xs_tsdf_gauss_newton_terms_ex(depthRawScaled_d.ptr(), depthRawScaled_d.step(), depth_frame_d.rows(), depth_frame_d.cols(), &kinect_intrinsic.fx,
+                                               res3(), voxel_size, R ? &R[0][0] : nullptr, t ? &t[0][0] : nullptr, tsdf_volume_d_ptr->getTsdfTruncDist(), gt, zo0,
+                                               zo1, reloc_.gn_ws.ptr(), reloc_.gn_sums.ptr(), &o, st), "GaussNewtonTerms");
+    } else {
+        const float *depth = depthRawScaled_d.ptr();
+        check_rc(xs_tsdf_gauss_newton_terms_band_ex(1, &depth, depthRawScaled_d.step(), depth_frame_d.rows(), depth_frame_d.cols(), &kinect_intrinsic.fx, voxel_size,
+                                                    R ? &R[0][0] : nullptr, t ? &t[0][0] : nullptr, tsdf_volume_d_ptr->getTsdfTruncDist(), &reloc_.band,
+                                                    reloc_.band_ws.ptr(), reloc_.gn_sums.ptr(), &o, st), "GaussNewtonTermsBand");
+    }
     if (e1) hipSafeCall(hipEventRecord(e1, st));
     if (sharded && gn_publish_sharded) {
         collective(collective_user, 0, reloc_.gn_sums.ptr(), 29);
@@ -88,7 +100,7 @@
 
 int KinectFusionReconstruction::GaussNewtonTerms(const DeviceArray2D<ushort> &depth_frame_d, const Matrix4cf &camera2volume, double out29[29]) {
     if (!tsdf_volume_d_ptr) return 0;
-    const float *gt = GaussNewtonPrepare(depth_frame_d);
+    const float *gt = GaussNewtonPrepare(depth_frame_d, 1);
     float R[6][18], t[6][6];
     gn_seeded_poses(camera2volume, R, t);
     const unsigned long long seq = ++reloc_.gn_seq;
@@ -103,7 +115,7 @@
     if (!tsdf_volume_d_ptr) return 0;
     const int passes = iterations + (loss_history ? 1 : 0);
     if (passes <= 0) return 1;
-    const float *gt = GaussNewtonPrepare(depth_frame_d);
+    const float *gt = GaussNewtonPrepare(depth_frame_d, passes);
     const bool ahead = gn_post_pose && shard_count == 1 && reloc_.gn_mailbox && reloc_.gn_mailbox_in_device;
     float R[6][18], t[6][6];
     gn_seeded_poses(camera2volume, R, t);
@@ -147,8 +159,9 @@
     return rc;
 }
 
+bool KinectFusionReconstruction::BandIndexValid() const { return reloc_.band_key == BandKey{volume_generation} && reloc_.band.nblocks > 0; }
 void KinectFusionReconstruction::BandIndexPrepare() {
-    if (reloc_.band_key == BandKey{volume_generation} && reloc_.band.nblocks > 0) return;
+    if (BandIndexValid()) return;
     hipStream_t st = current_stream();
     const int *res = res3();
     const float *gt = GaussNewtonDenseView();
```
